# deweylab/RSEM

Hardware: AMD Instinct MI355X
Metric: EM read-alignments/s (nnz x EM iterations per second), rsem-run-em theta-only rounds (higher is better)
Workload: dtype f64; 1 GPU; BASELINE configs[2] (PairedEndQModel-shaped, the north-star target config): EM matrix of 50000000 reads x 200000 transcripts, 570042118 alignments (11.40/read) per GPU, frozen conprb (rounds >= 12); synthetic_config=C3, kernel=0, parallelism=1 GPU

## Files before the change

### rsem_amd/csrc/em.hip

```cpp
#include <climits>
#include <cstdlib>
#include <cmath>
#include <type_traits>

#include "comm_internal.hpp"
#include "em_internal.hpp"
#include "upload.hpp"
#include "sell_layout.hpp"

namespace {

using rsem::kEpsilon;

constexpr int kReduceBlocks = 64;
constexpr int kMaxTimedRounds = 4096;
constexpr int kWindow = 2048;
static_assert(kWindow == kLayoutWindow, "the layout sorts reads apart and sizes windows for the E step's LDS window (sell_layout.hpp)");

constexpr int kTotSlots = 64;

struct Ctrl {
    int done;
    int final_round;
    int totNum;
// ... 256 lines not shown
constexpr int kCloseMax = 128;
__device__ inline void solo_close_round(const SoloArgs& A, int M, double N0, const double* __restrict__ cur) {
    const int n_close = min((int)gridDim.x, kCloseMax);
    const int stride = (int)gridDim.x / n_close;
    const int rel = (int)blockIdx.x - stride / 2;
    if (rel < 0 || rel % stride != 0 || rel / stride >= n_close) return;
    const int me = rel / stride;
    const int lane = threadIdx.x & 63;
    const int n = M + 1;
    const int per = (n + n_close - 1) / n_close;
    const int lo = me * per, hi = min(n, lo + per);
    constexpr int kPre = 8;
    double pc[kPre], pp[kPre];
    const bool pre = per <= kPre * kBlock;
    if (pre) {
#pragma unroll
        for (int k = 0; k < kPre; k++) {
            const int i = lo + (int)threadIdx.x + kBlock * k;
            pc[k] = i < hi ? cur[i] : 0.0;
            pp[k] = i < hi ? A.prev[i] : 0.0;
        }
    }
    const double extra_c = wave_sum(cur[n + lane]) + N0, sum_c = wave_sum(cur[n + kTotSlots + lane]) + N0;
    const double extra_p = wave_sum(A.prev[n + lane]) + N0, sum_p = wave_sum(A.prev[n + kTotSlots + lane]) + N0;
    int tot = 0;
    double bmax = 0.0, csum = 0.0;
    auto one = [&](int i, double craw, double praw) {
        csum += craw + (i == 0 ? extra_c : 0.0);
        const double th = (craw + (i == 0 ? extra_c : 0.0)) / sum_c;
        const double old = (praw + (i == 0 ? extra_p : 0.0)) / sum_p;
        A.prev[i] = 0.0;
        if (old >= 1e-7) {
            const double change = fabs(th - old) / old;
            if (change >= 0.001) ++tot;
            bmax = fmax(bmax, change);
        }
    };
    if (pre) {
#pragma unroll
        for (int k = 0; k < kPre; k++) {
            const int i = lo + (int)threadIdx.x + kBlock * k;
            if (i < hi) one(i, pc[k], pp[k]);
        }
    } else {
        for (int i = lo + threadIdx.x; i < hi; i += kBlock) one(i, cur[i], A.prev[i]);
    }
    for (int d = 32; d >= 1; d >>= 1) {
        tot += __shfl_xor(tot, d);
        bmax = fmax(bmax, __shfl_xor(bmax, d));
    }
    csum = wave_sum(csum);
    __shared__ int s_tot[kBlock / 64];
    __shared__ double s_b[kBlock / 64], s_c[kBlock / 64];
    if (lane == 0) { s_tot[threadIdx.x >> 6] = tot; s_b[threadIdx.x >> 6] = bmax; s_c[threadIdx.x >> 6] = csum; }
    __syncthreads();
    if (threadIdx.x == 0) {
        for (int i = 1; i < kBlock / 64; i++) { tot += s_tot[i]; bmax = fmax(bmax, s_b[i]); csum += s_c[i]; }
        Ctrl* ctrl = A.ctrl;
        unsigned int zero = 0;
        if (bmax > 0.0) {
            const unsigned long long was = __hip_atomic_fetch_max(&ctrl->bbits, (unsigned long long)__double_as_longlong(bmax),
                                                                  __ATOMIC_RELAXED, __HIP_MEMORY_SCOPE_AGENT);
            asm volatile("v_and_b32 %0, 0, %1" : "=v"(zero) : "v"((unsigned int)was));
        }
        zero += sum_slot_put(ctrl, me, csum);
        const unsigned long long old = __hip_atomic_fetch_add(&ctrl->tick2, (((unsigned long long)(unsigned)tot << 32) | 1ull) + zero,
                                                              __ATOMIC_RELAXED, __HIP_MEMORY_SCOPE_AGENT);
        if ((int)(old & 0xffffffffull) == n_close - 1) {
            const int round = A.stat_round;
            const int totNum = (int)(old >> 32) + tot;
            const unsigned long long bb = __hip_atomic_load(&ctrl->bbits, __ATOMIC_RELAXED, __HIP_MEMORY_SCOPE_AGENT);
            const double fsum = sum_slots_take(ctrl, n_close);
            ctrl->last_sum = fsum;
            ctrl->last_bchange = __longlong_as_double((long long)bb);
            ctrl->last_totNum = totNum;
            ctrl->last_round = round;
            const bool stop = !(round < A.min_round || (totNum > 0 && round < A.max_round));
            if (stop) {
                ctrl->done = 1;
                ctrl->final_round = round;
            }
            if (A.mirror) {
                RoundStat* h = &A.mirror->hist[(round - 1) % kHistCap];
                h->sum = fsum;
                h->bchange = __longlong_as_double((long long)bb);
                h->totNum = totNum;
                h->round = round;
                if (stop) A.mirror->final_round = round;
                __hip_atomic_store(&A.mirror->last_round, round, __ATOMIC_RELEASE, __HIP_MEMORY_SCOPE_SYSTEM);
                if (stop) __hip_atomic_store(&A.mirror->done, 1, __ATOMIC_RELEASE, __HIP_MEMORY_SCOPE_SYSTEM);
            }
            __hip_atomic_store(&ctrl->bbits, 0ull, __ATOMIC_RELAXED, __HIP_MEMORY_SCOPE_AGENT);
            __hip_atomic_store(&ctrl->tick2, 0ull, __ATOMIC_RELAXED, __HIP_MEMORY_SCOPE_AGENT);
            for (int k = 0; k < 2 * kTotSlots; k++) A.prev[n + k] = 0.0;
        }
    }
}

__global__ __launch_bounds__(kBlock) void k_solo_finish(int32_t M, double N0, const double* __restrict__ buf, double* theta, double* counts_last) {
    const int n = M + 1;
    const int lane = threadIdx.x & 63;
    const double extra0 = wave_sum(buf[n + lane]) + N0, sum = wave_sum(buf[n + kTotSlots + lane]) + N0;
    const int i = blockIdx.x * blockDim.x + threadIdx.x;
    if (i < n) {
        const double c = buf[i] + (i == 0 ? extra0 : 0.0);
        counts_last[i] = c;
        theta[i] = c / sum;
    }
}

#ifndef RSEM_FQ_DEPTH
#define RSEM_FQ_DEPTH 3
#endif
constexpr int kFarQDepth = RSEM_FQ_DEPTH;
template <bool kFC, bool kSolo = false, bool kFQ = false>
__global__ __launch_bounds__(kBlock) void k_estep_lane(
    const Shape* __restrict__ shapes, const Unit* __restrict__ units, uint32_t T, int M,
    const double* __restrict__ theta, const double* __restrict__ tsrc, double N0, const unsigned char* __restrict__ sval,
    const int16_t* __restrict__ sexp, const int32_t* __restrict__ ssid, const double* __restrict__ sncp,
    const unsigned long long* __restrict__ masks, double* counts, double* noise_partial, double* totals, const Ctrl* ctrl,
    unsigned long long* trace, SoloArgs solo = SoloArgs(), XArgs xa = XArgs()) {
    if (ctrl->done) return;
    if (trace && threadIdx.x == 0) trace[2 * blockIdx.x] = wall_clock64();
    __shared__ double th_win[kWindow];
    __shared__ double cnt_win[kWindow];
    __shared__ int fq_sid[kFQ ? (kBlock / 64) * kFarQCap : 1];
    __shared__ double fq_val[kFQ ? (kBlock / 64) * kFarQCap : 1];
    __shared__ int fq_n[kBlock / 64];
    const Unit U = units[blockIdx.x];
    const int lane = threadIdx.x & 63;
    const int w = __builtin_amdgcn_readfirstlane((int)(threadIdx.x >> 6));
    FarQueue fq;
    if (kFQ) {
        fq.sid = fq_sid + w * kFarQCap;
        fq.val = fq_val + w * kFarQCap;
        fq.n = fq_n + w;
        if (lane == 0) fq_n[w] = 0;
    }
    if (kSolo && solo.stat_round > 0) solo_close_round(solo, M, N0, theta);
    double noise = 0.0, neff = 0.0;
    {
        const Shape& G = U.S;
        Shape S;
        S.plane_base = G.plane_base;
        S.slice_base = G.slice_base;
        S.n_slices = G.n_slices;
        S.row_base = 0;
        S.n_rows = 0;
        S.slot_base = G.slot_base;
        S.K = G.K;
        S.lg = G.lg;
        S.fmt = G.fmt;
        S.val_base = G.val_base;
        const uint32_t u_end = S.slice_base + U.slice_begin + U.n_slices;
        const uint32_t s_begin = S.slice_base + U.slice_begin + (uint32_t)w * U.per_wave;
        const uint32_t s_end = min(u_end, s_begin + U.per_wave);
#define RSEM_ESTEP_BLOCK(KK, QQ, FF, XX) \
    estep_block<KK, kFC, QQ, (QQ ? kQ32Depth[KK - 1] : kF64Depth[KK - 1]), FF, XX>(S, s_begin, s_end, lane, U.base, U.span, theta, tsrc, N0, th_win, cnt_win, sval, sexp, ssid, sncp, masks, counts, noise, neff, M, xa)
#define RSEM_ESTEP_BLOCK_FQ(KK, QQ, XX) \
    estep_block<KK, kFC, QQ, kFarQDepth, true, XX, true>(S, s_begin, s_end, lane, U.base, U.span, theta, tsrc, N0, th_win, cnt_win, sval, sexp, ssid, sncp, masks, counts, noise, neff, M, xa, fq)
        const int code = (S.K - 1) | ((S.fmt == kFmtQ32 ? 1 : 0) << 2) | ((U.pad[0] != 0 ? 1 : 0) << 3) | (((!kFC && S.fmt == kFmtF64X) ? 1 : 0) << 4);
        if constexpr (kFQ) {
            if (s_begin < u_end) switch ((code & 7) | ((code >> 4) << 3)) {
                case 0: RSEM_ESTEP_BLOCK_FQ(1, false, false); break;
                case 1: RSEM_ESTEP_BLOCK_FQ(2, false, false); break;
                case 2: RSEM_ESTEP_BLOCK_FQ(3, false, false); break;
                case 3: RSEM_ESTEP_BLOCK_FQ(4, false, false); break;
                case 4: RSEM_ESTEP_BLOCK_FQ(1, true, false); break;
                case 5: RSEM_ESTEP_BLOCK_FQ(2, true, false); break;
                case 6: RSEM_ESTEP_BLOCK_FQ(3, true, false); break;
                case 7: RSEM_ESTEP_BLOCK_FQ(4, true, false); break;
                default:
                    if constexpr (!kFC) switch (code & 3) {
                        case 0: RSEM_ESTEP_BLOCK_FQ(1, false, true); break;
                        case 1: RSEM_ESTEP_BLOCK_FQ(2, false, true); break;
                        case 2: RSEM_ESTEP_BLOCK_FQ(3, false, true); break;
                        default: RSEM_ESTEP_BLOCK_FQ(4, false, true); break;
                    }
                    break;
            } else {
                const ThetaSrc th = theta_src<kFC>(theta, tsrc, N0, lane);
                stage_windows<kFC>(U.base, U.span, M, th, th_win, cnt_win);
            }
        } else
        if (s_begin < u_end) switch (code) {
            case 0: RSEM_ESTEP_BLOCK(1, false, false, false); break;
            case 1: RSEM_ESTEP_BLOCK(2, false, false, false); break;
            case 2: RSEM_ESTEP_BLOCK(3, false, false, false); break;
            case 3: RSEM_ESTEP_BLOCK(4, false, false, false); break;
            case 4: RSEM_ESTEP_BLOCK(1, true, false, false); break;
            case 5: RSEM_ESTEP_BLOCK(2, true, false, false); break;
            case 6: RSEM_ESTEP_BLOCK(3, true, false, false); break;
            case 7: RSEM_ESTEP_BLOCK(4, true, false, false); break;
            case 8: RSEM_ESTEP_BLOCK(1, false, true, false); break;
            case 9: RSEM_ESTEP_BLOCK(2, false, true, false); break;
            case 10: RSEM_ESTEP_BLOCK(3, false, true, false); break;
            case 11: RSEM_ESTEP_BLOCK(4, false, true, false); break;
            case 12: RSEM_ESTEP_BLOCK(1, true, true, false); break;
            case 13: RSEM_ESTEP_BLOCK(2, true, true, false); break;
            case 14: RSEM_ESTEP_BLOCK(3, true, true, false); break;
            case 15: RSEM_ESTEP_BLOCK(4, true, true, false); break;
            default:
                if constexpr (!kFC) switch (code & 11) {
                    case 0: RSEM_ESTEP_BLOCK(1, false, false, true); break;
                    case 1: RSEM_ESTEP_BLOCK(2, false, false, true); break;
                    case 2: RSEM_ESTEP_BLOCK(3, false, false, true); break;
                    case 3: RSEM_ESTEP_BLOCK(4, false, false, true); break;
                    case 8: RSEM_ESTEP_BLOCK(1, false, true, true); break;
                    case 9: RSEM_ESTEP_BLOCK(2, false, true, true); break;
                    case 10: RSEM_ESTEP_BLOCK(3, false, true, true); break;
                    default: RSEM_ESTEP_BLOCK(4, false, true, true); break;
                }
                break;
#undef RSEM_ESTEP_BLOCK
#undef RSEM_ESTEP_BLOCK_FQ
        } else {
            const ThetaSrc th = theta_src<kFC>(theta, tsrc, N0, lane);
            stage_windows<kFC>(U.base, U.span, M, th, th_win, cnt_win);
        }
    }
    __syncthreads();
    for (int i = threadIdx.x; i < U.span; i += blockDim.x) {
        const double v = cnt_win[i];
        if (v != 0.0) unsafeAtomicAdd(&counts[U.base + i], v);
    }
    block_add_totals(noise, neff, noise_partial, totals);
    if (trace && threadIdx.x == 0) trace[2 * blockIdx.x + 1] = wall_clock64();
}


__device__ inline double block_sum_det(double v) {
    __shared__ double red[kBlock / 64];
    __syncthreads();
    v = wave_sum(v);
    if ((threadIdx.x & 63) == 0) red[threadIdx.x >> 6] = v;
    __syncthreads();
    double t = 0.0;
    for (int i = 0; i < kBlock / 64; i++) t += red[i];
    return t;
}

__global__ __launch_bounds__(kBlock) void k_mstep_reduce(int32_t M, double N0, double* counts,
                                                          const double* __restrict__ noise_a, int n_a,
                                                          const double* __restrict__ noise_b, int n_b,
                                                          double* partials, const Ctrl* ctrl) {
    if (ctrl && ctrl->done) return;
    const int n = M + 1;
    const int per = (n + gridDim.x - 1) / gridDim.x;
    const int lo = blockIdx.x * per, hi = min(n, lo + per);
    if (blockIdx.x == 0) {
        double v = 0.0;
        for (int i = threadIdx.x; i < n_a; i += blockDim.x) v += noise_a[i];
        for (int i = threadIdx.x; i < n_b; i += blockDim.x) v += noise_b[i];
        double t = block_sum_det(v);
        if (threadIdx.x == 0) counts[0] = counts[0] + t + N0;
        __syncthreads();
    }
    double v = 0.0;
    for (int i = lo + threadIdx.x; i < hi; i += blockDim.x) v += counts[i];
    double t = block_sum_det(v);
    if (threadIdx.x == 0) partials[blockIdx.x] = t;
}

__global__ __launch_bounds__(kBlock) void k_mstep_apply(int32_t M, const double* __restrict__ partials,
                                                         int n_partials, double* counts,
                                                         const double* __restrict__ theta_old,
                                                         double* theta_new, double* counts_last, Ctrl* ctrl,
                                                         int round, int min_round, int max_round) {
    if (ctrl->done) return;
    double sum = 0.0;
    for (int i = 0; i < n_partials; i++) sum += partials[i];
    int tot = 0;
    double bmax = 0.0;
    for (int i = blockIdx.x * blockDim.x + threadIdx.x; i <= M; i += gridDim.x * blockDim.x) {
        double c = counts[i];
        double th = c / sum;
        theta_new[i] = th;
        counts_last[i] = c;
        counts[i] = 0.0;
        double old = theta_old[i];
        if (old >= 1e-7) {
            double change = fabs(th - old) / old;
            if (change >= 0.001) ++tot;
            bmax = fmax(bmax, change);
        }
    }
    __shared__ int s_tot[kBlock / 64];
    __shared__ double s_b[kBlock / 64];
    for (int d = 32; d >= 1; d >>= 1) {
        tot += __shfl_xor(tot, d);
        bmax = fmax(bmax, __shfl_xor(bmax, d));
    }
    if ((threadIdx.x & 63) == 0) { s_tot[threadIdx.x >> 6] = tot; s_b[threadIdx.x >> 6] = bmax; }
    __syncthreads();
    if (threadIdx.x == 0) {
        for (int i = 1; i < kBlock / 64; i++) { tot += s_tot[i]; bmax = fmax(bmax, s_b[i]); }
        if (tot) atomicAdd(&ctrl->totNum, tot);
        atomicMax(&ctrl->bbits, (unsigned long long)__double_as_longlong(bmax));
        __threadfence();
        unsigned int t = atomicAdd(&ctrl->ticket, 1u);
        if (t == gridDim.x - 1) {
            int totNum = atomicAdd(&ctrl->totNum, 0);
            unsigned long long bb = atomicMax(&ctrl->bbits, 0ull);
            ctrl->last_sum = sum;
            ctrl->last_bchange = __longlong_as_double((long long)bb);
            ctrl->last_totNum = totNum;
// ... 84 lines not shown
        unsigned int tk = atomicAdd(&ctrl->ticket, 1u);
        if (tk == gridDim.x - 1) {
            int totNum = atomicAdd(&ctrl->totNum, 0);
            unsigned long long bb = atomicMax(&ctrl->bbits, 0ull);
            ctrl->last_sum = sum;
            ctrl->last_bchange = __longlong_as_double((long long)bb);
            ctrl->last_totNum = totNum;
            ctrl->last_round = round;
            if (!(round < min_round || (totNum > 0 && round < max_round))) {
                ctrl->done = 1;
                ctrl->final_round = round;
            }
            atomicExch(&ctrl->totNum, 0);
            atomicExch(&ctrl->bbits, 0ull);
            atomicExch(&ctrl->ticket, 0u);
            atomicExch(&ctrl->bar, 0u);
        }
    }
}

template <bool kFused>
__global__ __launch_bounds__(kBlock) void k_mstep_fast(int32_t M, double N0, double* counts, double* totals,
                                                        const double* __restrict__ theta_old, double* theta_new,
                                                        double* counts_last, Ctrl* ctrl, int round, int min_round, int max_round,
                                                        HostMirror* mirror, double* spent) {
    if (ctrl->done) return;
    const int n = M + 1;
    const int nb = gridDim.x;
    const int per = (n + nb - 1) / nb;
    const int lo = blockIdx.x * per, hi = min(n, lo + per);
    __shared__ double s_totals[2];
    if (threadIdx.x < 64) {
        double a = __hip_atomic_load(&totals[threadIdx.x], __ATOMIC_RELAXED, __HIP_MEMORY_SCOPE_AGENT);
        double b = __hip_atomic_load(&totals[kTotSlots + threadIdx.x], __ATOMIC_RELAXED, __HIP_MEMORY_SCOPE_AGENT);
        a = wave_sum(a);
        b = wave_sum(b);
        if (threadIdx.x == 0) { s_totals[0] = a; s_totals[1] = b; }
    }
    constexpr int kPre = 8;
    const bool pre = (hi - lo) <= kPre * (int)blockDim.x;
    double pc[kPre], po[kPre];
    if (pre) {
#pragma unroll
        for (int k = 0; k < kPre; k++) {
            const int i = lo + (int)threadIdx.x + k * (int)blockDim.x;
            pc[k] = i < hi ? counts[i] : 0.0;
            po[k] = i < hi ? theta_old[i] : 0.0;
        }
    }
    __syncthreads();
    const double extra0 = s_totals[0] + N0;
    const double sum = s_totals[1] + N0;
    int tot = 0;
    double bmax = 0.0, csum = 0.0;
    auto one = [&](int i, double craw, double old) {
        const double c = craw + (i == 0 ? extra0 : 0.0);
        csum += c;
        const double th = c / sum;
        theta_new[i] = th;
        counts_last[i] = c;
        if (kFused) spent[i] = 0.0;
        else counts[i] = 0.0;
        if (old >= 1e-7) {
            const double change = fabs(th - old) / old;
            if (change >= 0.001) ++tot;
            bmax = fmax(bmax, change);
        }
    };
    if (kFused && blockIdx.x == 0 && threadIdx.x < 2 * kTotSlots) spent[n + threadIdx.x] = 0.0;
    if (pre) {
#pragma unroll
        for (int k = 0; k < kPre; k++) {
            const int i = lo + (int)threadIdx.x + k * (int)blockDim.x;
            if (i < hi) one(i, pc[k], po[k]);
        }
    } else {
        for (int i = lo + threadIdx.x; i < hi; i += blockDim.x) one(i, counts[i], theta_old[i]);
    }
    __shared__ int s_tot[kBlock / 64];
    __shared__ double s_b[kBlock / 64], s_c[kBlock / 64];
    for (int d = 32; d >= 1; d >>= 1) {
        tot += __shfl_xor(tot, d);
        bmax = fmax(bmax, __shfl_xor(bmax, d));
    }
    csum = wave_sum(csum);
    __shared__ int s_last;
    if ((threadIdx.x & 63) == 0) { s_tot[threadIdx.x >> 6] = tot; s_b[threadIdx.x >> 6] = bmax; s_c[threadIdx.x >> 6] = csum; }
    if (threadIdx.x == 0) s_last = 0;
    __syncthreads();
    if (threadIdx.x == 0) {
        for (int i = 1; i < kBlock / 64; i++) { tot += s_tot[i]; bmax = fmax(bmax, s_b[i]); csum += s_c[i]; }
        unsigned int zero = 0;
        if (bmax > 0.0) {
            const unsigned long long was = __hip_atomic_fetch_max(&ctrl->bbits, (unsigned long long)__double_as_longlong(bmax),
                                                                  __ATOMIC_RELAXED, __HIP_MEMORY_SCOPE_AGENT);
            asm volatile("v_and_b32 %0, 0, %1" : "=v"(zero) : "v"((unsigned int)was));
        }
        zero += sum_slot_put(ctrl, (int)blockIdx.x, csum);
        const unsigned long long old = __hip_atomic_fetch_add(&ctrl->tick2, (((unsigned long long)(unsigned)tot << 32) | 1ull) + zero,
                                                              __ATOMIC_RELAXED, __HIP_MEMORY_SCOPE_AGENT);
        if ((unsigned)(old & 0xffffffffull) == gridDim.x - 1) {
            const int totNum = (int)(old >> 32) + tot;
            const unsigned long long bb = __hip_atomic_load(&ctrl->bbits, __ATOMIC_RELAXED, __HIP_MEMORY_SCOPE_AGENT);
            const double fsum = sum_slots_take(ctrl, (int)gridDim.x);
            ctrl->last_sum = fsum;
            ctrl->last_bchange = __longlong_as_double((long long)bb);
            ctrl->last_totNum = totNum;
            ctrl->last_round = round;
            const bool stop = !(round < min_round || (totNum > 0 && round < max_round));
            if (stop) {
                ctrl->done = 1;
                ctrl->final_round = round;
            }
            if (mirror) {
                RoundStat* h = &mirror->hist[(round - 1) % kHistCap];
                h->sum = fsum;
                h->bchange = __longlong_as_double((long long)bb);
                h->totNum = totNum;
                h->round = round;
                if (stop) mirror->final_round = round;
                __hip_atomic_store(&mirror->last_round, round, __ATOMIC_RELEASE, __HIP_MEMORY_SCOPE_SYSTEM);
                if (stop) __hip_atomic_store(&mirror->done, 1, __ATOMIC_RELEASE, __HIP_MEMORY_SCOPE_SYSTEM);
            }
            __hip_atomic_store(&ctrl->bbits, 0ull, __ATOMIC_RELAXED, __HIP_MEMORY_SCOPE_AGENT);
            __hip_atomic_store(&ctrl->tick2, 0ull, __ATOMIC_RELAXED, __HIP_MEMORY_SCOPE_AGENT);
            s_last = 1;
        }
    }
    __syncthreads();
    if (!kFused && s_last && threadIdx.x < 2 * kTotSlots) __hip_atomic_store(&totals[threadIdx.x], 0.0, __ATOMIC_RELAXED, __HIP_MEMORY_SCOPE_AGENT);
}

}


struct rsem_em_ctx {
    int device = 0;
    int32_t M = 0;
    uint64_t N1 = 0, nnz = 0;
    hipStream_t stream = nullptr;
    bool own_stream = true;
    uint64_t* d_row_ptr = nullptr;
    int32_t* d_sid = nullptr;
    double* d_cp = nullptr;
    double* d_ncp = nullptr;
    bool have_values = false;
    SellLayout L;
    unsigned char* d_sval = nullptr;
    double* d_sncp = nullptr;
    int16_t* d_sexp = nullptr;
    int* d_fill_err = nullptr;
    int value_bits = 64;
    int value_range_bits = 8;
    bool layout_has_q32 = false;
    bool layout_ok = false;
    Unit* d_units = nullptr;
    unsigned long long* d_trace = nullptr;
    std::vector<Unit> h_units;
    uint64_t long_nnz = 0;
    uint32_t* d_rank = nullptr;
    double *d_xextra = nullptr, *d_xinv = nullptr;
    int split_rows = 1;
    int split_policy = 1;
    uint32_t n_far_units = 0;
    unsigned long long n_stray_reads = 0;
    int tune_passes_left = 1;
    uint32_t n_units = 0;
    uint32_t n_units_main = 0;
    uint32_t n_units_compact = 0;
    uint32_t n_units_queued = 0;
    int far_queue = 1;
    hipStream_t stream_x = nullptr;
    hipEvent_t ev_x_fork = nullptr, ev_x_join = nullptr;
    int x_overlap = 0;
    int noise_n = 0;
    size_t noise_cap = 0;
    double* d_theta[2] = {nullptr, nullptr};
    double* d_red3 = nullptr;
    double* d_red = nullptr;
    double* d_counts = nullptr;
    double* d_counts_last = nullptr;
    double* d_noise_a = nullptr;
    double* d_noise_b = nullptr;
    double* d_totals = nullptr;
    bool use_totals = false;
    double* d_partials = nullptr;
    double* d_w = nullptr;
    double* d_wn = nullptr;
    Ctrl* d_ctrl = nullptr;
    int grid_main = 0, grid_long = 0, grid_apply = 0;
    int kernel = RSEM_EM_KERNEL_AUTO;
    uint32_t forced_T = 0;
    int check_every = 64;
    int n_cus = 256;
    std::vector<hipEvent_t> events;
    HostMirror* mirror = nullptr;
    hipEvent_t lag_ev[2] = {nullptr, nullptr};
    hipStream_t stream2 = nullptr;
    hipEvent_t ev_e[4] = {nullptr, nullptr, nullptr, nullptr}, ev_s[4] = {nullptr, nullptr, nullptr, nullptr};
    rsem_comm* comm = nullptr;
    bool csr_released = false;
    int views_out = 0;
    rsem_em_progress_fn progress = nullptr;
    void* progress_user = nullptr;
};

namespace {

int resolved_kernel(const rsem_em_ctx* c) {
    return c->kernel == RSEM_EM_KERNEL_AUTO ? RSEM_EM_KERNEL_LANE : c->kernel;
}

bool same_unit(const Unit& a, const Unit& b) {
    return a.shape == b.shape && a.slice_begin == b.slice_begin && a.n_slices == b.n_slices && a.per_wave == b.per_wave && a.base == b.base &&
           a.span == b.span && a.pad[0] == b.pad[0] && a.pad[1] == b.pad[1] && !memcmp(&a.S, &b.S, sizeof(Shape));
}

int partition_units(rsem_em_ctx* c) {
    auto is_main = [](const Unit& u) { return u.S.fmt != kFmtF64X; };
    const auto mid = std::stable_partition(c->h_units.begin(), c->h_units.end(), is_main);
    c->n_units_main = (uint32_t)(mid - c->h_units.begin());
    auto queued = [](const Unit& u) { return u.pad[0] != 0 && (uint64_t)u.pad[1] <= 48ull * u.n_slices; };
    c->n_units_queued = (uint32_t)std::count_if(c->h_units.begin(), mid, queued);
    c->n_units_compact = c->n_units_main;
    if (c->far_queue && c->n_units_queued * 25ull >= c->n_units_main && c->n_units_queued)
        c->n_units_compact = (uint32_t)(std::stable_partition(c->h_units.begin(), mid, [&](const Unit& u) { return !queued(u); }) - c->h_units.begin());
    if (c->n_units)
        RSEM_HIP_TRY(hipMemcpyAsync(c->d_units, c->h_units.data(), sizeof(Unit) * c->n_units, hipMemcpyHostToDevice, c->stream));
    RSEM_HIP_TRY(hipStreamSynchronize(c->stream));
    return RSEM_OK;
}

int launch_estep(rsem_em_ctx* c, const double* d_theta, double* d_counts, hipStream_t st, bool use_ctrl) {
    const Ctrl* ctrl = c->d_ctrl;
    (void)use_ctrl;
    c->noise_n = (int)c->n_units;
    {
        XArgs xa;
        const uint32_t nc = c->n_units_compact, n_main = c->n_units_main, n_all = c->n_units;
        const bool far_launch = c->far_queue && nc < n_main;
        const bool x_beside = c->x_overlap && c->L.n_x_rows && n_main > 0 && n_main < n_all;
        const bool second = c->stream_x && (x_beside || (far_launch && nc > 0));
        hipStream_t s2 = second ? c->stream_x : st;
        hipStream_t sx = x_beside ? s2 : st, sf = far_launch ? s2 : st;
        if (second) {
            RSEM_HIP_TRY(hipEventRecord(c->ev_x_fork, st));
            RSEM_HIP_TRY(hipStreamWaitEvent(s2, c->ev_x_fork, 0));
        }
        auto lane = [&](uint32_t u0, uint32_t u1, hipStream_t s) {
            if (u1 > u0)
                hipLaunchKernelGGL((k_estep_lane<false, false>), dim3(u1 - u0), dim3(kBlock), 0, s, c->L.d_shapes, c->d_units + u0, c->L.T, c->M,
                                   d_theta, (const double*)nullptr, 0.0, (const unsigned char*)c->d_sval, (const int16_t*)c->d_sexp, c->L.d_ssid,
                                   c->d_sncp, c->L.d_masks, d_counts, c->d_noise_a + u0, c->use_totals ? c->d_totals : nullptr, ctrl,
                                   c->d_trace ? c->d_trace + 2 * (size_t)u0 : nullptr, SoloArgs(), xa);
        };
        auto lane_fq = [&](uint32_t u0, uint32_t u1, hipStream_t s) {
            if (u1 > u0)
                hipLaunchKernelGGL((k_estep_lane<false, false, true>), dim3(u1 - u0), dim3(kBlock), 0, s, c->L.d_shapes, c->d_units + u0, c->L.T, c->M,
                                   d_theta, (const double*)nullptr, 0.0, (const unsigned char*)c->d_sval, (const int16_t*)c->d_sexp, c->L.d_ssid,
                                   c->d_sncp, c->L.d_masks, d_counts, c->d_noise_a + u0, c->use_totals ? c->d_totals : nullptr, ctrl,
                                   c->d_trace ? c->d_trace + 2 * (size_t)u0 : nullptr, SoloArgs(), xa);
        };
        if (c->L.n_x_rows) {
            xa.extra = c->d_xextra; xa.inv = c->d_xinv; xa.slot_base = c->L.x_slot_base;
            static const bool batched = !(getenv("RSEM_HIP_ROWSUM_BATCHED") && atoi(getenv("RSEM_HIP_ROWSUM_BATCHED")) == 0);
            hipLaunchKernelGGL(batched ? k_far_rowsum<true> : k_far_rowsum<false>, dim3(rsem::ceil_div(c->L.n_x_slots, kBlock)), dim3(kBlock), 0, sx, c->L.n_x_slots,
                               (const uint64_t*)c->L.d_far_ptr, (const int32_t*)c->L.d_far_sid, (const double*)c->L.d_far_cp, d_theta, c->d_xextra, ctrl);
        }
        if (far_launch) lane_fq(nc, n_main, sf);
        if (!far_launch && sx == st) lane(0, n_all, st);
        else {
            lane(0, far_launch ? nc : n_main, st);
            lane(n_main, n_all, sx);
        }
        if (c->L.n_far) {
            const int grid = std::max(1, rsem::ceil_div(c->L.n_far, kBlock * 4));
            static const bool xcd = !(getenv("RSEM_HIP_COLSUM_XCD") && atoi(getenv("RSEM_HIP_COLSUM_XCD")) == 0);
            hipLaunchKernelGGL(xcd ? k_far_colsum<true> : k_far_colsum<false>, dim3(grid), dim3(kBlock), 0, sx, c->L.n_far, (const int32_t*)c->L.d_csc_sid,
                               (const double*)c->L.d_csc_cp, (const uint32_t*)c->L.d_csc_slot, c->L.x_slot_base, d_theta, (const double*)c->d_xinv, d_counts, ctrl);
        }
        if (second) {
            RSEM_HIP_TRY(hipGetLastError());
            RSEM_HIP_TRY(hipEventRecord(c->ev_x_join, s2));
            RSEM_HIP_TRY(hipStreamWaitEvent(st, c->ev_x_join, 0));
        }
    }
    RSEM_HIP_TRY(hipGetLastError());
    if (c->L.n_long_rows) {
        hipLaunchKernelGGL(k_estep_long, dim3(c->grid_long), dim3(kBlock), 0, st, (uint64_t)c->L.n_long_rows,
                           (const uint32_t*)(c->L.d_order + c->L.n_sell_rows), (const uint64_t*)c->d_row_ptr, (const int32_t*)c->d_sid, (const double*)c->d_cp,
                           (const double*)c->d_ncp, d_theta, d_counts, c->d_noise_b, ctrl, c->use_totals ? c->d_totals : nullptr);
        RSEM_HIP_TRY(hipGetLastError());
    }
    return RSEM_OK;
}

int n_noise_b(const rsem_em_ctx* c) {
    return c->L.n_long_rows ? c->grid_long : 0;
}

int launch_weights(rsem_em_ctx* c, const double* d_theta, hipStream_t st) {
    const int grid = std::max(1, std::min<int>(c->n_cus * 16, rsem::ceil_div(c->N1, kBlock)));
    hipLaunchKernelGGL(k_weights_csr, dim3(grid), dim3(kBlock), 0, st, c->N1, c->d_row_ptr, c->d_sid, c->d_cp, c->d_ncp, d_theta,
                       c->d_w, c->d_wn);
    RSEM_HIP_TRY(hipGetLastError());
    return RSEM_OK;
}

int launch_mstep(rsem_em_ctx* c, double N0, double* d_counts, const double* d_theta_old, double* d_theta_new,
                 int round, int min_round, int max_round, hipStream_t st, HostMirror* mirror = nullptr) {
    const int grid = std::max(1, std::min(kMstepBlocks, rsem::ceil_div((uint64_t)c->M + 1, kBlock * 4)));
    if (c->use_totals) {
        const int gridf = std::max(1, std::min(2 * kMstepBlocks, rsem::ceil_div((uint64_t)c->M + 1, kBlock * 2)));
        hipLaunchKernelGGL(k_mstep_fast<false>, dim3(gridf), dim3(kBlock), 0, st, c->M, N0, d_counts, c->d_totals, d_theta_old, d_theta_new,
                           c->d_counts_last, c->d_ctrl, round, min_round, max_round, mirror, (double*)nullptr);
        RSEM_HIP_TRY(hipGetLastError());
        return RSEM_OK;
    }
    hipLaunchKernelGGL(k_mstep_fused, dim3(grid), dim3(kBlock), 0, st, c->M, N0, d_counts, c->d_noise_a, c->noise_n,
                       c->d_noise_b, n_noise_b(c), c->d_partials, d_theta_old, d_theta_new, c->d_counts_last, c->d_ctrl,
                       round, min_round, max_round);
    RSEM_HIP_TRY(hipGetLastError());
    return RSEM_OK;
}

int build_layout(rsem_em_ctx* c);
void free_layout(rsem_em_ctx* c);

__global__ void k_sum_row_lengths(uint32_t n, const uint32_t* __restrict__ rows, const uint64_t* __restrict__ row_ptr, unsigned long long* out) {
    unsigned long long v = 0;
    for (uint32_t i = blockIdx.x * blockDim.x + threadIdx.x; i < n; i += gridDim.x * blockDim.x) v += row_ptr[rows[i] + 1] - row_ptr[rows[i]];
    for (int d = 32; d >= 1; d >>= 1) v += __shfl_xor(v, d);
    if ((threadIdx.x & 63) == 0 && v) atomicAdd(out, v);
}

int release_csr(rsem_em_ctx* c) {
    if (c->csr_released) return RSEM_OK;
    const char* why = nullptr;
    if (!c->layout_ok || !c->have_values) why = "there is no layout with values yet";
    else if (c->layout_has_q32 || c->value_bits == 32) why = "Q32 planes hold rounded values";
    else if (c->L.n_x_rows) why = "split rows keep part of their alignments outside the planes";
    else if (c->L.n_long_rows) why = "reads with more than 256 alignments live in the CSR alone";
    else if (c->views_out > 0) why = "a model context still holds the arrays";
    if (why) { rsem::set_last_error("release_csr: %s", why); return RSEM_ERR_STATE; }
    RSEM_HIP_TRY(hipSetDevice(c->device));
    RSEM_HIP_TRY(hipStreamSynchronize(c->stream));
    (void)hipFree(c->d_sid); c->d_sid = nullptr;
    (void)hipFree(c->d_cp); c->d_cp = nullptr;
    c->csr_released = true;
    return RSEM_OK;
}

int ensure_csr(rsem_em_ctx* c) {
    if (!c->csr_released) return RSEM_OK;
    RSEM_HIP_TRY(hipSetDevice(c->device));
    RSEM_HIP_TRY(dmalloc(&c->d_sid, c->nnz));
    if (hipError_t e = dmalloc(&c->d_cp, c->nnz); e != hipSuccess) {
        (void)hipFree(c->d_sid);
        c->d_sid = nullptr;
        RSEM_HIP_TRY(e);
    }
    if (c->L.n_sell_rows)
        hipLaunchKernelGGL(k_unfill_sell, dim3(rsem::ceil_div(c->L.n_sell_rows, kBlock)), dim3(kBlock), 0, c->stream, c->L.d_shapes, c->L.n_shapes, c->L.T,
                           c->L.n_sell_rows, (const uint32_t*)c->L.d_order, (const uint64_t*)c->d_row_ptr, (const int32_t*)c->L.d_ssid,
                           (const unsigned char*)c->d_sval, c->d_sid, c->d_cp);
    RSEM_HIP_TRY(hipGetLastError());
    RSEM_HIP_TRY(hipStreamSynchronize(c->stream));
    c->csr_released = false;
    return RSEM_OK;
}

int write_values(rsem_em_ctx* c) {
    if (c->d_fill_err) RSEM_HIP_TRY(hipMemsetAsync(c->d_fill_err, 0, sizeof(int), c->stream));
    int rc = sell_fill_values(c->L, c->stream, c->d_row_ptr, c->d_cp, c->d_ncp, c->d_sval, c->d_sncp, c->d_sexp, c->d_fill_err, c->d_sid);
    if (rc != RSEM_OK) return rc;
    if (c->layout_has_q32) {
        int h = 0;
        RSEM_HIP_TRY(hipMemcpyAsync(&h, c->d_fill_err, sizeof(int), hipMemcpyDeviceToHost, c->stream));
        RSEM_HIP_TRY(hipStreamSynchronize(c->stream));
        if (h) { rsem::set_last_error("Q32 planes: a read's values left the range its format was chosen for"); return RSEM_ERR_STATE; }
    }
    return RSEM_OK;
}

int fill_values(rsem_em_ctx* c) {
    if (c->value_bits == 32 || c->layout_has_q32) {
        free_layout(c);
        return build_layout(c);
    }
    return write_values(c);
}

void free_layout(rsem_em_ctx* c) {
    sell_free(c->L);
    hipFree(c->d_rank); hipFree(c->d_xextra); hipFree(c->d_xinv);
    c->d_rank = nullptr; c->d_xextra = nullptr; c->d_xinv = nullptr;
    hipFree(c->d_sval); hipFree(c->d_sncp); hipFree(c->d_sexp); hipFree(c->d_fill_err); hipFree(c->d_units); hipFree(c->d_noise_a);
    c->d_sval = nullptr; c->d_sncp = nullptr; c->d_sexp = nullptr; c->d_fill_err = nullptr; c->d_units = nullptr; c->d_noise_a = nullptr;
    c->h_units.clear();
    c->n_units = 0;
    c->layout_has_q32 = false;
    c->layout_ok = false;
}

int build_layout(rsem_em_ctx* c) {
    const uint32_t target_waves = (uint32_t)c->n_cus * 4 * 6 * 5 / 2;
    const bool q32 = c->value_bits == 32 && c->have_values;
    std::vector<Unit> units;
    int split = c->split_rows && resolved_kernel(c) == RSEM_EM_KERNEL_LANE && !q32;
    if (const char* e = getenv("RSEM_HIP_SPLIT")) split = split && atoi(e) != 0;
    if (split) split = c->split_policy;
    if (const char* e = getenv("RSEM_HIP_SPLIT_POLICY")) { if (split) split = !strcmp(e, "all") ? 2 : 1; }
    int rc = sell_build_refined(c->L, c->stream, c->N1, c->M, c->d_row_ptr, c->d_sid, target_waves, c->forced_T,
                                q32 ? c->d_cp : nullptr, c->value_range_bits, kWindow, units, &c->d_units, &c->n_stray_reads, split);
    if (rc != RSEM_OK) return rc;
    if (c->L.n_x_rows) {
        const size_t nxs = (size_t)(c->L.n_slots - c->L.x_slot_base);
        RSEM_HIP_TRY(dmalloc(&c->d_xextra, nxs));
        RSEM_HIP_TRY(dmalloc(&c->d_xinv, nxs));
        RSEM_HIP_TRY(hipMemsetAsync(c->d_xextra, 0, sizeof(double) * std::max<size_t>(nxs, 1), c->stream));
        RSEM_HIP_TRY(hipMemsetAsync(c->d_xinv, 0, sizeof(double) * std::max<size_t>(nxs, 1), c->stream));
    }
    c->layout_has_q32 = q32;
    RSEM_HIP_TRY(hipMalloc((void**)&c->d_sval, std::max<uint64_t>(c->L.val_bytes, 1)));
    RSEM_HIP_TRY(dmalloc(&c->d_sncp, (size_t)c->L.n_slots));
    if (q32) {
        RSEM_HIP_TRY(dmalloc(&c->d_sexp, (size_t)c->L.n_slots));
        RSEM_HIP_TRY(dmalloc(&c->d_fill_err, 1));
    }
    RSEM_HIP_TRY(hipMemsetAsync(c->d_sval, 0, c->L.val_bytes, c->stream));
    RSEM_HIP_TRY(hipMemsetAsync(c->d_sncp, 0, sizeof(double) * c->L.n_slots, c->stream));
    if (c->have_values) {
        rc = write_values(c);
        if (rc != RSEM_OK) return rc;
    }
    RSEM_HIP_TRY(hipStreamSynchronize(c->stream));
    c->n_units = (uint32_t)units.size();
    c->h_units = units;
    if (const char* e = getenv("RSEM_HIP_X_OVERLAP")) c->x_overlap = atoi(e);
    if (const char* e = getenv("RSEM_HIP_FAR_QUEUE")) c->far_queue = atoi(e);
    rc = partition_units(c);
    if (rc != RSEM_OK) return rc;
    if ((c->L.n_x_rows || c->n_units_compact < c->n_units_main) && !c->stream_x) {
        RSEM_HIP_TRY(hipStreamCreateWithFlags(&c->stream_x, hipStreamNonBlocking));
        RSEM_HIP_TRY(hipEventCreateWithFlags(&c->ev_x_fork, hipEventDisableTiming));
        RSEM_HIP_TRY(hipEventCreateWithFlags(&c->ev_x_join, hipEventDisableTiming));
    }
    c->tune_passes_left = 1;
    if (const char* e = getenv("RSEM_HIP_TUNE")) c->tune_passes_left = atoi(e);
    c->n_far_units = 0;
    for (const Unit& u : c->h_units) c->n_far_units += u.pad[0] != 0;
    c->noise_cap = std::max<size_t>((size_t)c->n_cus * 8, c->n_units);
    RSEM_HIP_TRY(dmalloc(&c->d_noise_a, c->noise_cap));
    RSEM_HIP_TRY(hipMemsetAsync(c->d_noise_a, 0, sizeof(double) * c->noise_cap, c->stream));

    c->grid_long = std::max(1, std::min<int>(c->n_cus * 8, rsem::ceil_div(c->L.n_long_rows, kBlock / 64)));
    c->long_nnz = 0;
    if (c->L.n_long_rows) {
        unsigned long long* d_n = (unsigned long long*)c->d_noise_a;
        hipLaunchKernelGGL(k_sum_row_lengths, dim3(c->grid_long), dim3(kBlock), 0, c->stream, c->L.n_long_rows, c->L.d_order + c->L.n_sell_rows,
                           c->d_row_ptr, d_n);
        RSEM_HIP_TRY(hipGetLastError());
        unsigned long long h = 0;
        RSEM_HIP_TRY(hipMemcpyAsync(&h, d_n, sizeof(h), hipMemcpyDeviceToHost, c->stream));
        RSEM_HIP_TRY(hipMemsetAsync(c->d_noise_a, 0, sizeof(double), c->stream));
        RSEM_HIP_TRY(hipStreamSynchronize(c->stream));
        c->long_nnz = h;
    }
    c->layout_ok = true;
    return RSEM_OK;
}

void set_grid_for_kernel(rsem_em_ctx* c) {
    c->grid_main = std::max(1, std::min<int>(c->n_cus * 8, rsem::ceil_div(c->L.n_slices, kBlock / 64)));
}

}

extern "C" {

int rsem_em_create(rsem_em_ctx** out, int device, int32_t M, uint64_t N1, uint64_t nnz, const uint64_t* row_ptr,
                   const int32_t* sid, const double* conprb, const double* ncp) {
    RSEM_REQUIRE(out != nullptr, "out is NULL");
    *out = nullptr;
    RSEM_REQUIRE(M >= 1, "M must be >= 1");
    RSEM_REQUIRE(row_ptr != nullptr && (sid != nullptr || nnz == 0), "row_ptr / sid is NULL");
    RSEM_REQUIRE(N1 < 0xfffffff0ull, "N1 too large for one shard (max 2^32-16 reads)");
    RSEM_REQUIRE(row_ptr[0] == 0 && row_ptr[N1] == nnz, "row_ptr[0] != 0 or row_ptr[N1] != nnz");
    RSEM_REQUIRE((conprb == nullptr) == (ncp == nullptr), "conprb and ncp must be given together");
    int ndev = 0;
    if (hipGetDeviceCount(&ndev) != hipSuccess || device < 0 || device >= ndev) {
        (void)hipGetLastError();
        rsem::set_last_error("no HIP device %d (have %d)", device, ndev);
        return RSEM_ERR_NODEVICE;
    }
    RSEM_HIP_TRY(hipSetDevice(device));
    hipDeviceProp_t prop;
    RSEM_HIP_TRY(hipGetDeviceProperties(&prop, device));
    rsem_em_ctx* c = new (std::nothrow) rsem_em_ctx();
    if (!c) return RSEM_ERR_NOMEM;
    c->device = device;
    c->M = M;
    c->N1 = N1;
    c->nnz = nnz;
    c->n_cus = prop.multiProcessorCount > 0 ? prop.multiProcessorCount : 256;
    int rc = RSEM_OK;
    auto fail = [&](int code) { rsem_em_destroy(c); return code; };
#define TRY_OR_FAIL(expr)                                                                               \
    do {                                                                                                \
        hipError_t _e = (expr);                                                                         \
        if (_e != hipSuccess) {                                                                         \
            rsem::set_last_error("%s:%d: %s -> %s", __FILE__, __LINE__, #expr, hipGetErrorString(_e));  \
            return fail(_e == hipErrorOutOfMemory ? RSEM_ERR_NOMEM : RSEM_ERR_HIP);                     \
        }                                                                                               \
    } while (0)
    TRY_OR_FAIL(hipStreamCreateWithFlags(&c->stream, hipStreamNonBlocking));
    TRY_OR_FAIL(dmalloc(&c->d_row_ptr, N1 + 1));
    TRY_OR_FAIL(dmalloc(&c->d_sid, nnz));
    TRY_OR_FAIL(dmalloc(&c->d_cp, nnz));
    TRY_OR_FAIL(dmalloc(&c->d_ncp, N1));
    if ((rc = rsem::staged_h2d(c->d_row_ptr, row_ptr, sizeof(uint64_t) * (N1 + 1), c->stream)) != RSEM_OK) return fail(rc);
    if ((rc = rsem::staged_h2d(c->d_sid, sid, sizeof(int32_t) * nnz, c->stream)) != RSEM_OK) return fail(rc);
    if (conprb) {
        if ((rc = rsem::staged_h2d(c->d_cp, conprb, sizeof(double) * nnz, c->stream)) != RSEM_OK) return fail(rc);
        if ((rc = rsem::staged_h2d(c->d_ncp, ncp, sizeof(double) * N1, c->stream)) != RSEM_OK) return fail(rc);
        c->have_values = true;
    }
    for (int i = 0; i < 2; i++) TRY_OR_FAIL(dmalloc(&c->d_theta[i], (size_t)M + 1));
    TRY_OR_FAIL(dmalloc(&c->d_red3, 3 * ((size_t)M + 1 + 2 * kTotSlots)));
    c->d_red = c->d_red3;
    c->d_counts = c->d_red;
    c->d_totals = c->d_red + (size_t)M + 1;
    TRY_OR_FAIL(dmalloc(&c->d_counts_last, (size_t)M + 1));
    TRY_OR_FAIL(dmalloc(&c->d_noise_b, (size_t)c->n_cus * 8));
    TRY_OR_FAIL(hipMemsetAsync(c->d_totals, 0, sizeof(double) * 2 * kTotSlots, c->stream));
    TRY_OR_FAIL(hipHostMalloc((void**)&c->mirror, sizeof(HostMirror), hipHostMallocDefault));
    memset(c->mirror, 0, sizeof(HostMirror));
    for (int i = 0; i < 2; i++) TRY_OR_FAIL(hipEventCreateWithFlags(&c->lag_ev[i], hipEventDisableTiming));
    {
        int least = 0, greatest = 0;
        TRY_OR_FAIL(hipDeviceGetStreamPriorityRange(&least, &greatest));
        TRY_OR_FAIL(hipStreamCreateWithPriority(&c->stream2, hipStreamNonBlocking, greatest));
    }
    for (int i = 0; i < 4; i++) {
        TRY_OR_FAIL(hipEventCreateWithFlags(&c->ev_e[i], hipEventDisableTiming));
        TRY_OR_FAIL(hipEventCreateWithFlags(&c->ev_s[i], hipEventDisableTiming));
    }
    TRY_OR_FAIL(dmalloc(&c->d_partials, 2 * kReduceBlocks));
    TRY_OR_FAIL(dmalloc(&c->d_ctrl, 1));
    TRY_OR_FAIL(hipMemsetAsync(c->d_counts, 0, sizeof(double) * ((size_t)M + 1), c->stream));
    TRY_OR_FAIL(hipMemsetAsync(c->d_noise_b, 0, sizeof(double) * c->n_cus * 8, c->stream));
    TRY_OR_FAIL(hipMemsetAsync(c->d_ctrl, 0, sizeof(Ctrl), c->stream));
    c->grid_apply = std::max(1, std::min(c->n_cus * 2, rsem::ceil_div((uint64_t)M + 1, kBlock)));
    if (const char* e = getenv("RSEM_HIP_T")) c->forced_T = (uint32_t)atoi(e);
    rc = build_layout(c);
    if (rc != RSEM_OK) return fail(rc);
    set_grid_for_kernel(c);
    rsem::thread_stager().release();
#undef TRY_OR_FAIL
    *out = c;
    return RSEM_OK;
}

int rsem_em_set_values(rsem_em_ctx* c, const double* conprb, const double* ncp) {
    RSEM_REQUIRE(c && conprb && ncp, "NULL argument");
    RSEM_HIP_TRY(hipSetDevice(c->device));
    { int rc0 = ensure_csr(c); if (rc0 != RSEM_OK) return rc0; }
    if (c->nnz) RSEM_HIP_TRY(hipMemcpyAsync(c->d_cp, conprb, sizeof(double) * c->nnz, hipMemcpyHostToDevice, c->stream));
    if (c->N1) RSEM_HIP_TRY(hipMemcpyAsync(c->d_ncp, ncp, sizeof(double) * c->N1, hipMemcpyHostToDevice, c->stream));
    c->have_values = true;
    int rc = fill_values(c);
    if (rc != RSEM_OK) return rc;
    RSEM_HIP_TRY(hipStreamSynchronize(c->stream));
    return RSEM_OK;
}

int rsem_em_get_values(rsem_em_ctx* c, double* conprb, double* ncp) {
    RSEM_REQUIRE(c && conprb && ncp, "NULL argument");
    if (!c->have_values) { rsem::set_last_error("CSR values were never set"); return RSEM_ERR_STATE; }
    RSEM_HIP_TRY(hipSetDevice(c->device));
    { int rc0 = ensure_csr(c); if (rc0 != RSEM_OK) return rc0; }
    if (c->nnz) RSEM_HIP_TRY(hipMemcpyAsync(conprb, c->d_cp, sizeof(double) * c->nnz, hipMemcpyDeviceToHost, c->stream));
    if (c->N1) RSEM_HIP_TRY(hipMemcpyAsync(ncp, c->d_ncp, sizeof(double) * c->N1, hipMemcpyDeviceToHost, c->stream));
    RSEM_HIP_TRY(hipStreamSynchronize(c->stream));
    return RSEM_OK;
}

int rsem_em_shard_rows(uint64_t N1, const uint64_t* row_ptr, int world, uint64_t* bounds) {
    RSEM_REQUIRE(row_ptr && bounds && world >= 1, "bad argument");
    const uint64_t nhT = row_ptr[N1] / (uint64_t)world;
    uint64_t cur = 0;
    bounds[0] = 0;
    for (int i = 0; i < world; i++) {
        const uint64_t left_threads = (uint64_t)(world - i - 1);
        if (i == world - 1) cur = N1;
        else {
            const uint64_t cap = N1 > left_threads ? N1 - left_threads : 0;
            const uint64_t target = row_ptr[cur] + nhT;
            uint64_t nxt = (uint64_t)(std::lower_bound(row_ptr + cur, row_ptr + N1 + 1, target) - row_ptr);
            nxt = std::min(nxt, std::max(cap, cur));
            cur = std::max(cur, nxt);
        }
        bounds[i + 1] = cur;
    }
    return RSEM_OK;
}

int rsem_em_set_comm(rsem_em_ctx* c, rsem_comm* comm) {
    RSEM_REQUIRE(c != nullptr, "NULL argument");
    c->comm = comm;
    return RSEM_OK;
}

int rsem_em_set_progress(rsem_em_ctx* c, rsem_em_progress_fn fn, void* user) {
    RSEM_REQUIRE(c != nullptr, "NULL argument");
    c->progress = fn;
    c->progress_user = user;
    return RSEM_OK;
}

int rsem_em_set_option(rsem_em_ctx* c, const char* key, int64_t value) {
    RSEM_REQUIRE(c && key, "NULL argument");
    if (!strcmp(key, "release_csr")) {
        RSEM_REQUIRE(value == 0 || value == 1, "release_csr must be 0 or 1");
        return value ? release_csr(c) : ensure_csr(c);
    }
    if (!strcmp(key, "kernel") || !strcmp(key, "split_rows") || !strcmp(key, "split_policy") || !strcmp(key, "value_bits") || !strcmp(key, "value_range_bits")) {
        int rc0 = ensure_csr(c);
        if (rc0 != RSEM_OK) return rc0;
    }
    if (!strcmp(key, "kernel")) {
        RSEM_REQUIRE(value >= RSEM_EM_KERNEL_AUTO && value <= RSEM_EM_KERNEL_LANE, "unknown kernel variant");
        RSEM_REQUIRE(value == RSEM_EM_KERNEL_AUTO || value == RSEM_EM_KERNEL_LANE, "kernel variants CSR (1) and SELL (2) were retired: AUTO (0) or LANE (3)");
        c->kernel = (int)value;
        if (c->layout_ok && c->L.n_x_rows && resolved_kernel(c) != RSEM_EM_KERNEL_LANE) {
            RSEM_HIP_TRY(hipSetDevice(c->device));
            free_layout(c);
            int rc = build_layout(c);
            if (rc != RSEM_OK) return rc;
        }
        set_grid_for_kernel(c);
        return RSEM_OK;
    }
    if (!strcmp(key, "split_overlap")) {
        RSEM_REQUIRE(value == 0 || value == 1, "split_overlap must be 0 or 1");
        c->x_overlap = (int)value;
        return RSEM_OK;
    }
    if (!strcmp(key, "split_policy")) {
        RSEM_REQUIRE(value == 1 || value == 2, "split_policy must be 1 (reads mostly outside their window) or 2 (every read with an id outside)");
        if (c->split_policy == (int)value) return RSEM_OK;
        c->split_policy = (int)value;
        c->x_overlap = value == 2 ? 1 : 0;
        RSEM_HIP_TRY(hipSetDevice(c->device));
        free_layout(c);
        int rc = build_layout(c);
        if (rc != RSEM_OK) return rc;
        set_grid_for_kernel(c);
        return RSEM_OK;
    }
    if (!strcmp(key, "split_rows")) {
        RSEM_REQUIRE(value == 0 || value == 1, "split_rows must be 0 or 1");
        if (c->split_rows == (int)value) return RSEM_OK;
        c->split_rows = (int)value;
        RSEM_HIP_TRY(hipSetDevice(c->device));
        free_layout(c);
        int rc = build_layout(c);
        if (rc != RSEM_OK) return rc;
        set_grid_for_kernel(c);
        return RSEM_OK;
    }
    if (!strcmp(key, "value_bits") || !strcmp(key, "value_range_bits")) {
        const bool bits = !strcmp(key, "value_bits");
        if (bits) RSEM_REQUIRE(value == 64 || value == 32, "value_bits must be 64 or 32");
        else RSEM_REQUIRE(value >= 0 && value <= 24, "value_range_bits must be in 0..24");
        int& field = bits ? c->value_bits : c->value_range_bits;
        if (field == (int)value) return RSEM_OK;
        field = (int)value;
        if (c->value_bits == 64 && !c->layout_has_q32) return RSEM_OK;
        RSEM_HIP_TRY(hipSetDevice(c->device));
        free_layout(c);
        int rc = build_layout(c);
        if (rc != RSEM_OK) return rc;
        set_grid_for_kernel(c);
        return RSEM_OK;
    }
    if (!strcmp(key, "check_every")) {
        RSEM_REQUIRE(value >= 1 && value <= kHistCap / 4, "check_every out of range");
        c->check_every = (int)value;
        return RSEM_OK;
    }
    rsem::set_last_error("unknown option '%s'", key);
    return RSEM_ERR_INVALID;
}

int rsem_em_get_info(const rsem_em_ctx* c, const char* key, int64_t* value) {
    RSEM_REQUIRE(c && key && value, "NULL argument");
    if (!strcmp(key, "value_bits")) *value = c->value_bits;
    else if (!strcmp(key, "csr_released")) *value = c->csr_released ? 1 : 0;
    else if (!strcmp(key, "csr_bytes")) *value = (int64_t)(12 * c->nnz);
    else if (!strcmp(key, "value_range_bits")) *value = c->value_range_bits;
    else if (!strcmp(key, "far_units")) *value = c->n_far_units;
    else if (!strcmp(key, "units")) *value = c->n_units;
    else if (!strcmp(key, "units_compact")) *value = c->n_units_compact;
    else if (!strcmp(key, "units_main")) *value = c->n_units_main;
    else if (!strcmp(key, "units_queued")) *value = c->n_units_queued;
    else if (!strcmp(key, "unit_tables_agree")) {
        std::vector<Unit> d(c->n_units);
        if (c->n_units) {
            RSEM_HIP_TRY(hipSetDevice(c->device));
            RSEM_HIP_TRY(hipMemcpyAsync(d.data(), c->d_units, sizeof(Unit) * c->n_units, hipMemcpyDeviceToHost, c->stream));
            RSEM_HIP_TRY(hipStreamSynchronize(c->stream));
        }
        bool same = d.size() == c->h_units.size();
        for (size_t i = 0; same && i < d.size(); i++) same = same_unit(d[i], c->h_units[i]);
        *value = same ? 1 : 0;
    }
    else if (!strcmp(key, "stray_reads")) *value = (int64_t)c->n_stray_reads;
    else if (!strcmp(key, "reads_q32")) *value = c->L.n_q32_rows;
    else if (!strcmp(key, "reads_sliced")) *value = c->L.n_sell_rows;
    else if (!strcmp(key, "reads_long")) *value = c->L.n_long_rows;
    else if (!strcmp(key, "value_plane_bytes")) *value = (int64_t)c->L.val_bytes;
    else if (!strcmp(key, "sid_plane_bytes")) *value = (int64_t)(c->L.n_planes * 256);
    else if (!strcmp(key, "slots")) *value = c->L.n_slots;
    else if (!strcmp(key, "sid_plane_bytes_loaded")) *value = (int64_t)(c->L.n_sid_planes_loaded * 256);
    else if (!strcmp(key, "slices")) *value = c->L.n_slices;
    else if (!strcmp(key, "split_rows")) *value = c->L.n_x_rows;
    else if (!strcmp(key, "far_entries")) *value = (int64_t)c->L.n_far;
    else if (!strcmp(key, "window_entries")) {
        int64_t w = 0;
        for (const Unit& u : c->h_units) w += u.span;
        *value = w;
    } else if (!strcmp(key, "physical_bytes_per_launch")) {
        int64_t w = 0;
        for (const Unit& u : c->h_units) w += u.span;
        const uint64_t long_nnz = c->long_nnz + (c->L.n_long_rows * 4ull) / 3;
        const uint64_t far_bytes = 28 * c->L.n_far + 40 * (uint64_t)c->L.n_x_slots;
        *value = (int64_t)(c->L.val_bytes + c->L.n_sid_planes_loaded * 256 + (uint64_t)c->L.n_slots * (8 + (c->layout_has_q32 ? 2 : 0)) +
                           (uint64_t)c->L.n_slices * 8 + (uint64_t)c->n_units * sizeof(Unit) + (uint64_t)w * 16 + 16 * ((uint64_t)c->M + 1)) +
                 (int64_t)(12 * long_nnz + far_bytes);
    }
    else if (!strcmp(key, "units")) *value = c->n_units;
    else { rsem::set_last_error("unknown info key '%s'", key); return RSEM_ERR_INVALID; }
    return RSEM_OK;
}

int rsem_em_debug_trace(rsem_em_ctx* c, const double* theta, unsigned long long* out, uint32_t* n_units_io) {
    RSEM_REQUIRE(c && theta && out && n_units_io, "NULL argument");
    RSEM_REQUIRE(resolved_kernel(c) == RSEM_EM_KERNEL_LANE && c->have_values && c->layout_ok, "needs the LANE kernel with values set");
    RSEM_REQUIRE(*n_units_io >= c->n_units, "trace buffer too small");
    RSEM_HIP_TRY(hipSetDevice(c->device));
    unsigned long long* d = nullptr;
    RSEM_HIP_TRY(hipMalloc((void**)&d, sizeof(unsigned long long) * 2 * std::max<uint32_t>(c->n_units, 1)));
    RSEM_HIP_TRY(hipMemcpyAsync(c->d_theta[0], theta, sizeof(double) * ((size_t)c->M + 1), hipMemcpyHostToDevice, c->stream));
    RSEM_HIP_TRY(hipMemsetAsync(c->d_ctrl, 0, sizeof(Ctrl), c->stream));
    int rc = RSEM_OK;
    for (int rep = 0; rep < 3 && rc == RSEM_OK; rep++) {
        c->d_trace = d;
        rc = launch_estep(c, c->d_theta[0], c->d_counts, c->stream, true);
        c->d_trace = nullptr;
    }
    hipError_t e = hipMemcpyAsync(out, d, sizeof(unsigned long long) * 2 * c->n_units, hipMemcpyDeviceToHost, c->stream);
    if (e == hipSuccess) e = hipStreamSynchronize(c->stream);
    (void)hipMemsetAsync(c->d_counts, 0, sizeof(double) * ((size_t)c->M + 1), c->stream);
    (void)hipStreamSynchronize(c->stream);
    (void)hipFree(d);
    if (e != hipSuccess) { rsem::set_last_error("trace download failed"); return RSEM_ERR_HIP; }
    *n_units_io = c->n_units;
    return rc;
}

int rsem_em_destroy(rsem_em_ctx* c) {
    if (!c) return RSEM_OK;
    (void)hipSetDevice(c->device);
    for (hipEvent_t e : c->events) (void)hipEventDestroy(e);
    hipFree(c->d_row_ptr); hipFree(c->d_sid); hipFree(c->d_cp); hipFree(c->d_ncp);
    sell_free(c->L); hipFree(c->d_sval); hipFree(c->d_sncp); hipFree(c->d_sexp); hipFree(c->d_fill_err);
    hipFree(c->d_theta[0]); hipFree(c->d_theta[1]); hipFree(c->d_red3);
    for (int i = 0; i < 4; i++) { if (c->ev_e[i]) (void)hipEventDestroy(c->ev_e[i]); if (c->ev_s[i]) (void)hipEventDestroy(c->ev_s[i]); }
    if (c->stream2) (void)hipStreamDestroy(c->stream2);
    if (c->stream_x) (void)hipStreamDestroy(c->stream_x);
    if (c->ev_x_fork) (void)hipEventDestroy(c->ev_x_fork);
    if (c->ev_x_join) (void)hipEventDestroy(c->ev_x_join);
    hipFree(c->d_counts_last); hipFree(c->d_noise_a); hipFree(c->d_noise_b); hipFree(c->d_partials);
    if (c->mirror) (void)hipHostFree(c->mirror);
    for (int i = 0; i < 2; i++) if (c->lag_ev[i]) (void)hipEventDestroy(c->lag_ev[i]);
    hipFree(c->d_w); hipFree(c->d_wn); hipFree(c->d_ctrl); hipFree(c->d_units);
    if (c->stream && c->own_stream) (void)hipStreamDestroy(c->stream);
    delete c;
    return RSEM_OK;
}

static int tune_unit_order(rsem_em_ctx* c, const double* d_theta) {
    while (c->tune_passes_left > 0) {
        --c->tune_passes_left;
        if (resolved_kernel(c) != RSEM_EM_KERNEL_LANE || c->n_units < 2048) return RSEM_OK;
        const uint32_t n = c->n_units;
        unsigned long long* d = nullptr;
        RSEM_HIP_TRY(hipMalloc((void**)&d, sizeof(unsigned long long) * 2 * n));
        std::vector<unsigned long long> t(2 * (size_t)n);
        int rc = RSEM_OK;
        for (int rep = 0; rep < 2 && rc == RSEM_OK; rep++) {
            c->d_trace = d;
            rc = launch_estep(c, d_theta, c->d_counts, c->stream, true);
            c->d_trace = nullptr;
        }
        hipError_t e = hipMemcpyAsync(t.data(), d, sizeof(unsigned long long) * 2 * n, hipMemcpyDeviceToHost, c->stream);
        if (e == hipSuccess) e = hipStreamSynchronize(c->stream);
        (void)hipFree(d);
        if (rc != RSEM_OK) return rc;
        if (e != hipSuccess) { rsem::set_last_error("unit tuning: trace download failed"); return RSEM_ERR_HIP; }
        std::vector<uint32_t> order(n);
        for (uint32_t i = 0; i < n; i++) order[i] = i;
        std::stable_sort(order.begin(), order.end(), [&](uint32_t a, uint32_t b) { return t[2 * a + 1] - t[2 * a] > t[2 * b + 1] - t[2 * b]; });
        std::vector<Unit> sorted(n);
        for (uint32_t i = 0; i < n; i++) sorted[i] = c->h_units[order[i]];
        c->h_units.swap(sorted);
        rc = partition_units(c);
        if (rc != RSEM_OK) return rc;
    }
    return RSEM_OK;
}

namespace {
__global__ void k_seed_theta_source(int32_t M, const double* __restrict__ theta, double N0, double* buf) {
    const int i = blockIdx.x * blockDim.x + threadIdx.x;
    const int n = M + 1;
    if (i < n) buf[i] = theta[i];
    if (i < 2 * kTotSlots) buf[n + i] = (i == 0) ? -N0 : (i == kTotSlots ? 1.0 - N0 : 0.0);
}

__global__ __launch_bounds__(kBlock) void k_solo_close(int M, const double* __restrict__ cur, double N0, const Ctrl* ctrl, SoloArgs solo) {
    if (ctrl->done) return;
    solo_close_round(solo, M, N0, cur);
}

enum class Loop { PLAIN, FUSED, SOLO };
Loop loop_wanted(const rsem_em_ctx* c, bool sharded) {
    const bool possible = resolved_kernel(c) == RSEM_EM_KERNEL_LANE && c->L.n_long_rows == 0 && c->n_units > 0 && c->L.n_x_rows == 0;
    if (!possible) return Loop::PLAIN;
    const char* e = getenv("RSEM_EM_FUSED");
    if (e && !strcmp(e, "0")) return Loop::PLAIN;
    if (e && !strcmp(e, "1")) return Loop::FUSED;
    if (e && !strcmp(e, "2") && !sharded) return Loop::SOLO;
    if (!sharded) return Loop::SOLO;
    return 12ull * c->nnz + 16ull * c->N1 >= 2500000000ull ? Loop::FUSED : Loop::PLAIN;
}
}

int rsem_em_run(rsem_em_ctx* c, double* theta, double N0, int round0, int min_round, int max_round, int* rounds_done,
                double* counts, double* bChange, int32_t* totNum, rsem_em_profile* prof) {
    RSEM_REQUIRE(c && theta, "NULL argument");
    RSEM_REQUIRE(max_round > round0, "max_round must exceed round0");
    if (!c->have_values) { rsem::set_last_error("CSR values were never set"); return RSEM_ERR_STATE; }
    if (!c->layout_ok) { rsem::set_last_error("the device layout could not be rebuilt after the last change of values / options"); return RSEM_ERR_STATE; }
    RSEM_HIP_TRY(hipSetDevice(c->device));
    hipStream_t st = c->stream;
    const size_t nb = sizeof(double) * ((size_t)c->M + 1);
    RSEM_HIP_TRY(hipMemcpyAsync(c->d_theta[round0 & 1], theta, nb, hipMemcpyHostToDevice, st));
    RSEM_HIP_TRY(hipMemsetAsync(c->d_ctrl, 0, sizeof(Ctrl), st));
    if (c->tune_passes_left > 0) {
        int trc = tune_unit_order(c, c->d_theta[round0 & 1]);
        if (trc != RSEM_OK) return trc;
    }
    RSEM_HIP_TRY(hipMemsetAsync(c->d_counts, 0, nb, st));
    RSEM_HIP_TRY(hipMemsetAsync(c->d_totals, 0, sizeof(double) * 2 * kTotSlots, st));
    c->use_totals = resolved_kernel(c) == RSEM_EM_KERNEL_LANE;
    struct TotalsOff { rsem_em_ctx* c; ~TotalsOff() { c->use_totals = false; } } totals_off{c};
    const int timed = prof ? std::min(max_round - round0, kMaxTimedRounds) : 0;
    if (prof) {
        while ((int)c->events.size() < 2 * timed + 2) {
            hipEvent_t e;
            RSEM_HIP_TRY(hipEventCreate(&e));
            c->events.push_back(e);
        }
// ... 317 lines not shown
```

### rsem_amd/csrc/estep_block.hpp

```cpp
#pragma once
#include <type_traits>

#include "simt_macros.hpp"

RSEM_DEVFN double wave_sum(double v) {
#pragma unroll
    for (int d = 32; d >= 1; d >>= 1) v += RSEM_SHFL_XOR(v, d);
    return v;
}


struct ThetaSrc {
    const double* v;
    double extra0, sum;
};
template <bool kFC>
RSEM_DEVFN double theta_at(const ThetaSrc& t, int i) {
    if (!kFC) return t.v[i];
    return (t.v[i] + (i == 0 ? t.extra0 : 0.0)) / t.sum;
}
template <bool kFC>
RSEM_DEVFN ThetaSrc theta_src(const double* __restrict__ v, const double* __restrict__ tsrc, double N0, int lane);

template <bool kFC>
RSEM_DEVFN void stage_windows(int base, int span, int M, const ThetaSrc& th, double* th_win, double* cnt_win) {
    for (int i = RSEM_TIDX; i < span; i += RSEM_BDIM) {
        const int sidv = base + i;
        th_win[i] = (sidv >= 0 && sidv <= M) ? theta_at<kFC>(th, sidv) : 0.0;
        cnt_win[i] = 0.0;
    }
    RSEM_SYNC();
}

struct XArgs {
    const double* extra = nullptr;
    double* inv = nullptr;
    uint32_t slot_base = 0;
};

#ifndef RSEM_FARQ_CAP
#define RSEM_FARQ_CAP 384
#endif
constexpr int kFarQCap = RSEM_FARQ_CAP;
static_assert(kFarQCap > 256, "a slice of K = 4 planes can append 256 entries");
struct FarQueue {
    int* sid = nullptr;
    double* val = nullptr;
    int* n = nullptr;
};

template <int K, bool kQ>
struct SliceRegs {
    int id[K];
    typename std::conditional<kQ, uint32_t, double>::type c[K];
    double nc;
    int e;
    double x;
    uint32_t slot0;
    double traw[K];
};

RSEM_DEVFN double pow2_of(int e) { return RSEM_LL_AS_DOUBLE((long long)(1023 + e) << 52); }

#ifndef RSEM_F64_DEPTHS
#define RSEM_F64_DEPTHS 2, 2, 2, 2
#endif
#ifndef RSEM_Q32_DEPTHS
#define RSEM_Q32_DEPTHS 2, 2, 2, 2
#endif
template <typename T>
RSEM_DEVFN T stream_load(const T* p) { return RSEM_NT_LOAD(p); }
template <int kCtrl>
RSEM_DEVFN double dpp_take(double v) {
    const long long b = RSEM_DOUBLE_AS_LL(v);
    const int lo = RSEM_DPP_MOV((int)(unsigned)b, kCtrl);
    const int hi = RSEM_DPP_MOV((int)(unsigned)(b >> 32), kCtrl);
    return RSEM_LL_AS_DOUBLE(((long long)hi << 32) | (unsigned)lo);
}
RSEM_DEVFN double read_sum_dpp(double part, int lg) {
    if (lg >= 1) part += dpp_take<0xB1>(part);
    if (lg >= 2) part += dpp_take<0x4E>(part);
    if (lg >= 3) part += dpp_take<0x141>(part);
    if (lg >= 4) part += dpp_take<0x140>(part);
    for (int d = 16; d < (1 << lg); d <<= 1) part += RSEM_SHFL_XOR(part, d);
    return part;
}
constexpr int kF64Depth[4] = {RSEM_F64_DEPTHS};
constexpr int kQ32Depth[4] = {RSEM_Q32_DEPTHS};

template <int K, bool kFC, bool kQ, int NBUF, bool kFar, bool kX = false, bool kFQ = false>
RSEM_DEVFN void estep_block(const Shape& S, uint32_t s_begin, uint32_t s_end, int lane, int base, int span,
                                   const double* __restrict__ theta, const double* __restrict__ tsrc, double N0, double* th_win, double* cnt_win,
                                   const unsigned char* __restrict__ sval, const int16_t* __restrict__ sexp, const int32_t* __restrict__ ssid,
                                   const double* __restrict__ sncp, const unsigned long long* __restrict__ masks,
                                   double* counts, double& noise, double& neff, int M, const XArgs& X = XArgs(), const FarQueue& FQ = FarQueue()) {
    static_assert(!kFQ || kFar, "the far queue belongs to the loop of the units with ids outside their window");
    static_assert(!kFQ || NBUF >= 3, "the far-queue loop requests theta a slice ahead: three register sets at least (the ring loop)");
    using ValT = typename std::conditional<kQ, uint32_t, double>::type;
    const ValT* __restrict__ scp = (const ValT*)(sval + S.val_base);
    const int lg = S.lg;
    const int g = lane & ((1 << lg) - 1);
    const bool g0 = (g == 0);
    const uint32_t R = 64u >> lg;
    uint32_t m_base = s_begin;
    unsigned long long mv = (s_begin + lane < s_end) ? masks[s_begin + lane] : ~0ull;
    auto mask_of = [&](uint32_t t) -> unsigned long long {
        if (t - m_base >= 64u) {
            m_base = t;
            mv = (t + lane < s_end) ? masks[t + lane] : ~0ull;
            RSEM_PIN(mv);
        }
        const int src = (int)(t - m_base);
        const uint32_t lo = RSEM_READLANE((int)(uint32_t)mv, src);
        const uint32_t hi = RSEM_READLANE((int)(uint32_t)(mv >> 32), src);
        return ((unsigned long long)hi << 32) | lo;
    };
    const unsigned ulane = (unsigned)lane, uslot = ulane >> lg;
    auto issue = [&](uint32_t t, unsigned long long m, SliceRegs<K, kQ>& b) {
        const uint32_t sl = t - S.slice_base;
        const uint64_t v0 = (uint64_t)sl * (K * 64);
        const ValT* __restrict__ vp = scp + v0;
        if (kFQ || m != 0ull) {
            const int32_t* __restrict__ ip = ssid + (S.plane_base * 64 + v0);
#pragma unroll
            for (int k = 0; k < K; k++) b.id[k] = ip[k * 64 + ulane];
        }
#pragma unroll
        for (int k = 0; k < K; k++) b.c[k] = stream_load(&vp[k * 64 + ulane]);
        const uint32_t slot0 = S.slot_base + sl * R;
        b.nc = (sncp + slot0)[uslot];
        b.e = kQ ? (int)(sexp + slot0)[uslot] : 0;
        b.x = kX ? (X.extra + (slot0 - X.slot_base))[uslot] : 0.0;
        b.slot0 = slot0;
    };
    auto spill = [&](const int* rsid, double* acc) {
#pragma unroll
        for (int k = 0; k < K; k++) {
            if (acc[k] != 0.0) {
                const unsigned off = (unsigned)(rsid[k] - base);
                if (!kFar) RSEM_LDS_ADD(&cnt_win[off < (unsigned)span ? off : 0u], acc[k]);
                else if (off < (unsigned)span) RSEM_LDS_ADD(&cnt_win[off], acc[k]);
                else if (kFQ) {
                    const int at = RSEM_LDS_FETCH_ADD_I32(FQ.n, 1);
                    FQ.sid[at] = rsid[k];
                    FQ.val[at] = acc[k];
                } else RSEM_ATOMIC_ADD(&counts[rsid[k]], acc[k]);
            }
            acc[k] = 0.0;
        }
    };
    auto far_queue_room = [&](bool all) {
        if (!kFQ) return;
        RSEM_WAVE_SYNC();
        const int n = RSEM_READFIRSTLANE(*FQ.n);
        if (n > (all ? 0 : kFarQCap - 64 * K)) {
            for (int i = lane; i < n; i += 64) RSEM_ATOMIC_ADD(&counts[FQ.sid[i]], FQ.val[i]);
            RSEM_WAIT_VM0();
            RSEM_WAVE_SYNC();
            if (lane == 0) *FQ.n = 0;
            RSEM_WAVE_SYNC();
        }
    };

    int rsid[K];
    double rth[K], acc[K];
#pragma unroll
    for (int k = 0; k < K; k++) { rsid[k] = 0; rth[k] = 0.0; acc[k] = 0.0; }
    ThetaSrc th{theta, 0.0, 1.0};
    double th0 = 0.0;
    auto pregather = [&](SliceRegs<K, kQ>& b, unsigned long long m) {
        if (!kFQ) return;
        const bool starts = ((m >> lane) & 1ull) != 0ull;
#pragma unroll
        for (int k = 0; k < K; k++) {
            const int sidv = b.id[k];
            const bool want = starts && !((unsigned)(sidv - base) < (unsigned)span);
            b.traw[k] = th.v[want ? sidv : 0];
        }
    };
    auto reduce = [&](const SliceRegs<K, kQ>& cur, unsigned long long cur_m) {
        if (cur_m != 0ull) {
            far_queue_room(false);
            if ((cur_m >> lane) & 1ull) {
                spill(rsid, acc);
                bool far = false;
#pragma unroll
                for (int k = 0; k < K; k++) {
                    const int sidv = cur.id[k];
                    rsid[k] = sidv;
                    const unsigned off = (unsigned)(sidv - base);
                    const bool in = off < (unsigned)span;
                    rth[k] = th_win[in ? off : 0u];
                    far = far || !in;
                }
                if (kFQ) {
#pragma unroll
                    for (int k = 0; k < K; k++)
                        if (!((unsigned)(rsid[k] - base) < (unsigned)span))
                            rth[k] = kFC ? (cur.traw[k] + (rsid[k] == 0 ? th.extra0 : 0.0)) / th.sum : cur.traw[k];
                } else if (kFar && far) {
                    double t[K];
#pragma unroll
                    for (int k = 0; k < K; k++) {
                        const bool in = (unsigned)(rsid[k] - base) < (unsigned)span;
                        t[k] = theta_at<kFC>(th, in ? 0 : rsid[k]);
                    }
#pragma unroll
                    for (int k = 0; k < K; k++) {
                        RSEM_PIN(t[k]);
                        if (!((unsigned)(rsid[k] - base) < (unsigned)span)) rth[k] = t[k];
                    }
                }
            }
        }
        double f0 = g0 ? th0 * cur.nc : 0.0;
        if (f0 < kEpsilon) f0 = 0.0;
        double f[K];
        double part = f0 + ((kX && g0) ? cur.x : 0.0);
        const double scale = kQ ? pow2_of(cur.e) : 1.0;
#pragma unroll
        for (int k = 0; k < K; k++) {
            const double cv = kQ ? (double)cur.c[k] * scale : (double)cur.c[k];
            double v = rth[k] * cv;
            if (v < kEpsilon) v = 0.0;
            f[k] = v;
            part += v;
        }
        part = read_sum_dpp(part, lg);
        const double inv = (part >= kEpsilon) ? 1.0 / part : 0.0;
        if (kX) RSEM_STORE_SAME(&(X.inv + (cur.slot0 - X.slot_base))[uslot], inv);
        noise += f0 * inv;
        neff += (g0 && part >= kEpsilon) ? 1.0 : 0.0;
#pragma unroll
        for (int k = 0; k < K; k++) acc[k] = acc[k] + f[k] * inv;
    };
    if constexpr (NBUF == 2) {
        SliceRegs<K, kQ> A, B;
        unsigned long long mA = ~0ull, mB = 0;
        issue(s_begin, mA, A);
        th = theta_src<kFC>(theta, tsrc, N0, lane);
        th0 = theta_at<kFC>(th, 0);
        stage_windows<kFC>(base, span, M, th, th_win, cnt_win);
        uint32_t s = s_begin;
        for (; s + 2 < s_end; s += 2) {
            mB = mask_of(s + 1);
            issue(s + 1, mB, B);
            reduce(A, mA);
            mA = mask_of(s + 2);
            issue(s + 2, mA, A);
            reduce(B, mB);
        }
        if (s + 1 < s_end) {
            mB = mask_of(s + 1);
            issue(s + 1, mB, B);
            reduce(A, mA);
            reduce(B, mB);
        } else {
            reduce(A, mA);
        }
    } else {
        SliceRegs<K, kQ> buf[NBUF];
        unsigned long long mk[NBUF];
        mk[0] = ~0ull;
        issue(s_begin, mk[0], buf[0]);
        th = theta_src<kFC>(theta, tsrc, N0, lane);
        th0 = theta_at<kFC>(th, 0);
        stage_windows<kFC>(base, span, M, th, th_win, cnt_win);
        auto within = [&](uint32_t t) -> uint32_t { return t < s_end ? t : s_end - 1u; };
#pragma unroll
        for (int j = 1; j < NBUF - 1; j++) {
            const uint32_t tt = within(s_begin + j);
            mk[j] = mask_of(tt);
            issue(tt, mk[j], buf[j]);
        }
        pregather(buf[0], mk[0]);
        uint32_t s = s_begin;
        for (; s + NBUF <= s_end; s += NBUF) {
#pragma unroll
            for (int j = 0; j < NBUF; j++) {
                constexpr int ahead = NBUF - 1;
                const int nj = (j + ahead) % NBUF;
                const uint32_t tt = within(s + j + ahead);
                mk[nj] = mask_of(tt);
                issue(tt, mk[nj], buf[nj]);
                pregather(buf[(j + 1) % NBUF], mk[(j + 1) % NBUF]);
                reduce(buf[j], mk[j]);
            }
        }
#pragma unroll
        for (int j = 0; j < NBUF - 1; j++)
            if (s + j < s_end) {
                if (j > 0) pregather(buf[j], mk[j]);
                reduce(buf[j], mk[j]);
            }
    }
    far_queue_room(false);
    spill(rsid, acc);
    far_queue_room(true);
}

template <bool kFC>
RSEM_DEVFN ThetaSrc theta_src(const double* __restrict__ v, const double* __restrict__ tsrc, double N0, int lane) {
    ThetaSrc t{v, 0.0, 1.0};
    if (kFC) {
        const double a = wave_sum(tsrc[lane]);
        const double b = wave_sum(tsrc[kTotSlots + lane]);
        t.extra0 = a + N0;
        t.sum = b + N0;
    }
    return t;
}
```

### rsem_amd/csrc/model.hip

```cpp
#include <cmath>
#include <thread>
#include <vector>

#include <hipcub/hipcub.hpp>

#include "em_internal.hpp"
#include "upload.hpp"

namespace {

using rsem::kEpsilon;
constexpr int kBlk = 256;

#include "sell_shape.hpp"
#include "model_block.hpp"

__device__ inline bool same_window(const uint64_t* __restrict__ refw, uint64_t a, uint64_t b, int len) {
    if (a == b) return true;
    const uint64_t* ra = refw + (a >> 3);
    const uint64_t* rb = refw + (b >> 3);
    const int sa = (int)(a & 7) * 8, sb = (int)(b & 7) * 8;
    uint64_t a0 = ra[0], b0 = rb[0];
    for (int i = 0; i < len; i += 8) {
        const uint64_t a1 = ra[(i >> 3) + 1], b1 = rb[(i >> 3) + 1];
// ... 75 lines not shown
        for (int i = threadIdx.x; i < kRspdLds; i += blockDim.x) s_rspd[i] = 0.0;
        for (int i = threadIdx.x; i < kGldLds; i += blockDim.x) s_gld[i] = 0.0;
    }
    __syncthreads();
    const int lane = threadIdx.x & 63;
    const uint64_t waves_per_block = blockDim.x / 64;
    if (kGroupChunk > 0)
        model_group_rows<kQ, kPE, kUpdate>(D, T, theta, cp, ncp, A, kQ ? s_prob : T.prof, s_nprob, s_prof, s_noise, s_rspd, s_gld, (uint64_t)(threadIdx.x >> 6) * 4,
                                           waves_per_block * 4, lane, PO, (uint64_t)kGroupChunk, (uint64_t)blockIdx.x, (uint64_t)gridDim.x);
    else
        model_group_rows<kQ, kPE, kUpdate>(D, T, theta, cp, ncp, A, kQ ? s_prob : T.prof, s_nprob, s_prof, s_noise, s_rspd, s_gld,
                                           ((uint64_t)blockIdx.x * waves_per_block + (threadIdx.x >> 6)) * 4, (uint64_t)gridDim.x * waves_per_block * 4, lane, PO);
    if (!kUpdate) return;
    __syncthreads();
    const int nprof = min(kProfCap, T.prof_rows * 25);
    for (int i = threadIdx.x; i < nprof; i += blockDim.x)
        if (s_prof[i] != 0.0) unsafeAtomicAdd(&A.prof[i], s_prof[i]);
    const int nnoise = kQ ? 500 : 5;
    for (int i = threadIdx.x; i < nnoise; i += blockDim.x)
        if (s_noise[i] != 0.0) unsafeAtomicAdd(&A.noise[i], s_noise[i]);
    if (A.rspd)
        for (int i = threadIdx.x; i < min(kRspdLds, T.B + 2); i += blockDim.x)
            if (s_rspd[i] != 0.0) unsafeAtomicAdd(&A.rspd[i], s_rspd[i]);
    if (A.gld)
        for (int i = threadIdx.x; i < min(kGldLds, A.gld0_ub - A.gld0_lb + 1); i += blockDim.x)
            if (s_gld[i] != 0.0) unsafeAtomicAdd(&A.gld[i], s_gld[i]);
}

__global__ void k_hit_rows(uint64_t N1, const uint64_t* __restrict__ row_ptr, uint32_t* hit_row) {
    const uint64_t i = (uint64_t)blockIdx.x * blockDim.x + threadIdx.x;
    if (i >= N1) return;
    for (uint64_t j = row_ptr[i]; j < row_ptr[i + 1]; j++) hit_row[j] = (uint32_t)i;
}

template <typename T>
hipError_t dmalloc(T** p, size_t n) { return hipMalloc((void**)p, (n ? n : 1) * sizeof(T)); }

template <typename T>
int upload(T** d, const T* h, size_t n, hipStream_t st) {
    RSEM_HIP_TRY(dmalloc(d, n));
    if (n) return rsem::staged_h2d(*d, h, sizeof(T) * n, st);
    return RSEM_OK;
}

__global__ void k_read_words(uint64_t N1, const uint64_t* __restrict__ off, uint64_t* nwords, int32_t* len) {
    const uint64_t i = (uint64_t)blockIdx.x * blockDim.x + threadIdx.x;
    if (i > N1) return;
    if (i == N1) { nwords[i] = 0; return; }
    const uint64_t l = off[i + 1] - off[i];
    len[i] = (int32_t)l;
    nwords[i] = (l + 7) / 8;
}

__global__ void k_pack_reads(uint64_t N1, const uint64_t* __restrict__ off, const uint64_t* __restrict__ off8,
                             const uint8_t* __restrict__ raw, uint64_t* words) {
    const uint64_t i = (uint64_t)blockIdx.x * blockDim.x + threadIdx.x;
    if (i >= N1) return;
    const uint64_t b0 = off[i] - off[0], l = off[i + 1] - off[i];
    uint64_t* o = words + off8[i];
    for (uint64_t w = 0; w * 8 < l; w++) {
        uint64_t v = 0;
        const uint64_t n = l - w * 8 < 8 ? l - w * 8 : 8;
        for (uint64_t k = 0; k < n; k++) v |= (uint64_t)raw[b0 + w * 8 + k] << (8 * k);
        o[w] = v;
    }
}

__global__ void k_code_reads(uint64_t N1, const uint64_t* __restrict__ off, const uint64_t* __restrict__ off8, const uint8_t* __restrict__ seq,
                             const uint8_t* __restrict__ qual, uint64_t* lo, uint64_t* hi) {
    const uint64_t t = (uint64_t)blockIdx.x * blockDim.x + threadIdx.x;
    const uint64_t i = t >> 4;
    if (i >= N1) return;
    const uint64_t b0 = off[i] - off[0], l = off[i + 1] - off[i], o8 = off8[i];
    for (uint64_t w = t & 15u; w * 8 < l; w += 16) {
        const uint64_t at = b0 + w * 8, n = l - w * 8 < 8 ? l - w * 8 : 8;
        uint64_t sb = 0, qb = 0;
        if (n == 8) {
            __builtin_memcpy(&sb, seq + at, 8);
            __builtin_memcpy(&qb, qual + at, 8);
        } else {
            for (uint64_t k = 0; k < n; k++) { sb |= (uint64_t)seq[at + k] << (8 * k); qb |= (uint64_t)qual[at + k] << (8 * k); }
        }
        uint64_t v[2] = {0, 0};
#pragma unroll
        for (int k = 0; k < 8; k++) {
            const uint64_t c = (uint64_t)k < n ? (uint64_t)read_code8((unsigned)((qb >> (8 * k)) & 0xff), (unsigned)((sb >> (8 * k)) & 0xff)) : (uint64_t)kPadCode8;
            v[k >> 2] |= c << (16 * (k & 3));
        }
        lo[o8 + w] = v[0];
        hi[o8 + w] = v[1];
    }
}

}

struct rsem_model_ctx {
    rsem_em_ctx* em = nullptr;
    bool holds_view = false;
    rsem::EmDeviceView v;
    DevData D;
    DevTables T;
    bool have_tables = false;
    int B_alloc = 0, gld_n = 0, mld_n = 0, prof_n = 0, noise_n = 0;
    std::vector<void*> owned;
    uint32_t *d_aw0 = nullptr, *d_aw1 = nullptr, *d_afull = nullptr, *d_atot = nullptr;
    uint8_t* d_flags = nullptr;
    int fields_seedLen = -1;
    double* d_theta = nullptr;
    int n_cus = 0;
    double *t_rspd_pdf = nullptr, *t_rspd_cdf = nullptr, *t_gld_pdf = nullptr, *t_gld_cdf = nullptr, *t_mld_pdf = nullptr,
           *t_mld_cdf = nullptr, *t_prof = nullptr, *t_noise = nullptr, *t_mw = nullptr;
    double *a_prof = nullptr, *a_noise = nullptr, *a_rspd = nullptr, *a_gld = nullptr;
    size_t a_prof_n = 0, a_gld_n = 0;
};

namespace {

template <typename T>
int up_field(rsem_model_ctx* c, const T*& field, const T* src, size_t n, hipStream_t st) {
    T* p = nullptr;
    int rc = upload(&p, src, n, st);
    if (rc != RSEM_OK) return rc;
    c->owned.push_back(p);
    field = p;
    return RSEM_OK;
}

template <bool kQ, bool kPE>
int launch_group(rsem_model_ctx* c, const double* d_theta, const AccumPtrs* A, const PlaneOut& PO) {
    if (!c->D.N1) return RSEM_OK;
    if (!c->n_cus) {
        hipDeviceProp_t p;
        RSEM_HIP_TRY(hipGetDeviceProperties(&p, c->v.device));
        c->n_cus = std::max(1, p.multiProcessorCount);
    }
    const uint64_t chunks = kGroupChunk > 0 ? (c->D.N1 + kGroupChunk - 1) / kGroupChunk : (c->D.N1 + 31) / 32;
    const int grid = (int)std::max<uint64_t>(1, std::min<uint64_t>((uint64_t)c->n_cus * 2, chunks));
    if (A)
        hipLaunchKernelGGL((k_model_group<kQ, kPE, true>), dim3(grid), dim3(kGroupBlk), 0, c->v.stream, c->D, c->T, d_theta, c->v.d_cp, c->v.d_ncp, *A, PO);
    else
        hipLaunchKernelGGL((k_model_group<kQ, kPE, false>), dim3(grid), dim3(kGroupBlk), 0, c->v.stream, c->D, c->T, (const double*)nullptr, c->v.d_cp,
                           c->v.d_ncp, AccumPtrs{nullptr, nullptr, nullptr, nullptr, 0, 0}, PO);
    RSEM_HIP_TRY(hipGetLastError());
    return RSEM_OK;
}
int launch_group_any(rsem_model_ctx* c, const double* d_theta, const AccumPtrs* A) {
    PlaneOut PO{nullptr, nullptr, 0, 0, 0, nullptr, nullptr};
    rsem::EmPlanesView pv;
    const char* e = getenv("RSEM_MODEL_PLANES");
    bool in_place = !(e && !strcmp(e, "0")) && rsem::em_planes_writable(c->em);
    if (in_place) {
        const int vrc = rsem::em_planes_view(c->em, &pv);
        if (vrc != RSEM_OK) return vrc;
    }
    if (in_place) PO = PlaneOut{pv.d_rank, (const Shape*)pv.d_shapes, pv.n_shapes, pv.T, pv.n_sell_rows, pv.d_sval, pv.d_sncp};
    int rc;
    switch (c->D.model_type) {
        case 0: rc = launch_group<false, false>(c, d_theta, A, PO); break;
        case 1: rc = launch_group<true, false>(c, d_theta, A, PO); break;
        case 2: rc = launch_group<false, true>(c, d_theta, A, PO); break;
        default: rc = launch_group<true, true>(c, d_theta, A, PO); break;
    }
    if (rc != RSEM_OK) return rc;
    return in_place ? rsem::em_values_written_in_place(c->em) : rsem::em_values_changed(c->em);
}

int resize_buf(double** p, int* cur, int n) {
    if (*p && *cur >= n) return RSEM_OK;
    if (*p) hipFree(*p);
    *p = nullptr;
    RSEM_HIP_TRY(dmalloc(p, (size_t)n));
    *cur = n;
    return RSEM_OK;
}

}

extern "C" {

int rsem_model_destroy(rsem_model_ctx* c) {
    if (!c) return RSEM_OK;
    (void)hipSetDevice(c->v.device);
    if (c->em && c->holds_view) rsem::em_view_release(c->em);
    for (void* p : c->owned) hipFree(p);
    hipFree(c->d_aw0); hipFree(c->d_aw1); hipFree(c->d_afull); hipFree(c->d_atot);
    hipFree(c->t_rspd_pdf); hipFree(c->t_rspd_cdf); hipFree(c->t_gld_pdf); hipFree(c->t_gld_cdf); hipFree(c->t_mld_pdf);
    hipFree(c->t_mld_cdf); hipFree(c->t_prof); hipFree(c->t_noise); hipFree(c->t_mw);
    hipFree(c->a_prof); hipFree(c->a_noise); hipFree(c->a_rspd); hipFree(c->a_gld);
    hipFree(c->d_theta);
    delete c;
    return RSEM_OK;
}

int rsem_model_create(rsem_model_ctx** out, rsem_em_ctx* em, const rsem_model_data* d) {
    RSEM_REQUIRE(out && em && d, "NULL argument");
    *out = nullptr;
    RSEM_REQUIRE(d->model_type >= 0 && d->model_type <= 3, "model_type must be 0..3");
    const bool q = d->model_type == 1 || d->model_type == 3, pe = d->model_type >= 2;
    RSEM_REQUIRE(d->row_ptr && d->sid_signed && d->pos && d->read_off[0] && d->read_seq[0] && d->low_quality && d->ref_off &&
                     d->ref_seq && d->fullLen && d->totLen && d->mask_off && d->mask_words,
                 "NULL array in rsem_model_data");
    RSEM_REQUIRE(!pe || (d->insertL && d->read_off[1] && d->read_seq[1]), "paired-end data needs insertL and mate 2");
    RSEM_REQUIRE(!q || (d->read_qual[0] && (!pe || d->read_qual[1])), "quality models need read_qual");
    rsem_model_ctx* c = new (std::nothrow) rsem_model_ctx();
    if (!c) return RSEM_ERR_NOMEM;
    c->em = em;
    int rc = rsem::em_device_view(em, &c->v);
    if (rc != RSEM_OK) { delete c; return rc; }
    rsem::em_view_hold(em);
    c->holds_view = true;
    if (c->v.N1 != d->N1 || c->v.nnz != d->nnz || c->v.M != d->M) {
        rsem_model_destroy(c);
        rsem::set_last_error("model data does not match the EM context (N1/nnz/M)");
        return RSEM_ERR_INVALID;
    }
    hipStream_t st = c->v.stream;
    DevData& D = c->D;
    memset(&D, 0, sizeof(D));
    D.model_type = d->model_type; D.M = d->M; D.N1 = d->N1; D.nnz = d->nnz;
    D.row_ptr = c->v.d_row_ptr;
#define UP(field, src, n)                                           \
    do {                                                            \
        rc = up_field(c, D.field, src, (size_t)(n), st);            \
        if (rc != RSEM_OK) { rsem_model_destroy(c); return rc; }    \
    } while (0)
    std::vector<uint64_t> soff(2 * ((size_t)d->M + 1), 0);
    uint64_t tot = 0;
    for (int sid = 1; sid <= d->M; sid++)
        for (int dir = 0; dir < 2; dir++) {
            soff[2 * sid + dir] = tot;
            tot += ((uint64_t)d->totLen[sid] + 7) / 8 * 8;
        }
    std::vector<uint8_t> strands;
    std::thread strand_builder([&]() {
        strands.assign(tot + 16, 0);
        const int nt = d->M > 2000 ? 16 : 1;
        std::vector<std::thread> th;
        for (int t = 0; t < nt; t++)
            th.emplace_back([&, t]() {
                for (int sid = 1 + t; sid <= d->M; sid += nt) {
                    const uint8_t* f = d->ref_seq + d->ref_off[sid];
                    const int tl = d->totLen[sid];
                    uint8_t* o0 = strands.data() + soff[2 * sid];
                    uint8_t* o1 = strands.data() + soff[2 * sid + 1];
                    memcpy(o0, f, (size_t)tl);
                    for (int p = 0; p < tl; p++) {
                        const uint8_t b = f[tl - p - 1];
                        o1[p] = b == 4 ? 4 : 3 - b;
                    }
                }
            });
        for (auto& x : th) x.join();
    });
    struct StrandJoin { std::thread& t; ~StrandJoin() { if (t.joinable()) t.join(); } } strand_join{strand_builder};
    UP(sid_signed, d->sid_signed, d->nnz);
    UP(pos, d->pos, d->nnz);
    if (pe) UP(insertL, d->insertL, d->nnz);
    for (int m = 0; m < (pe ? 2 : 1); m++) {
        const uint64_t b_lo = d->read_off[m][0], nbytes = d->read_off[m][d->N1] - b_lo;
        uint64_t *d_off = nullptr, *d_nw = nullptr, *d_off8 = nullptr, *d_ws = nullptr, *d_wq = nullptr;
        int32_t* d_len = nullptr;
        uint8_t *d_raw = nullptr, *d_raw_q = nullptr;
        void* d_tmp = nullptr;
        auto drop = [&]() { hipFree(d_off); hipFree(d_nw); hipFree(d_raw); hipFree(d_raw_q); hipFree(d_tmp); };
        auto bail = [&](int code) { drop(); hipFree(d_off8); hipFree(d_len); hipFree(d_ws); hipFree(d_wq); rsem_model_destroy(c); return code; };
        if ((rc = upload(&d_off, d->read_off[m], (size_t)d->N1 + 1, st)) != RSEM_OK) return bail(rc);
        if (dmalloc(&d_nw, (size_t)d->N1 + 1) != hipSuccess || dmalloc(&d_off8, (size_t)d->N1 + 1) != hipSuccess ||
            dmalloc(&d_len, (size_t)d->N1) != hipSuccess || dmalloc(&d_raw, (size_t)nbytes) != hipSuccess)
            return bail(RSEM_ERR_NOMEM);
        hipLaunchKernelGGL(k_read_words, dim3(rsem::ceil_div(d->N1 + 1, kBlk)), dim3(kBlk), 0, st, d->N1, d_off, d_nw, d_len);
        size_t tb = 0;
        if (hipcub::DeviceScan::ExclusiveSum(nullptr, tb, d_nw, d_off8, d->N1 + 1, st) != hipSuccess || hipMalloc(&d_tmp, tb ? tb : 1) != hipSuccess ||
            hipcub::DeviceScan::ExclusiveSum(d_tmp, tb, d_nw, d_off8, d->N1 + 1, st) != hipSuccess)
            return bail(RSEM_ERR_HIP);
        uint64_t nw = 0;
        if (hipMemcpyAsync(&nw, d_off8 + d->N1, sizeof(uint64_t), hipMemcpyDeviceToHost, st) != hipSuccess || hipStreamSynchronize(st) != hipSuccess)
            return bail(RSEM_ERR_HIP);
        nw += 1;
        for (int what = 0; what < (q ? 2 : 1); what++) {
            uint64_t*& d_w = what ? d_wq : d_ws;
            if (dmalloc(&d_w, (size_t)nw) != hipSuccess) return bail(RSEM_ERR_NOMEM);
            if (hipMemsetAsync(d_w + (nw - 1), 0, sizeof(uint64_t), st) != hipSuccess) return bail(RSEM_ERR_HIP);
        }
        if ((rc = rsem::staged_h2d(d_raw, d->read_seq[m] + b_lo, (size_t)nbytes, st)) != RSEM_OK) return bail(rc);
        if (q) {
            if (dmalloc(&d_raw_q, (size_t)nbytes) != hipSuccess) return bail(RSEM_ERR_NOMEM);
            if ((rc = rsem::staged_h2d(d_raw_q, d->read_qual[m] + b_lo, (size_t)nbytes, st)) != RSEM_OK) return bail(rc);
        }
        if (d->N1) {
            if (!q) hipLaunchKernelGGL(k_pack_reads, dim3(rsem::ceil_div(d->N1, kBlk)), dim3(kBlk), 0, st, d->N1, d_off, d_off8, d_raw, d_ws);
            else hipLaunchKernelGGL(k_code_reads, dim3(rsem::ceil_div(d->N1 * 16, kBlk)), dim3(kBlk), 0, st, d->N1, d_off, d_off8, d_raw, d_raw_q, d_ws, d_wq);
        }
        if (hipGetLastError() != hipSuccess) return bail(RSEM_ERR_HIP);
        if (hipStreamSynchronize(st) != hipSuccess) return bail(RSEM_ERR_HIP);
        drop();
        c->owned.push_back(d_off8); D.roff8[m] = d_off8;
        c->owned.push_back(d_len); D.rlen[m] = d_len;
        c->owned.push_back(d_ws); D.rseq_w[m] = d_ws;
        if (q) { c->owned.push_back(d_wq); D.rqual_w[m] = d_wq; }
    }
    UP(lq, d->low_quality, d->N1);
    {
        strand_builder.join();
        UP(soff, soff.data(), soff.size());
        const uint64_t* wptr = nullptr;
        rc = up_field(c, wptr, reinterpret_cast<const uint64_t*>(strands.data()), (tot + 16) / 8, st);
// ... 163 lines not shown
```

### rsem_amd/csrc/model_block.hpp

```cpp
#pragma once
#include "simt_macros.hpp"

constexpr int kProfLds = 5120;
constexpr int kGldLds = 1024;
constexpr int kRspdLds = 128;
constexpr int kNoiseLds = 512;
constexpr unsigned kPadCode8 = 8u * 2500u;
constexpr int kQProbLds = 2528, kQNoiseProbLds = 512;
RSEM_DEVFN unsigned read_code8(unsigned quality, unsigned base) { return 8u * (25u * quality + base); }
RSEM_DEVFN unsigned noise_off8(unsigned code8) { return code8 - 160u * ((code8 * 1311u) >> 18); }

struct DevTables {
    double probF;
    int seedLen, estRSPD, B;
    const double *rspd_pdf, *rspd_cdf;
    int gld_lb, gld_ub;
    const double *gld_pdf, *gld_cdf;
    int has_mld, mld_lb, mld_ub;
    const double *mld_pdf, *mld_cdf;
    int prof_rows;
    const double* prof;
    const double* noise;
    const double* mw;
};

struct DevData {
    int model_type, M;
    uint64_t N1, nnz;
    const uint64_t* row_ptr;
    const uint32_t* hit_row;
    const int32_t* sid_signed;
    const int32_t* pos;
    const int32_t* insertL;
    const uint64_t* roff8[2];
    const int32_t* rlen[2];
    const uint64_t* rseq_w[2];
    const uint64_t* rqual_w[2];
    const uint8_t* lq;
    const uint64_t* soff;
    const uint64_t* refw;
    const int32_t* fullLen;
    const int32_t* totLen;
    const uint64_t* mask_off;
    const uint32_t* mask_words;
    const uint8_t* same_prev;
    const uint32_t* aw0;
    const uint32_t* aw1;
    const uint32_t* afull;
    const uint32_t* atot;
};

struct PlaneOut {
    const uint32_t* rank;
    const Shape* shapes;
    int n_shapes;
    uint32_t T, n_sell_rows;
    unsigned char* sval;
    double* sncp;
};
constexpr int kPlaneShapesMax = 96;

RSEM_DEVFN int plane_shape_of(const Shape* shapes, int n_shapes, uint32_t ps) {
    int lo = 0, hi = n_shapes;
    while (hi - lo > 1) {
        const int mid = (lo + hi) >> 1;
        if (shapes[mid].row_base <= ps) lo = mid; else hi = mid;
    }
    return lo;
}

struct AccumPtrs {
    double* prof;
    double* noise;
    double* rspd;
    double* gld;
    int gld0_lb, gld0_ub;
};

RSEM_DEVFN double ld_adj(const double* pdf, const double* cdf, int lb, int ub, int len, int refL) {
    if (len <= lb || len > ub || refL <= lb) return 0.0;
    return pdf[len - lb] / cdf[(ub < refL ? ub : refL) - lb];
}
RSEM_DEVFN double rspd_cdf_at(const DevTables& T, int fpos, int fullLen) {
    int i = (int)(((long long)fpos) * T.B / fullLen);
    double val = fpos * 1.0 / fullLen * T.B;
    return T.rspd_cdf[i] + (val - i) * T.rspd_pdf[i + 1];
}
RSEM_DEVFN double rspd_adj(const DevTables& T, int fpos, int effL, int fullLen) {
    if (!T.estRSPD) return 1.0 / effL;
    double denom = rspd_cdf_at(T, effL, fullLen);
    return denom >= kEpsilon ? (rspd_cdf_at(T, fpos + 1, fullLen) - rspd_cdf_at(T, fpos, fullLen)) / denom : 0.0;
}
RSEM_DEVFN uint64_t funnel8(uint64_t w0, uint64_t w1, int sh) { return sh ? (w0 >> sh) | (w1 << (64 - sh)) : w0; }
RSEM_DEVFN bool ref_mask(const DevData& D, int sid, int p) {
    return (D.mask_words[D.mask_off[sid] + (p >> 5)] >> (p & 31)) & 1u;
}
struct AlnFields { uint32_t a0, a1, full, tot; bool masked; };
template <bool kPE>
RSEM_DEVFN AlnFields alignment_fields(const DevData& D, int seedLen, uint64_t j) {
    AlnFields F;
    const int s = D.sid_signed[j];
    const int sid = s < 0 ? -s : s, dir = s < 0 ? 1 : 0;
    const int pos = D.pos[j], ins = kPE ? D.insertL[j] : 0;
    const int full = D.fullLen[sid], tot = D.totLen[sid];
    F.full = (uint32_t)full;
    F.tot = (uint32_t)tot;
    F.a0 = (uint32_t)(D.soff[2 * sid + dir] + (uint64_t)pos);
    F.a1 = kPE ? (uint32_t)(D.soff[2 * sid + (dir ^ 1)] + (uint64_t)(tot - pos - ins)) : 0u;
    const int p = kPE ? (dir == 0 ? pos : tot - pos - ins) : (dir == 0 ? pos : tot - pos - seedLen);
    F.masked = (p >= 0 && p < full) ? ref_mask(D, sid, p) : false;
    return F;
}
RSEM_DEVFN void add_tbl(double* lds, int cap, double* glob, int idx, double v) {
    if (idx < cap) RSEM_LDS_ADD(&lds[idx], v);
    else RSEM_ATOMIC_ADD(&glob[idx], v);
}
RSEM_DEVFN void rspd_update(double* lds, double* glob, int B, int fpos, int fullLen, double frac) {
    if (fpos >= fullLen) return;
    int i;
    double a = fpos * 1.0 / fullLen, b;
    for (i = (int)(((long long)fpos) * B / fullLen + 1); i < (int)((((long long)fpos + 1) * B - 1) / fullLen + 1); i++) {
        b = i * 1.0 / B;
        add_tbl(lds, kRspdLds, glob, i, (b - a) * fullLen * frac);
        a = b;
    }
    b = (fpos + 1.0) / fullLen;
    add_tbl(lds, kRspdLds, glob, i, (b - a) * fullLen * frac);
}

constexpr int kGrp = 16;

template <int kCtrl>
RSEM_DEVFN double mdl_dpp_take(double v) {
    const long long b = RSEM_DOUBLE_AS_LL(v);
    const int lo = RSEM_DPP_MOV((int)(unsigned)b, kCtrl);
    const int hi = RSEM_DPP_MOV((int)(unsigned)(b >> 32), kCtrl);
    return RSEM_LL_AS_DOUBLE(((long long)hi << 32) | (unsigned)lo);
}
RSEM_DEVFN double grp_sum(double v) {
    v += mdl_dpp_take<0xB1>(v);
    v += mdl_dpp_take<0x4E>(v);
    v += mdl_dpp_take<0x141>(v);
    v += mdl_dpp_take<0x140>(v);
    return v;
}
RSEM_DEVFN double grp_prod(double v) {
    v *= mdl_dpp_take<0xB1>(v);
    v *= mdl_dpp_take<0x4E>(v);
    v *= mdl_dpp_take<0x141>(v);
    v *= mdl_dpp_take<0x140>(v);
    return v;
}
RSEM_DEVFN int grp_ctz(unsigned m) {
    int i = 0;
    while (!((m >> i) & 1u)) ++i;
    return i;
}

struct MateWords {
    const uint64_t* seq;
    const uint64_t* qual;
    uint64_t r8;
    int len;
};

template <bool kQ>
RSEM_DEVFN double lane_profile_product(const double* prof, const MateWords& W, const uint64_t* __restrict__ refw, uint64_t a, int g, bool on) {
    double p = 1.0;
    if (!on) return p;
    const uint64_t* rw = refw + (a >> 3);
    const int sh = (int)(a & 7) * 8;
    for (int wi = g; wi * 8 < W.len; wi += kGrp) {
        const uint64_t rf = funnel8(rw[wi], rw[wi + 1], sh);
        const uint64_t sb = W.seq[W.r8 + wi];
        const uint64_t qb = kQ ? W.qual[W.r8 + wi] : 0;
        if (kQ) {
            double t[8];
#pragma unroll
            for (int u = 0; u < 8; u++) {
                const unsigned code = (unsigned)(((u < 4 ? sb : qb) >> (16 * (u & 3))) & 0xffffu);
                const unsigned r = (unsigned)((rf >> (8 * u)) & 0xffu);
                t[u] = *(const double*)((const char*)prof + (code + 40u * r));
            }
            RSEM_SCHED_FENCE();
#pragma unroll
            for (int u = 0; u < 8; u++) p *= t[u];
            continue;
        }
        const int n = W.len - wi * 8;
#pragma unroll
        for (int u = 0; u < 8; u++) {
            const int row = wi * 8 + u;
            const int idx = (row * 5 + (int)((rf >> (8 * u)) & 0xff)) * 5 + (int)((sb >> (8 * u)) & 0xff);
            const double t = prof[(u < n) ? idx : 0];
            p *= (u < n) ? t : 1.0;
        }
    }
    return p;
}

template <bool kQ>
RSEM_DEVFN void lane_profile_update(double* s_prof, double* g_prof, const MateWords& W, const uint64_t* __restrict__ refw, uint64_t a, int g,
                                    double frac) {
    const uint64_t* rw = refw + (a >> 3);
    const int sh = (int)(a & 7) * 8;
    for (int wi = g; wi * 8 < W.len; wi += kGrp) {
        const uint64_t rf = funnel8(rw[wi], rw[wi + 1], sh);
        const uint64_t sb = W.seq[W.r8 + wi];
        const uint64_t qb = kQ ? W.qual[W.r8 + wi] : 0;
        const int n = W.len - wi * 8 < 8 ? W.len - wi * 8 : 8;
        for (int u = 0; u < n; u++) {
            if (kQ) {
                const unsigned code = (unsigned)(((u < 4 ? sb : qb) >> (16 * (u & 3))) & 0xffffu);
// ... 7 lines not shown

template <bool kQ>
RSEM_DEVFN double lane_noise_product(const double* nprob, const MateWords& W, int g, bool on) {
    double p = 1.0;
    if (!on) return p;
    for (int wi = g; wi * 8 < W.len; wi += kGrp) {
        const uint64_t sb = W.seq[W.r8 + wi];
        const uint64_t qb = kQ ? W.qual[W.r8 + wi] : 0;
        if (kQ) {
            double t[8];
#pragma unroll
            for (int u = 0; u < 8; u++) {
                const unsigned code = (unsigned)(((u < 4 ? sb : qb) >> (16 * (u & 3))) & 0xffffu);
                t[u] = *(const double*)((const char*)nprob + noise_off8(code));
            }
            RSEM_SCHED_FENCE();
#pragma unroll
            for (int u = 0; u < 8; u++) p *= t[u];
            continue;
        }
        const int n = W.len - wi * 8;
#pragma unroll
        for (int u = 0; u < 8; u++) {
            const int b = (int)((sb >> (8 * u)) & 0xff);
            const double t = nprob[(u < n) ? b : 0];
            p *= (u < n) ? t : 1.0;
        }
    }
    return p;
}
template <bool kQ>
RSEM_DEVFN void lane_noise_update(double* s_noise, const MateWords& W, int g, double frac) {
    for (int wi = g; wi * 8 < W.len; wi += kGrp) {
        const uint64_t sb = W.seq[W.r8 + wi];
        const uint64_t qb = kQ ? W.qual[W.r8 + wi] : 0;
        const int n = W.len - wi * 8 < 8 ? W.len - wi * 8 : 8;
        for (int u = 0; u < n; u++) {
            if (kQ) {
                const unsigned code = (unsigned)(((u < 4 ? sb : qb) >> (16 * (u & 3))) & 0xffffu);
                RSEM_LDS_ADD((double*)((char*)s_noise + noise_off8(code)), frac);
            } else {
                RSEM_LDS_ADD(&s_noise[(int)((sb >> (8 * u)) & 0xff)], frac);
            }
        }
    }
}

struct ChunkRegs {
    bool has;
    int sid, dir, pos, insertL, fullLen, totLen;
    unsigned flags;
    uint64_t a[2];
    double cp;
};

template <bool kPE>
RSEM_DEVFN double alignment_prob(const DevData& D, const DevTables& T, const ChunkRegs& R, int len1, int len2, double pp1, double pp2) {
    double prob = 0.0;
    const int sid = R.sid, dir = R.dir, pos = R.pos, fullLen = R.fullLen, totLen = R.totLen;
    if (!kPE) {
        const int fpos = dir == 0 ? pos : totLen - pos - len1;
        const int seedPos = dir == 0 ? pos : totLen - pos - T.seedLen;
        if (!(seedPos >= fullLen || (R.flags & 4u))) {
            double value;
            if (T.has_mld) {
                const int minL = len1 > T.gld_lb + 1 ? len1 : T.gld_lb + 1, maxL = totLen - pos < T.gld_ub ? totLen - pos : T.gld_ub;
                value = 0.0;
                for (int fragLen = minL; fragLen <= maxL; fragLen++) {
                    const int pfpos = dir == 0 ? pos : totLen - pos - fragLen;
                    const int effL = fullLen < totLen - fragLen + 1 ? fullLen : totLen - fragLen + 1;
                    value += ld_adj(T.gld_pdf, T.gld_cdf, T.gld_lb, T.gld_ub, fragLen, totLen) * rspd_adj(T, pfpos, effL, fullLen) *
                             ld_adj(T.mld_pdf, T.mld_cdf, T.mld_lb, T.mld_ub, len1, fragLen);
                }
            } else {
                const int effL = fullLen < totLen - len1 + 1 ? fullLen : totLen - len1 + 1;
                value = ld_adj(T.gld_pdf, T.gld_cdf, T.gld_lb, T.gld_ub, len1, totLen) * rspd_adj(T, fpos, effL, fullLen);
            }
            const double ori = dir == 0 ? T.probF : 1.0 - T.probF;
            prob = ori * value * pp1;
            if (prob < kEpsilon) prob = 0.0;
            prob = (T.mw[sid] < kEpsilon) ? 0.0 : prob / T.mw[sid];
        }
    } else {
        const int insertLen = R.insertL;
        const int fpos = dir == 0 ? pos : totLen - pos - insertLen;
        const int effL = fullLen < totLen - insertLen + 1 ? fullLen : totLen - insertLen + 1;
        if (!(fpos >= fullLen || (R.flags & 4u))) {
            const double ori = dir == 0 ? T.probF : 1.0 - T.probF;
            prob = ori * ld_adj(T.gld_pdf, T.gld_cdf, T.gld_lb, T.gld_ub, insertLen, totLen) * rspd_adj(T, fpos, effL, fullLen);
            prob *= ld_adj(T.mld_pdf, T.mld_cdf, T.mld_lb, T.mld_ub, len1, insertLen) * pp1;
            prob *= ld_adj(T.mld_pdf, T.mld_cdf, T.mld_lb, T.mld_ub, len2, insertLen) * pp2;
            if (prob < kEpsilon) prob = 0.0;
            prob = (T.mw[sid] < kEpsilon) ? 0.0 : prob / T.mw[sid];
        }
    }
    return prob;
}

template <bool kQ, bool kPE, bool kUpdate>
RSEM_DEVFN void model_group_rows(const DevData& D, const DevTables& T, const double* __restrict__ theta, double* __restrict__ cp,
                                 double* __restrict__ ncp, const AccumPtrs& A, const double* prob, const double* nprob, double* s_prof,
                                 double* s_noise, double* s_rspd, double* s_gld, uint64_t row0, uint64_t row_stride, int lane,
                                 const PlaneOut& PO, uint64_t chunk_rows = 0, uint64_t chunk0 = 0, uint64_t chunk_stride = 1) {
    const int g = lane & (kGrp - 1);
    const int g0 = lane & ~(kGrp - 1);
    constexpr int kMates = kPE ? 2 : 1;
    struct RowHdr {
        uint8_t lq;
        uint64_t fr, to;
        uint64_t r8[2];
        int rl[2];
        uint32_t rank;
    };
    auto load_hdr = [&](uint64_t row) -> RowHdr {
        RowHdr H;
        const uint64_t rowc = row < D.N1 ? row : D.N1 - 1;
        H.lq = D.lq[rowc];
        H.fr = D.row_ptr[rowc];
        H.to = D.row_ptr[rowc + 1];
        H.r8[0] = H.r8[1] = 0;
        H.rl[0] = H.rl[1] = 0;
#pragma unroll
        for (int m = 0; m < (kPE ? 2 : 1); m++) { H.r8[m] = D.roff8[m][rowc]; H.rl[m] = D.rlen[m][rowc]; }
        H.rank = PO.rank ? PO.rank[rowc] : 0u;
        return H;
    };
    const uint64_t n_chunks = chunk_rows ? (D.N1 + chunk_rows - 1) / chunk_rows : 1;
    for (uint64_t ch = chunk_rows ? chunk0 : 0; ch < n_chunks; ch += chunk_stride)
    for (uint64_t rbase = ch * chunk_rows + row0, rend = chunk_rows ? (ch + 1) * chunk_rows : D.N1; rbase < rend && rbase < D.N1; rbase += row_stride) {
        const uint64_t row = rbase + (uint64_t)(lane >> 4);
        const bool valid = row < D.N1;
        const RowHdr H = load_hdr(row);
        const uint8_t lq_v = H.lq;
        const uint64_t fr_v = H.fr, to_v = H.to;
        uint64_t r8_v[2] = {H.r8[0], H.r8[1]};
        int rl_v[2] = {H.rl[0], H.rl[1]};
        const uint32_t rank_v = H.rank;
        const bool active = valid && !lq_v;
        const uint64_t fr = valid ? fr_v : 0, to = valid ? to_v : 0;
        const int L = (int)(to - fr);
        int maxL = L;
        { int o = RSEM_SHFL_XOR(maxL, 16); maxL = o > maxL ? o : maxL; o = RSEM_SHFL_XOR(maxL, 32); maxL = o > maxL ? o : maxL; }
        MateWords W[kMates];
#pragma unroll
        for (int m = 0; m < kMates; m++) {
            W[m].r8 = active ? r8_v[m] : 0;
            W[m].seq = D.rseq_w[m];
            W[m].qual = kQ ? D.rqual_w[m] : nullptr;
            W[m].len = active ? rl_v[m] : 0;
        }
        const int len1 = W[0].len, len2 = kPE ? W[kMates - 1].len : 0;
        double* plane = nullptr;
        double* nslot = nullptr;
        int p_lg = 0;
        uint32_t p_r = 0;
        if (PO.rank && valid) {
            const uint32_t ps = rank_v;
            if (ps < PO.n_sell_rows) {
                const Shape& S = PO.shapes[plane_shape_of(PO.shapes, PO.n_shapes, ps)];
                uint32_t slice_local;
                row_to_slot(S, PO.T, ps - S.row_base, slice_local, p_r);
                plane = (double*)(PO.sval + S.val_base) + (uint64_t)slice_local * S.K * 64;
                nslot = PO.sncp + (S.slot_base + slice_local * shape_R(S) + p_r);
                p_lg = S.lg;
                p_r = (p_r << p_lg);
            }
        }
        auto plane_put = [&](int c_idx, double v) {
            if (plane) plane[(uint64_t)(c_idx >> p_lg) * 64 + p_r + (uint32_t)(c_idx & ((1 << p_lg) - 1))] = v;
        };

        uint64_t carry_a[kMates];
        double carry_p[kMates];
#pragma unroll
        for (int m = 0; m < kMates; m++) { carry_a[m] = 0; carry_p[m] = 0.0; }

        auto load_chunk = [&](int c, ChunkRegs& R) {
            const int idx = c * kGrp + g;
            const bool in = valid && idx < L;
            R.has = active && idx < L;
            const uint64_t j = fr + (uint64_t)(in ? idx : 0);
            const int s_v = D.sid_signed[j], pos_v = D.pos[j], ins_v = kPE ? D.insertL[j] : 0;
            const unsigned fl_v = D.same_prev[j];
            const uint32_t a0_v = D.aw0[j], a1_v = kPE ? D.aw1[j] : 0u, full_v = D.afull[j], tot_v = D.atot[j];
            const int s = R.has ? s_v : 1;
            R.sid = s < 0 ? -s : s;
            R.dir = s < 0 ? 1 : 0;
            R.pos = R.has ? pos_v : 0;
            R.insertL = R.has ? ins_v : 0;
            R.flags = R.has ? fl_v : 0u;
            R.fullLen = R.has ? (int)full_v : 1;
            R.totLen = R.has ? (int)tot_v : 1;
            R.a[0] = R.has ? (uint64_t)a0_v : 0;
            if (kPE) R.a[kMates - 1] = R.has ? (uint64_t)a1_v : 0;
            R.cp = 0.0;
            if (in && !R.has) { cp[j] = 0.0; plane_put(idx, 0.0); }
        };
        auto runs_of = [&](const ChunkRegs& R, int m, int c, auto&& fn) {
            const unsigned bit = 1u << m;
            const bool cont0 = (g == 0) && c > 0 && R.has && (R.flags & bit);
            const bool head = R.has && (!(R.flags & bit) || g == 0);
            const unsigned long long hb = RSEM_BALLOT(head);
            unsigned hg = (unsigned)((hb >> g0) & 0xffffull);
            const uint64_t ea = cont0 ? carry_a[m] : R.a[m];
            const int c0 = RSEM_SHFL((int)cont0, g0);
            bool first = true;
            uint64_t last_a = carry_a[m];
            while (RSEM_BALLOT(hg != 0u) != 0ull) {
                const bool on = hg != 0u;
                const int h = on ? grp_ctz(hg) : 0;
                const unsigned rest = hg & (hg - 1u);
                const int nh = (on && rest) ? grp_ctz(rest) : kGrp;
                const uint64_t ah = RSEM_SHFL(ea, g0 + h);
                fn(on, ah, h, nh, on && first && c0 != 0);
                if (on) last_a = ah;
                first = false;
                hg = rest;
            }
            carry_a[m] = last_a;
        };

        double rowsum = 0.0;
        const int nchunks = (maxL + kGrp - 1) / kGrp;
        for (int c = 0; c < nchunks; c++) {
            ChunkRegs R;
            load_chunk(c, R);
            double pp[kMates];
#pragma unroll
            for (int m = 0; m < kMates; m++) {
                pp[m] = carry_p[m];
                double lastp = carry_p[m];
                runs_of(R, m, c, [&](bool on, uint64_t ah, int h, int nh, bool continues) {
                    double p;
                    if (RSEM_BALLOT(on && !continues) != 0ull) {
                        p = grp_prod(lane_profile_product<kQ>(prob, W[m], D.refw, ah, g, on && !continues));
                        if (continues) p = carry_p[m];
                    } else p = carry_p[m];
                    if (on && g >= h && g < nh) pp[m] = p;
                    if (on) lastp = p;
                });
                carry_p[m] = lastp;
            }
            if (R.has) {
                R.cp = alignment_prob<kPE>(D, T, R, len1, len2, pp[0], kPE ? pp[kMates - 1] : 1.0);
                cp[fr + (uint64_t)(c * kGrp + g)] = R.cp;
                plane_put(c * kGrp + g, R.cp);
            }
            if (kUpdate) {
                const double th_v = theta[R.sid];
                double f = R.has ? th_v * R.cp : 0.0;
                if (f < kEpsilon) f = 0.0;
                rowsum += grp_sum(f);
            }
        }
        double nval = 0.0;
        {
            const double* lpdf = (kPE || T.has_mld) ? T.mld_pdf : T.gld_pdf;
            const int llb = (kPE || T.has_mld) ? T.mld_lb : T.gld_lb;
            double p = grp_prod(lane_noise_product<kQ>(nprob, W[0], g, active));
            double pr = active ? lpdf[len1 - llb] * p : 0.0;
            if (kPE) {
                const double p2 = grp_prod(lane_noise_product<kQ>(nprob, W[kMates - 1], g, active));
                if (active) pr *= lpdf[len2 - llb] * p2;
            }
            if (pr < kEpsilon) pr = 0.0;
            nval = (T.mw[0] < kEpsilon) ? 0.0 : pr / T.mw[0];
            if (!active) nval = 0.0;
            if (valid && g == 0) {
                ncp[row] = nval;
                if (nslot) *nslot = nval;
            }
        }
        if (!kUpdate) continue;

        double f0 = theta[0] * nval;
        if (f0 < kEpsilon) f0 = 0.0;
        const double sum = rowsum + f0;
        const bool ok = active && sum >= kEpsilon;
        const double wn = ok ? f0 / sum : 0.0;
#pragma unroll
        for (int m = 0; m < kMates; m++) carry_a[m] = 0;
        for (int c = 0; c < nchunks; c++) {
            ChunkRegs R;
            load_chunk(c, R);
            const double cp_v = cp[fr + (uint64_t)((valid && c * kGrp + g < L) ? c * kGrp + g : 0)], th_v = theta[R.sid];
            R.cp = R.has ? cp_v : 0.0;
            double f = R.has ? th_v * R.cp : 0.0;
            if (f < kEpsilon) f = 0.0;
            double w = ok ? f / sum : 0.0;
            if (w < kEpsilon) w = 0.0;
            if (w > 0.0) {
                if (!kPE) {
                    if (T.estRSPD) {
                        if (T.probF >= 0.1 && R.dir == 0) rspd_update(s_rspd, A.rspd, T.B, R.pos, R.fullLen, w);
                        if (T.probF < 0.1 && R.dir == 1) rspd_update(s_rspd, A.rspd, T.B, R.totLen - R.pos - len1, R.fullLen, w);
                    }
                } else {
                    add_tbl(s_gld, kGldLds, A.gld, R.insertL - A.gld0_lb, w);
                    if (T.estRSPD) {
                        const int fpos = R.dir == 0 ? R.pos : R.totLen - R.pos - R.insertL;
                        rspd_update(s_rspd, A.rspd, T.B, fpos, R.fullLen, w);
                    }
                }
            }
#pragma unroll
            for (int m = 0; m < kMates; m++)
                runs_of(R, m, c, [&](bool on, uint64_t ah, int h, int nh, bool) {
                    const double gw = grp_sum((on && g >= h && g < nh) ? w : 0.0);
                    if (on && gw > 0.0) lane_profile_update<kQ>(s_prof, A.prof, W[m], D.refw, ah, g, gw);
                });
        }
        if (wn >= kEpsilon) {
#pragma unroll
            for (int m = 0; m < kMates; m++) lane_noise_update<kQ>(s_noise, W[m], g, wn);
        }
    }
}
```

### rsem_amd/csrc/sell_layout.hpp

```cpp
#pragma once
#include <hipcub/hipcub.hpp>

#include <algorithm>
#include <vector>

#include "common.hpp"

namespace {

#include "sell_shape.hpp"

constexpr int kShapesPerFmt = 28;
constexpr int kShapeBits = 7;
constexpr int kMaxShapes = 3 * kShapesPerFmt;
constexpr int kShapeIds = 1 << kShapeBits;
constexpr int kLongShape = kShapeIds - 1;
constexpr uint32_t kKeyMinSidCap = (1u << (31 - kShapeBits)) - 1;
constexpr int kKeyApartBit = 63 - kShapeBits;
constexpr int kMaxK = 4;
constexpr int kBlock = 256;

struct Q32Scale { int e; };
__host__ __device__ inline bool q32_scale_of(double mx, double mn_nonzero, int range_bits, Q32Scale& q) {
    if (!(mx > 0.0) || !(mx < 1e300)) return false;
    int ex;
    (void)frexp(mx, &ex);
    q.e = ex - 32;
    if (q.e < -1000 || q.e > 900) return false;
    return mn_nonzero >= ldexp(mx, -range_bits);
}
__host__ __device__ inline uint32_t q32_mantissa(double v, int e) {
    const double m = rint(ldexp(v, -e));
    return m >= 4294967295.0 ? 0xffffffffu : (uint32_t)m;
}

__host__ __device__ inline int shape_id_of(uint64_t L) {
    if (L <= 4) return (int)(L == 0 ? 0 : L - 1);
    int lg = 1;
    uint64_t cap = 8;
    while (L > cap) { cap <<= 1; ++lg; }
    if (lg > 6) return kLongShape;
    int K = (int)((L + (1u << lg) - 1) >> lg);
    return lg * 4 + (K - 1);
}

__host__ __device__ inline bool slot_to_row(const Shape& S, uint32_t T, uint32_t slice_local, uint32_t r, uint32_t& q) {
    const uint32_t R = shape_R(S), rpb = R * T;
    const uint32_t b = slice_local / T, t = slice_local % T;
    if ((uint64_t)b * rpb >= S.n_rows) return false;
    const uint32_t left = S.n_rows - b * rpb;
    const uint32_t nb = left < rpb ? left : rpb;
    const uint32_t Tb = (nb + R - 1) / R;
    if (t >= Tb || r * Tb + t >= nb) return false;
    q = b * rpb + r * Tb + t;
    return true;
}

__host__ __device__ inline uint32_t mix32(uint32_t h, uint32_t v) {
    h ^= v + 0x9e3779b9u + (h << 6) + (h >> 2);
    return h;
}


constexpr int kLayoutWindow = 2048;
constexpr int kAnchorReach = kLayoutWindow / 2;
constexpr int kMedianExactMax = 64;
__host__ __device__ inline uint64_t row_key_of(uint64_t i, int32_t M, const uint64_t* __restrict__ row_ptr,
                                               const int32_t* __restrict__ sid, const double* __restrict__ cp, int range_bits,
                                               int apart, int* err, int split = 0, uint32_t* split_far = nullptr) {
    uint64_t fr = row_ptr[i], to = row_ptr[i + 1];
    if (to < fr) { *err = 1; return 0; }
    uint32_t h = 0x811c9dc5u, mn = 0xffffffffu;
    double vmx = 0.0, vmn = 1.79e308;
    for (uint64_t j = fr; j < to; j++) {
        int32_t s = sid[j];
        if (s < 1 || s > M) { *err = 2; s = 1; }
        h = mix32(h, (uint32_t)s);
        mn = (uint32_t)s < mn ? (uint32_t)s : mn;
        if (cp) {
            const double v = cp[j];
            if (!(v >= 0.0)) vmx = 1e308;
            vmx = fmax(vmx, v);
            if (v > 0.0) vmn = fmin(vmn, v);
        }
    }
    const uint64_t L = to - fr;
    if (L > 1 && !*err) {
        uint32_t med = (uint32_t)sid[fr + L / 2];
        if (L <= (uint64_t)kMedianExactMax) {
            for (uint64_t j = fr; j < to; j++) {
                const uint32_t v = (uint32_t)sid[j];
                uint32_t less = 0, leq = 0;
                for (uint64_t k = fr; k < to; k++) {
                    const uint32_t u = (uint32_t)sid[k];
                    less += u < v ? 1u : 0u;
                    leq += u <= v ? 1u : 0u;
                }
                if (less <= L / 2 && L / 2 < leq) { med = v; break; }
            }
        }
        const uint32_t floor_sid = med > (uint32_t)kAnchorReach ? med - (uint32_t)kAnchorReach : 0u;
        uint32_t lo = med;
        for (uint64_t j = fr; j < to; j++) {
            const uint32_t v = (uint32_t)sid[j];
            if (v >= floor_sid && v < lo) lo = v;
        }
        mn = lo;
    }
    uint64_t far = 0, L_in = 0;
    uint32_t h_in = 0x811c9dc5u;
    if (apart && L > 1 && !*err)
        for (uint64_t j = fr; j < to; j++) {
            const uint32_t v = (uint32_t)sid[j];
            if (v < mn || v >= mn + (uint32_t)apart) far = 1;
            else { ++L_in; h_in = mix32(h_in, v); }
        }
    int shape = shape_id_of(to - fr);
    if (far && split && (split == 2 || 2 * L_in <= L) && shape != kLongShape && (uint64_t)mn <= kKeyMinSidCap) {
        shape = shape_id_of(L_in) + 2 * kShapesPerFmt;
        if (split_far) *split_far = (uint32_t)(L - L_in);
        return ((uint64_t)shape << (64 - kShapeBits)) | ((uint64_t)mn << 32) | h_in;
    }
    if (mn > kKeyMinSidCap) mn = kKeyMinSidCap;
    Q32Scale q;
    if (cp && shape != kLongShape && q32_scale_of(vmx, vmn, range_bits, q)) shape += kShapesPerFmt;
    return ((uint64_t)shape << (64 - kShapeBits)) | (far << kKeyApartBit) | ((uint64_t)mn << 32) | h;
}

__global__ void k_row_keys(uint64_t N1, int32_t M, const uint64_t* __restrict__ row_ptr,
                           const int32_t* __restrict__ sid, const double* __restrict__ cp, int range_bits, int apart, int split,
                           const unsigned char* __restrict__ also_apart, uint64_t* keys, uint32_t* vals, int* err,
                           unsigned long long* n_split = nullptr ) {
    uint64_t i = (uint64_t)blockIdx.x * blockDim.x + threadIdx.x;
    if (i >= N1) return;
    int e = 0;
    uint32_t nf = 0;
    uint64_t key = row_key_of(i, M, row_ptr, sid, cp, range_bits, apart, &e, split, &nf);
    if (n_split && nf) { atomicAdd(&n_split[0], 1ull); atomicAdd(&n_split[1], (unsigned long long)nf); }
    if (also_apart && also_apart[i] && (int)(key >> (64 - kShapeBits)) < 2 * kShapesPerFmt) key |= 1ull << kKeyApartBit;
    if (e) *err = e;
    if (e == 1) return;
    keys[i] = key;
    vals[i] = (uint32_t)i;
}

__global__ void k_shape_bounds(uint64_t N1, const uint64_t* __restrict__ keys, uint32_t* first) {
    uint64_t p = (uint64_t)blockIdx.x * blockDim.x + threadIdx.x;
    if (p >= N1) return;
    int sh = (int)(keys[p] >> (64 - kShapeBits));
    if (p == 0 || sh != (int)(keys[p - 1] >> (64 - kShapeBits))) first[sh] = (uint32_t)p;
}

__device__ inline int find_shape_by_row(const Shape* shapes, int n, uint32_t p) {
    int sh = 0;
    while (sh + 1 < n && p >= shapes[sh + 1].row_base) ++sh;
    return sh;
}

__host__ __device__ inline bool in_split_window(int32_t id, uint32_t anchor, int reach) { return (uint32_t)id - anchor < (uint32_t)reach; }

template <bool kIds>
__host__ __device__ inline void sell_fill_row(const Shape& S, uint32_t T, uint32_t p, const uint32_t* __restrict__ order,
                                              const uint64_t* __restrict__ row_ptr, const int32_t* __restrict__ sid,
                                              const double* __restrict__ cp, const double* __restrict__ ncp, int32_t* ssid,
                                              unsigned char* sval, double* sncp, int16_t* sexp, int* err, uint32_t anchor = 0,
                                              int reach = kLayoutWindow) {
    const int G = shape_G(S);
    uint32_t slice_local, r;
    row_to_slot(S, T, p - S.row_base, slice_local, r);
    uint32_t orig = order[p];
    uint64_t fr = row_ptr[orig];
    int L = (int)(row_ptr[orig + 1] - fr);
    const uint64_t pl_local = (uint64_t)slice_local * S.K * 64;
    const uint64_t pl0 = S.plane_base * 64 + pl_local;
    const uint32_t slot = S.slot_base + slice_local * shape_R(S) + r;
    Q32Scale q{0};
    if (cp && S.fmt == kFmtQ32) {
        double vmx = 0.0;
        for (int c = 0; c < L; c++) vmx = fmax(vmx, cp[fr + c]);
        if (!q32_scale_of(vmx, vmx, 0, q)) { if (err) *err = 3; q.e = 0; }
        if (sexp) sexp[slot] = (int16_t)q.e;
    }
    int ci = 0;
    for (int c = 0; c < L; c++) {
        if (S.fmt == kFmtF64X && !in_split_window(sid[fr + c], anchor, reach)) continue;
        const uint64_t off = (uint64_t)(ci >> S.lg) * 64 + r * G + (ci & (G - 1));
        ++ci;
        if (kIds) ssid[pl0 + off] = sid[fr + c];
        if (cp) {
            if (S.fmt == kFmtQ32) ((uint32_t*)(sval + S.val_base))[pl_local + off] = q32_mantissa(cp[fr + c], q.e);
            else ((double*)(sval + S.val_base))[pl_local + off] = cp[fr + c];
        }
    }
    if (ncp) sncp[slot] = ncp[orig];
}

__global__ void k_unfill_sell(const Shape* __restrict__ shapes, int n_shapes, uint32_t T, uint32_t n_sell_rows,
                              const uint32_t* __restrict__ order, const uint64_t* __restrict__ row_ptr, const int32_t* __restrict__ ssid,
                              const unsigned char* __restrict__ sval, int32_t* sid, double* cp) {
    const uint32_t p = blockIdx.x * blockDim.x + threadIdx.x;
    if (p >= n_sell_rows) return;
    const Shape S = shapes[find_shape_by_row(shapes, n_shapes, p)];
    const int G = shape_G(S);
    uint32_t slice_local, r;
    row_to_slot(S, T, p - S.row_base, slice_local, r);
    const uint32_t orig = order[p];
    const uint64_t fr = row_ptr[orig];
    const int L = (int)(row_ptr[orig + 1] - fr);
    const uint64_t pl_local = (uint64_t)slice_local * S.K * 64;
    const uint64_t pl0 = S.plane_base * 64 + pl_local;
    for (int c = 0; c < L; c++) {
        const uint64_t off = (uint64_t)(c >> S.lg) * 64 + r * G + (c & (G - 1));
        sid[fr + c] = ssid[pl0 + off];
        cp[fr + c] = ((const double*)(sval + S.val_base))[pl_local + off];
    }
}

template <bool kIds>
__global__ void k_fill_sell(const Shape* __restrict__ shapes, int n_shapes, uint32_t T, uint32_t n_sell_rows,
                            const uint32_t* __restrict__ order, const uint64_t* __restrict__ row_ptr,
                            const int32_t* __restrict__ sid, const double* __restrict__ cp,
                            const double* __restrict__ ncp, int32_t* ssid, unsigned char* sval, double* sncp,
                            int16_t* sexp, int* err, const uint32_t* __restrict__ xanchor, uint32_t x_row_base, int reach,
                            const uint32_t* __restrict__ xreach = nullptr ) {
    uint32_t p = blockIdx.x * blockDim.x + threadIdx.x;
    if (p >= n_sell_rows) return;
    const Shape S = shapes[find_shape_by_row(shapes, n_shapes, p)];
    const bool x = S.fmt == kFmtF64X;
    sell_fill_row<kIds>(S, T, p, order, row_ptr, sid, cp, ncp, ssid, sval, sncp, sexp, err, x ? xanchor[p - x_row_base] : 0u,
                        (x && xreach) ? (int)xreach[p - x_row_base] : reach);
}

__host__ __device__ inline bool slice_lane_changed(const Shape& S, uint32_t T, uint32_t sl, int lane, const int32_t* __restrict__ ssid) {
    if (sl % T == 0) return true;
    const uint64_t pl0 = (S.plane_base + (uint64_t)sl * S.K) * 64;
    bool changed = false;
    for (int k = 0; k < S.K; k++) {
        int v = ssid[pl0 + (uint64_t)k * 64 + lane];
        int pv = ssid[pl0 - (uint64_t)S.K * 64 + (uint64_t)k * 64 + lane];
        changed = changed || (pv != v);
    }
    return changed;
}
__host__ __device__ inline unsigned long long read_lanes_of(const Shape& S, int lane) {
    const int G = shape_G(S);
    const int gb = lane & ~(G - 1);
    return (G == 64) ? ~0ull : (((1ull << G) - 1) << gb);
}

__global__ void k_slice_masks(const Shape* __restrict__ shapes, int n_shapes, uint32_t T, uint32_t n_slices,
                              const int32_t* __restrict__ ssid, unsigned long long* masks) {
    __shared__ Shape sh_shapes[kMaxShapes];
    for (int i = threadIdx.x; i < n_shapes; i += blockDim.x) sh_shapes[i] = shapes[i];
    __syncthreads();
    int lane = threadIdx.x & 63;
    uint32_t s = blockIdx.x * (blockDim.x / 64) + (threadIdx.x >> 6);
    if (s >= n_slices) return;
    int sh = 0;
    while (sh + 1 < n_shapes && s >= sh_shapes[sh + 1].slice_base) ++sh;
    const Shape S = sh_shapes[sh];
    const bool changed = slice_lane_changed(S, T, s - S.slice_base, lane, ssid);
    unsigned long long m = __ballot(changed);
    m = __ballot((m & read_lanes_of(S, lane)) != 0);
    if (lane == 0) masks[s] = m;
}

__global__ void k_count_sid_planes(const Shape* __restrict__ shapes, int n_shapes, uint32_t n_slices,
                                   const unsigned long long* __restrict__ masks, unsigned long long* out) {
    const uint32_t s = blockIdx.x * blockDim.x + threadIdx.x;
    unsigned long long k = 0;
    if (s < n_slices && masks[s] != 0ull) {
        int sh = 0;
        while (sh + 1 < n_shapes && s >= shapes[sh + 1].slice_base) ++sh;
        k = (unsigned long long)shapes[sh].K;
    }
    for (int d = 32; d >= 1; d >>= 1) k += __shfl_xor(k, d);
    if ((threadIdx.x & 63) == 0 && k) atomicAdd(out, k);
}

__global__ void k_slice_minsid(const Shape* __restrict__ shapes, int n_shapes, uint32_t T, uint32_t n_slices,
                               const uint64_t* __restrict__ keys_sorted, uint32_t* slice_minsid) {
    uint32_t s = blockIdx.x * blockDim.x + threadIdx.x;
    if (s >= n_slices) return;
    int sh = 0;
    while (sh + 1 < n_shapes && s >= shapes[sh + 1].slice_base) ++sh;
    const Shape S = shapes[sh];
    const uint32_t sl = s - S.slice_base, R = shape_R(S);
    uint32_t q = (sl / T) * R * T + sl % T;
    slice_minsid[s] = (uint32_t)((keys_sorted[S.row_base + q] >> 32) & kKeyMinSidCap);
}

__global__ void k_slice_maxanchor(const Shape* __restrict__ shapes, int n_shapes, uint32_t T, uint32_t n_slices,
                                  const uint64_t* __restrict__ keys_sorted, uint32_t* slice_maxanchor) {
    uint32_t s = blockIdx.x * blockDim.x + threadIdx.x;
    if (s >= n_slices) return;
    int sh = 0;
    while (sh + 1 < n_shapes && s >= shapes[sh + 1].slice_base) ++sh;
    const Shape S = shapes[sh];
    const uint32_t sl = s - S.slice_base;
    uint32_t q = 0, best = 0;
    bool any = false;
    for (int r = (int)shape_R(S) - 1; r >= 0 && !any; r--)
        if (slot_to_row(S, T, sl, (uint32_t)r, q)) { best = q; any = true; }
    slice_maxanchor[s] = any ? (uint32_t)((keys_sorted[S.row_base + best] >> 32) & kKeyMinSidCap) : 0u;
}

__global__ void k_slice_maxsid(const Shape* __restrict__ shapes, int n_shapes, uint32_t n_slices,
                               const int32_t* __restrict__ ssid, const uint32_t* __restrict__ slice_minsid, int window_cap,
                               uint32_t* slice_maxsid) {
    __shared__ Shape sh_shapes[kMaxShapes];
    for (int i = threadIdx.x; i < n_shapes; i += blockDim.x) sh_shapes[i] = shapes[i];
    __syncthreads();
    int lane = threadIdx.x & 63;
    uint32_t s = blockIdx.x * (blockDim.x / 64) + (threadIdx.x >> 6);
    if (s >= n_slices) return;
    int sh = 0;
    while (sh + 1 < n_shapes && s >= sh_shapes[sh + 1].slice_base) ++sh;
    const Shape S = sh_shapes[sh];
    uint64_t pl0 = (S.plane_base + (uint64_t)(s - S.slice_base) * S.K) * 64;
    int mx = 0;
    const long long lim = (long long)slice_minsid[s] + window_cap;
    for (int k = 0; k < S.K; k++) {
        const int v = ssid[pl0 + (uint64_t)k * 64 + lane];
        if ((long long)v < lim) mx = max(mx, v);
    }
    for (int d = 32; d >= 1; d >>= 1) mx = max(mx, __shfl_xor(mx, d));
    if (lane == 0) slice_maxsid[s] = (uint32_t)mx;
}

template <typename T>
hipError_t dmalloc(T** p, size_t n) { return hipMalloc((void**)p, std::max<size_t>(n, 1) * sizeof(T)); }

__global__ void k_x_anchors(uint32_t n_x, uint32_t x_row_base, const uint64_t* __restrict__ keys_sorted, uint32_t* xanchor) {
    const uint32_t x = blockIdx.x * blockDim.x + threadIdx.x;
    if (x < n_x) xanchor[x] = (uint32_t)((keys_sorted[x_row_base + x] >> 32) & kKeyMinSidCap);
}
__global__ void k_x_far(const Shape* __restrict__ shapes, int n_shapes, uint32_t T, uint32_t n_x, uint32_t x_row_base, uint32_t x_slot_base,
                        const uint32_t* __restrict__ order, const uint64_t* __restrict__ row_ptr, const int32_t* __restrict__ sid,
                        const uint32_t* __restrict__ xanchor, uint64_t* nfar, const uint64_t* __restrict__ far_ptr, int32_t* far_sid, uint64_t* far_src,
                        uint32_t* far_eslot, int reach, const uint32_t* __restrict__ xreach = nullptr) {
    const uint32_t x = blockIdx.x * blockDim.x + threadIdx.x;
    if (x >= n_x) return;
    if (xreach) reach = (int)xreach[x];
    const uint32_t p = x_row_base + x, orig = order[p], anchor = xanchor[x];
    const uint64_t fr = row_ptr[orig], to = row_ptr[orig + 1];
    const Shape S = shapes[find_shape_by_row(shapes, n_shapes, p)];
    uint32_t slice_local, r;
    row_to_slot(S, T, p - S.row_base, slice_local, r);
    const uint32_t slot = S.slot_base + slice_local * shape_R(S) + r, xs = slot - x_slot_base;
    if (!far_ptr) {
        uint64_t n = 0;
        for (uint64_t j = fr; j < to; j++) n += in_split_window(sid[j], anchor, reach) ? 0 : 1;
        nfar[xs] = n;
        return;
    }
    uint64_t e = far_ptr[xs];
    for (uint64_t j = fr; j < to; j++)
        if (!in_split_window(sid[j], anchor, reach)) { far_sid[e] = sid[j]; far_src[e] = j; far_eslot[e] = slot; ++e; }
}
constexpr int kCscSlotBlockLg = 16;
__global__ void k_x_csc_keys(uint64_t n_far, uint32_t x_slot_base, const int32_t* __restrict__ far_sid, const uint32_t* __restrict__ far_eslot,
                             uint64_t* keys, uint64_t* vals, int block_lg) {
    const uint64_t e = (uint64_t)blockIdx.x * blockDim.x + threadIdx.x;
    if (e >= n_far) return;
    keys[e] = ((uint64_t)((far_eslot[e] - x_slot_base) >> block_lg) << 32) | (uint32_t)far_sid[e];
    vals[e] = e;
}
__global__ void k_x_csc(uint64_t n_far, const uint64_t* __restrict__ perm, const int32_t* __restrict__ far_sid, const uint64_t* __restrict__ far_src,
                        const uint32_t* __restrict__ far_eslot, int32_t* csc_sid, uint64_t* csc_src, uint32_t* csc_slot) {
    const uint64_t i = (uint64_t)blockIdx.x * blockDim.x + threadIdx.x;
    if (i >= n_far) return;
    const uint64_t e = perm[i];
    csc_sid[i] = far_sid[e];
    csc_src[i] = far_src[e];
    csc_slot[i] = far_eslot[e];
}
__global__ void k_x_values(uint64_t n_far, const double* __restrict__ cp, const uint64_t* __restrict__ far_src, const uint64_t* __restrict__ csc_src,
                           double* far_cp, double* csc_cp) {
    const uint64_t i = (uint64_t)blockIdx.x * blockDim.x + threadIdx.x;
    if (i >= n_far) return;
    far_cp[i] = cp[far_src[i]];
    csc_cp[i] = cp[csc_src[i]];
}

struct SellLayout {
    uint64_t N1 = 0;
    uint32_t T = 16;
    uint32_t* d_order = nullptr;
    uint32_t n_sell_rows = 0;
    uint32_t n_long_rows = 0;
    Shape h_shapes[kMaxShapes];
    int n_shapes = 0;
    Shape* d_shapes = nullptr;
    uint32_t n_slices = 0;
    uint32_t n_slots = 0;
    uint64_t n_planes = 0;
    uint64_t val_bytes = 0;
    uint32_t n_q32_rows = 0;
    uint64_t n_q32_planes = 0;
    uint64_t n_sid_planes_loaded = 0;
    uint32_t x_row_base = 0, n_x_rows = 0;
    uint32_t x_slot_base = 0;
    uint64_t n_far = 0;
    uint32_t* d_xanchor = nullptr;
    uint32_t* d_xreach = nullptr;
    uint32_t n_x_slots = 0;
    uint64_t* d_far_ptr = nullptr;
    int32_t* d_far_sid = nullptr;
    uint64_t* d_far_src = nullptr;
    double* d_far_cp = nullptr;
    int32_t* d_csc_sid = nullptr;
    uint64_t* d_csc_src = nullptr;
    uint32_t* d_csc_slot = nullptr;
    double* d_csc_cp = nullptr;
    int32_t* d_ssid = nullptr;
    unsigned long long* d_masks = nullptr;
    uint32_t* d_slice_minsid = nullptr;
    uint32_t* d_slice_maxsid = nullptr;
    uint32_t* d_slice_maxanchor = nullptr;
};

inline void sell_free(SellLayout& L) {
    hipFree(L.d_order); hipFree(L.d_shapes); hipFree(L.d_ssid); hipFree(L.d_masks); hipFree(L.d_slice_minsid); hipFree(L.d_slice_maxsid); hipFree(L.d_slice_maxanchor);
    hipFree(L.d_xanchor); hipFree(L.d_xreach); hipFree(L.d_far_ptr); hipFree(L.d_far_sid); hipFree(L.d_far_src); hipFree(L.d_far_cp);
    hipFree(L.d_csc_sid); hipFree(L.d_csc_src); hipFree(L.d_csc_slot); hipFree(L.d_csc_cp);
    L = SellLayout();
}

inline int sell_fill_values(const SellLayout& L, hipStream_t st, const uint64_t* d_row_ptr, const double* d_cp,
                            const double* d_ncp, void* d_sval, double* d_sncp, int16_t* d_sexp = nullptr,
                            int* d_err = nullptr, const int32_t* d_sid = nullptr) {
    RSEM_HIP_TRY(hipMemsetAsync(d_sval, 0, L.val_bytes, st));
    RSEM_HIP_TRY(hipMemsetAsync(d_sncp, 0, sizeof(double) * L.n_slots, st));
    if (d_sexp) RSEM_HIP_TRY(hipMemsetAsync(d_sexp, 0, sizeof(int16_t) * L.n_slots, st));
    if (L.n_x_rows && !d_sid) { rsem::set_last_error("a layout with split rows needs the transcript ids to place their values"); return RSEM_ERR_STATE; }
    if (L.n_sell_rows) {
        hipLaunchKernelGGL(k_fill_sell<false>, dim3(rsem::ceil_div(L.n_sell_rows, kBlock)), dim3(kBlock), 0, st,
                           L.d_shapes, L.n_shapes, L.T, L.n_sell_rows, L.d_order, d_row_ptr, d_sid,
                           d_cp, d_ncp, (int32_t*)nullptr, (unsigned char*)d_sval, d_sncp, d_sexp, d_err, (const uint32_t*)L.d_xanchor, L.x_row_base, kLayoutWindow,
                           (const uint32_t*)L.d_xreach);
        RSEM_HIP_TRY(hipGetLastError());
    }
    if (L.n_far) {
        hipLaunchKernelGGL(k_x_values, dim3(rsem::ceil_div(L.n_far, kBlock)), dim3(kBlock), 0, st, L.n_far, d_cp, (const uint64_t*)L.d_far_src,
                           (const uint64_t*)L.d_csc_src, L.d_far_cp, L.d_csc_cp);
        RSEM_HIP_TRY(hipGetLastError());
    }
    return RSEM_OK;
}

inline int sell_build_far(SellLayout& L, hipStream_t st, const uint64_t* d_row_ptr, const int32_t* d_sid, const uint64_t* d_keys_sorted) {
    const uint32_t nx = L.n_x_rows;
    if (!nx) return RSEM_OK;
    const uint32_t nxs = L.n_slots - L.x_slot_base;
    L.n_x_slots = nxs;
    if (d_keys_sorted) {
        RSEM_HIP_TRY(dmalloc(&L.d_xanchor, nx));
        hipLaunchKernelGGL(k_x_anchors, dim3(rsem::ceil_div(nx, kBlock)), dim3(kBlock), 0, st, nx, L.x_row_base, d_keys_sorted, L.d_xanchor);
    } else {
        hipFree(L.d_far_ptr); hipFree(L.d_far_sid); hipFree(L.d_far_src); hipFree(L.d_far_cp);
        hipFree(L.d_csc_sid); hipFree(L.d_csc_src); hipFree(L.d_csc_slot); hipFree(L.d_csc_cp);
        L.d_far_ptr = nullptr; L.d_far_sid = nullptr; L.d_far_src = nullptr; L.d_far_cp = nullptr;
        L.d_csc_sid = nullptr; L.d_csc_src = nullptr; L.d_csc_slot = nullptr; L.d_csc_cp = nullptr;
        L.n_far = 0;
    }
    RSEM_HIP_TRY(dmalloc(&L.d_far_ptr, (size_t)nxs + 1));
    uint64_t* d_n = nullptr;
    void* d_tmp = nullptr;
    uint64_t *d_perm_in = nullptr, *d_perm = nullptr, *d_k_in = nullptr, *d_k_out = nullptr;
    uint32_t* d_eslot = nullptr;
    auto cleanup = [&]() { hipFree(d_n); hipFree(d_tmp); hipFree(d_perm_in); hipFree(d_perm); hipFree(d_k_in); hipFree(d_k_out); hipFree(d_eslot); };
    hipError_t e = dmalloc(&d_n, (size_t)nxs + 1);
    if (e == hipSuccess) e = hipMemsetAsync(d_n, 0, sizeof(uint64_t) * ((size_t)nxs + 1), st);
    if (e != hipSuccess) { cleanup(); RSEM_HIP_TRY(e); }
    hipLaunchKernelGGL(k_x_far, dim3(rsem::ceil_div(nx, kBlock)), dim3(kBlock), 0, st, (const Shape*)L.d_shapes, L.n_shapes, L.T, nx, L.x_row_base, L.x_slot_base,
                       (const uint32_t*)L.d_order, d_row_ptr, d_sid, (const uint32_t*)L.d_xanchor, d_n, (const uint64_t*)nullptr, (int32_t*)nullptr,
                       (uint64_t*)nullptr, (uint32_t*)nullptr, kLayoutWindow, (const uint32_t*)L.d_xreach);
    size_t tb = 0;
    e = hipcub::DeviceScan::ExclusiveSum(nullptr, tb, d_n, L.d_far_ptr, (size_t)nxs + 1, st);
    if (e == hipSuccess) e = hipMalloc(&d_tmp, tb ? tb : 1);
    if (e == hipSuccess) e = hipcub::DeviceScan::ExclusiveSum(d_tmp, tb, d_n, L.d_far_ptr, (size_t)nxs + 1, st);
    uint64_t nf = 0;
    if (e == hipSuccess) e = hipMemcpyAsync(&nf, L.d_far_ptr + nxs, sizeof(uint64_t), hipMemcpyDeviceToHost, st);
    if (e == hipSuccess) e = hipStreamSynchronize(st);
    if (e != hipSuccess) { cleanup(); RSEM_HIP_TRY(e); }
    L.n_far = nf;
    e = dmalloc(&L.d_far_sid, nf);
    if (e == hipSuccess) e = dmalloc(&L.d_far_src, nf);
    if (e == hipSuccess) e = dmalloc(&L.d_far_cp, nf);
    if (e == hipSuccess) e = dmalloc(&L.d_csc_sid, nf);
    if (e == hipSuccess) e = dmalloc(&L.d_csc_src, nf);
    if (e == hipSuccess) e = dmalloc(&L.d_csc_slot, nf);
    if (e == hipSuccess) e = dmalloc(&L.d_csc_cp, nf);
    if (e == hipSuccess) e = dmalloc(&d_eslot, nf);
    if (e == hipSuccess) e = hipMemsetAsync(L.d_far_cp, 0, sizeof(double) * std::max<uint64_t>(nf, 1), st);
    if (e == hipSuccess) e = hipMemsetAsync(L.d_csc_cp, 0, sizeof(double) * std::max<uint64_t>(nf, 1), st);
    if (e != hipSuccess) { cleanup(); RSEM_HIP_TRY(e); }
    hipLaunchKernelGGL(k_x_far, dim3(rsem::ceil_div(nx, kBlock)), dim3(kBlock), 0, st, (const Shape*)L.d_shapes, L.n_shapes, L.T, nx, L.x_row_base, L.x_slot_base,
                       (const uint32_t*)L.d_order, d_row_ptr, d_sid, (const uint32_t*)L.d_xanchor, (uint64_t*)nullptr, (const uint64_t*)L.d_far_ptr,
                       L.d_far_sid, L.d_far_src, d_eslot, kLayoutWindow, (const uint32_t*)L.d_xreach);
    if (nf) {
        hipFree(d_tmp); d_tmp = nullptr;
        e = dmalloc(&d_perm_in, nf);
        if (e == hipSuccess) e = dmalloc(&d_perm, nf);
        if (e == hipSuccess) e = dmalloc(&d_k_in, nf);
        if (e == hipSuccess) e = dmalloc(&d_k_out, nf);
        if (e != hipSuccess) { cleanup(); RSEM_HIP_TRY(e); }
        int block_lg = kCscSlotBlockLg;
        if (const char* eb = getenv("RSEM_HIP_CSC_BLOCK_LG")) block_lg = std::min(31, std::max(8, atoi(eb)));
        hipLaunchKernelGGL(k_x_csc_keys, dim3(rsem::ceil_div(nf, kBlock)), dim3(kBlock), 0, st, nf, L.x_slot_base, (const int32_t*)L.d_far_sid,
                           (const uint32_t*)d_eslot, d_k_in, d_perm_in, block_lg);
        tb = 0;
        e = hipcub::DeviceRadixSort::SortPairs(nullptr, tb, (const uint64_t*)d_k_in, d_k_out, (const uint64_t*)d_perm_in, d_perm, nf, 0, 64, st);
        if (e == hipSuccess) e = hipMalloc(&d_tmp, tb ? tb : 1);
        if (e == hipSuccess) e = hipcub::DeviceRadixSort::SortPairs(d_tmp, tb, (const uint64_t*)d_k_in, d_k_out, (const uint64_t*)d_perm_in, d_perm, nf, 0, 64, st);
        if (e != hipSuccess) { cleanup(); RSEM_HIP_TRY(e); }
        hipLaunchKernelGGL(k_x_csc, dim3(rsem::ceil_div(nf, kBlock)), dim3(kBlock), 0, st, nf, (const uint64_t*)d_perm, (const int32_t*)L.d_far_sid,
                           (const uint64_t*)L.d_far_src, (const uint32_t*)d_eslot, L.d_csc_sid, L.d_csc_src, L.d_csc_slot);
    }
    e = hipGetLastError();
    if (e == hipSuccess) e = hipStreamSynchronize(st);
    cleanup();
    RSEM_HIP_TRY(e);
    return RSEM_OK;
}

inline int sell_build(SellLayout& L, hipStream_t st, uint64_t N1, int32_t M, const uint64_t* d_row_ptr,
                      const int32_t* d_sid, uint32_t target_waves, uint32_t forced_T = 0,
                      const double* d_cp_for_q32 = nullptr, int range_bits = 0, const unsigned char* d_also_apart = nullptr, int split = 0) {
    L.N1 = N1;
    int apart = kLayoutWindow;
    if (const char* e = getenv("RSEM_HIP_APART")) apart = atoi(e) ? kLayoutWindow : 0;
    uint64_t *d_keys = nullptr, *d_keys2 = nullptr;
    uint32_t *d_vals = nullptr, *d_first = nullptr;
    int* d_err = nullptr;
    void* d_tmp = nullptr;
    unsigned long long* d_ns = nullptr;
    auto cleanup = [&]() {
        hipFree(d_keys); hipFree(d_keys2); hipFree(d_vals); hipFree(d_first); hipFree(d_err); hipFree(d_tmp); hipFree(d_ns);
    };
    RSEM_HIP_TRY(dmalloc(&d_keys, N1));
    RSEM_HIP_TRY(dmalloc(&d_keys2, N1));
    RSEM_HIP_TRY(dmalloc(&d_vals, N1));
    RSEM_HIP_TRY(dmalloc(&L.d_order, N1));
    RSEM_HIP_TRY(dmalloc(&d_first, kShapeIds));
    RSEM_HIP_TRY(dmalloc(&d_err, 1));
    RSEM_HIP_TRY(hipMemsetAsync(d_err, 0, sizeof(int), st));
    RSEM_HIP_TRY(hipMemsetAsync(d_first, 0xff, kShapeIds * sizeof(uint32_t), st));
    if (N1) {
        int do_split = apart ? split : 0;
        if (do_split) {
            unsigned long long h_ns[2] = {0, 0};
            RSEM_HIP_TRY(dmalloc(&d_ns, 2));
            RSEM_HIP_TRY(hipMemsetAsync(d_ns, 0, 2 * sizeof(unsigned long long), st));
            hipLaunchKernelGGL(k_row_keys, dim3(rsem::ceil_div(N1, kBlock)), dim3(kBlock), 0, st, N1, M, d_row_ptr, d_sid,
                               d_cp_for_q32, range_bits, apart, do_split, d_also_apart, d_keys, d_vals, d_err, d_ns);
            RSEM_HIP_TRY(hipGetLastError());
            RSEM_HIP_TRY(hipMemcpyAsync(h_ns, d_ns, sizeof(h_ns), hipMemcpyDeviceToHost, st));
            RSEM_HIP_TRY(hipStreamSynchronize(st));
            if (h_ns[0] * 20ull < N1 && !getenv("RSEM_HIP_SPLIT_ALWAYS")) do_split = 0;
        }
        if (!do_split) {
            hipLaunchKernelGGL(k_row_keys, dim3(rsem::ceil_div(N1, kBlock)), dim3(kBlock), 0, st, N1, M, d_row_ptr, d_sid,
                               d_cp_for_q32, range_bits, apart, 0, d_also_apart, d_keys, d_vals, d_err, (unsigned long long*)nullptr);
            RSEM_HIP_TRY(hipGetLastError());
        }
        size_t tb = 0;
        RSEM_HIP_TRY(hipcub::DeviceRadixSort::SortPairs(nullptr, tb, d_keys, d_keys2, d_vals, L.d_order, N1, 0, 64, st));
        RSEM_HIP_TRY(hipMalloc(&d_tmp, tb ? tb : 1));
        RSEM_HIP_TRY(hipcub::DeviceRadixSort::SortPairs(d_tmp, tb, d_keys, d_keys2, d_vals, L.d_order, N1, 0, 64, st));
        hipLaunchKernelGGL(k_shape_bounds, dim3(rsem::ceil_div(N1, kBlock)), dim3(kBlock), 0, st, N1, d_keys2, d_first);
        RSEM_HIP_TRY(hipGetLastError());
    }
    uint32_t h_first[kShapeIds];
    int h_err = 0;
    RSEM_HIP_TRY(hipMemcpyAsync(h_first, d_first, sizeof(h_first), hipMemcpyDeviceToHost, st));
    RSEM_HIP_TRY(hipMemcpyAsync(&h_err, d_err, sizeof(int), hipMemcpyDeviceToHost, st));
    RSEM_HIP_TRY(hipStreamSynchronize(st));
    if (h_err) {
        cleanup();
        rsem::set_last_error(h_err == 1 ? "row_ptr is not monotone" : "sid outside 1..M");
        return RSEM_ERR_INVALID;
    }
    L.n_shapes = 0;
    L.n_slices = 0;
    L.n_planes = 0;
    L.n_slots = 0;
    L.val_bytes = 0;
    L.n_q32_rows = 0;
    L.n_q32_planes = 0;
    L.n_x_rows = 0;
    L.x_row_base = 0;
    L.x_slot_base = 0;
    L.n_far = 0;
    L.n_x_slots = 0;
    uint32_t long_first = (h_first[kLongShape] == 0xffffffffu) ? (uint32_t)N1 : h_first[kLongShape];
    L.n_sell_rows = long_first;
    L.n_long_rows = (uint32_t)N1 - long_first;
    for (int id = 0; id < kMaxShapes; id++) {
        if (h_first[id] == 0xffffffffu) continue;
        uint32_t next = long_first;
        for (int j = id + 1; j < kMaxShapes; j++)
            if (h_first[j] != 0xffffffffu) { next = h_first[j]; break; }
        Shape& S = L.h_shapes[L.n_shapes++];
        S.fmt = id / kShapesPerFmt;
        S.lg = (id % kShapesPerFmt) / 4;
        S.K = id % 4 + 1;
        S.row_base = h_first[id];
        S.n_rows = next - h_first[id];
        uint32_t rps = shape_R(S);
        S.n_slices = (S.n_rows + rps - 1) / rps;
        S.slice_base = L.n_slices;
        S.plane_base = L.n_planes;
        S.slot_base = L.n_slots;
        S.val_base = L.val_bytes;
        L.n_slices += S.n_slices;
        L.n_planes += (uint64_t)S.n_slices * S.K;
        L.n_slots += S.n_slices * rps;
        L.val_bytes += (uint64_t)S.n_slices * S.K * plane_bytes(S.fmt);
        if (S.fmt == kFmtQ32) { L.n_q32_rows += S.n_rows; L.n_q32_planes += (uint64_t)S.n_slices * S.K; }
        if (S.fmt == kFmtF64X) {
            if (!L.n_x_rows) { L.x_row_base = S.row_base; L.x_slot_base = S.slot_base; }
            L.n_x_rows += S.n_rows;
        }
    }
    uint32_t T = forced_T ? forced_T : L.n_slices / std::max(1u, target_waves);
    L.T = std::min<uint32_t>(256, std::max<uint32_t>(forced_T ? 1 : 8, T));
    RSEM_HIP_TRY(dmalloc(&L.d_shapes, kMaxShapes));
    RSEM_HIP_TRY(hipMemcpyAsync(L.d_shapes, L.h_shapes, sizeof(Shape) * kMaxShapes, hipMemcpyHostToDevice, st));
    RSEM_HIP_TRY(dmalloc(&L.d_ssid, L.n_planes * 64));
    RSEM_HIP_TRY(dmalloc(&L.d_masks, (size_t)L.n_slices));
    RSEM_HIP_TRY(dmalloc(&L.d_slice_minsid, (size_t)L.n_slices));
    RSEM_HIP_TRY(dmalloc(&L.d_slice_maxsid, (size_t)L.n_slices));
    RSEM_HIP_TRY(dmalloc(&L.d_slice_maxanchor, (size_t)L.n_slices));
    RSEM_HIP_TRY(hipMemsetAsync(L.d_ssid, 0, sizeof(int32_t) * L.n_planes * 64, st));
    if (L.n_x_rows) {
        const int frc = sell_build_far(L, st, d_row_ptr, d_sid, d_keys2);
        if (frc != RSEM_OK) { cleanup(); return frc; }
    }
    if (L.n_sell_rows) {
        hipLaunchKernelGGL(k_fill_sell<true>, dim3(rsem::ceil_div(L.n_sell_rows, kBlock)), dim3(kBlock), 0, st,
                           L.d_shapes, L.n_shapes, L.T, L.n_sell_rows, L.d_order, d_row_ptr, d_sid, (const double*)nullptr,
                           (const double*)nullptr, L.d_ssid, (unsigned char*)nullptr, (double*)nullptr, (int16_t*)nullptr,
                           (int*)nullptr, (const uint32_t*)L.d_xanchor, L.x_row_base, kLayoutWindow);
        RSEM_HIP_TRY(hipGetLastError());
        hipLaunchKernelGGL(k_slice_minsid, dim3(rsem::ceil_div(L.n_slices, kBlock)), dim3(kBlock), 0, st, L.d_shapes,
                           L.n_shapes, L.T, L.n_slices, d_keys2, L.d_slice_minsid);
        RSEM_HIP_TRY(hipGetLastError());
        hipLaunchKernelGGL(k_slice_maxanchor, dim3(rsem::ceil_div(L.n_slices, kBlock)), dim3(kBlock), 0, st, L.d_shapes,
                           L.n_shapes, L.T, L.n_slices, d_keys2, L.d_slice_maxanchor);
        RSEM_HIP_TRY(hipGetLastError());
        hipLaunchKernelGGL(k_slice_maxsid, dim3(rsem::ceil_div(L.n_slices, kBlock / 64)), dim3(kBlock), 0, st, L.d_shapes,
                           L.n_shapes, L.n_slices, L.d_ssid, L.d_slice_minsid, kLayoutWindow, L.d_slice_maxsid);
        RSEM_HIP_TRY(hipGetLastError());
        hipLaunchKernelGGL(k_slice_masks, dim3(rsem::ceil_div(L.n_slices, kBlock / 64)), dim3(kBlock), 0, st,
                           L.d_shapes, L.n_shapes, L.T, L.n_slices, L.d_ssid, L.d_masks);
        RSEM_HIP_TRY(hipGetLastError());
        unsigned long long* d_cnt = (unsigned long long*)d_keys;
        RSEM_HIP_TRY(hipMemsetAsync(d_cnt, 0, sizeof(unsigned long long), st));
        hipLaunchKernelGGL(k_count_sid_planes, dim3(rsem::ceil_div(L.n_slices, kBlock)), dim3(kBlock), 0, st, L.d_shapes, L.n_shapes,
                           L.n_slices, (const unsigned long long*)L.d_masks, d_cnt);
        RSEM_HIP_TRY(hipGetLastError());
        unsigned long long h_cnt = 0;
        RSEM_HIP_TRY(hipMemcpyAsync(&h_cnt, d_cnt, sizeof(h_cnt), hipMemcpyDeviceToHost, st));
        RSEM_HIP_TRY(hipStreamSynchronize(st));
        L.n_sid_planes_loaded = h_cnt;
    }
    RSEM_HIP_TRY(hipStreamSynchronize(st));
    cleanup();
    return RSEM_OK;
}

struct Unit {
    int32_t shape;
    uint32_t slice_begin;
    uint32_t n_slices;
    uint32_t per_wave;
    int32_t base;
    int32_t span;
    int32_t pad[2];
    Shape S;
};

inline int sell_build_units(const SellLayout& L, std::vector<Unit>& units, int window_cap) {
    std::vector<uint32_t> ms(L.n_slices), mx(L.n_slices), ma(L.n_slices);
    if (L.n_slices) {
        RSEM_HIP_TRY(hipMemcpy(ms.data(), L.d_slice_minsid, sizeof(uint32_t) * L.n_slices, hipMemcpyDeviceToHost));
        RSEM_HIP_TRY(hipMemcpy(mx.data(), L.d_slice_maxsid, sizeof(uint32_t) * L.n_slices, hipMemcpyDeviceToHost));
        RSEM_HIP_TRY(hipMemcpy(ma.data(), L.d_slice_maxanchor, sizeof(uint32_t) * L.n_slices, hipMemcpyDeviceToHost));
    }
    double f_full = 1.0, f_half = 0.0;
    if (const char* e = getenv("RSEM_HIP_TAPER")) {
        double a = 0, b = 0;
        if (sscanf(e, "%lf,%lf", &a, &b) == 2 && a >= 0 && b >= 0 && a + b <= 1.0) { f_full = a; f_half = b; }
    }
    constexpr uint32_t W = 4;
    units.clear();
    auto add = [&](int sh, const Shape& S, uint32_t sl0, uint32_t n, uint32_t per_wave) {
        Unit U;
        U.shape = sh;
        U.slice_begin = sl0;
        U.n_slices = n;
        U.per_wave = std::max<uint32_t>(per_wave, 1);
        const uint32_t s0 = S.slice_base + sl0, s1 = s0 + n;
        uint32_t top = 0, low = ms[s0];
        for (uint32_t t = s0; t < s1; t++) { top = std::max(top, mx[t]); low = std::min(low, ms[t]); }
        U.base = (int32_t)low;
        const long long span = (long long)top - U.base + 1;
        U.span = (int32_t)std::min<long long>(std::max<long long>(span, 1), window_cap);
        U.pad[0] = U.pad[1] = 0;
        U.S = S;
        units.push_back(U);
    };
    for (int sh = 0; sh < L.n_shapes; sh++) {
        const Shape& S = L.h_shapes[sh];
        const uint32_t T = L.T, nb = (S.n_slices + T - 1) / T;
        uint32_t b_full = (uint32_t)(nb * f_full) / W * W;
        uint32_t b_half = (uint32_t)(nb * f_half) / 2 * 2;
        if (T < 4) { b_full = nb / W * W; b_half = 0; }
        if (b_full + b_half > nb) b_half = (nb - b_full) / 2 * 2;
        uint32_t b = 0;
        auto emit = [&](uint32_t nblocks, uint32_t per_wave) {
            const uint32_t sl0 = b * T, n = std::min(S.n_slices, (b + nblocks) * T) - sl0;
            add(sh, S, sl0, n, per_wave);
            b += nblocks;
        };
        auto fits = [&](uint32_t nblocks) -> bool {
            const uint32_t s0 = S.slice_base + b * T, s1 = S.slice_base + std::min(S.n_slices, (b + nblocks) * T);
            uint32_t top = 0, low = 0xffffffffu;
            for (uint32_t t = s0; t < s1; t++) { top = std::max(top, std::max(mx[t], ma[t])); low = std::min(low, ms[t]); }
            return s1 <= s0 || (long long)top - (long long)low + 1 <= (long long)window_cap;
        };
        auto emit_fitting = [&](uint32_t want) {
            if (want >= W && fits(W)) emit(W, T);
            else if (want >= 2 && T >= 2 && fits(2)) emit(2, (T + 1) / 2);
            else if (T >= 4) emit(1, (T + 3) / 4);
            else emit(std::min<uint32_t>(want, nb - b), T);
        };
        while (b < b_full) emit_fitting(std::min<uint32_t>(W, b_full - b));
        while (b < b_full + b_half) emit_fitting(2);
        if (T < 4) while (b < nb) emit(std::min<uint32_t>(W, nb - b), T);
        else while (b < nb) emit(1, (T + 3) / 4);
    }
    std::stable_sort(units.begin(), units.end(), [&](const Unit& a, const Unit& b) {
        return (uint64_t)L.h_shapes[a.shape].K * a.n_slices > (uint64_t)L.h_shapes[b.shape].K * b.n_slices;
    });
    return RSEM_OK;
}

__host__ __device__ inline bool unit_entry_is_far(const Unit& U, int32_t v) { return v > 0 && (unsigned)(v - U.base) >= (unsigned)U.span; }

__global__ __launch_bounds__(256) void k_unit_far(Unit* units, const int32_t* __restrict__ ssid) {
    __shared__ int n_far;
    if (threadIdx.x == 0) n_far = 0;
    __syncthreads();
    const Unit U = units[blockIdx.x];
    const uint64_t p0 = (U.S.plane_base + (uint64_t)U.slice_begin * U.S.K) * 64, n = (uint64_t)U.n_slices * U.S.K * 64;
    int mine = 0;
    for (uint64_t i = threadIdx.x; i < n; i += blockDim.x) mine += unit_entry_is_far(U, ssid[p0 + i]) ? 1 : 0;
    if (mine) atomicAdd(&n_far, mine);
    __syncthreads();
    if (threadIdx.x == 0) {
        units[blockIdx.x].pad[0] = n_far != 0;
        units[blockIdx.x].pad[1] = n_far;
    }
}

inline int sell_flag_far_units(const SellLayout& L, std::vector<Unit>& units, Unit* d_units, hipStream_t st) {
    if (units.empty()) return RSEM_OK;
    hipLaunchKernelGGL(k_unit_far, dim3((unsigned)units.size()), dim3(256), 0, st, d_units, (const int32_t*)L.d_ssid);
    RSEM_HIP_TRY(hipGetLastError());
    RSEM_HIP_TRY(hipMemcpyAsync(units.data(), d_units, sizeof(Unit) * units.size(), hipMemcpyDeviceToHost, st));
    RSEM_HIP_TRY(hipStreamSynchronize(st));
    return RSEM_OK;
}

__global__ __launch_bounds__(256) void k_x_reach(const Unit* __restrict__ units, uint32_t T, const uint32_t* __restrict__ xanchor, uint32_t x_row_base, uint32_t* xreach) {
    const Unit U = units[blockIdx.x];
    const Shape& S = U.S;
    if (S.fmt != kFmtF64X) return;
    const uint32_t R = shape_R(S);
    for (uint32_t i = threadIdx.x; i < U.n_slices * R; i += blockDim.x) {
        uint32_t q;
        if (!slot_to_row(S, T, U.slice_begin + i / R, i % R, q)) continue;
        const uint32_t x = S.row_base + q - x_row_base;
        const long long top = (long long)U.base + U.span;
        const long long r = top - (long long)xanchor[x];
        xreach[x] = (uint32_t)(r < 1 ? kLayoutWindow : (r > kLayoutWindow ? kLayoutWindow : r));
    }
}

inline int sell_masks(SellLayout& L, hipStream_t st) {
    if (!L.n_slices) return RSEM_OK;
    hipLaunchKernelGGL(k_slice_masks, dim3(rsem::ceil_div(L.n_slices, kBlock / 64)), dim3(kBlock), 0, st, L.d_shapes, L.n_shapes, L.T, L.n_slices, L.d_ssid, L.d_masks);
    RSEM_HIP_TRY(hipGetLastError());
    unsigned long long* d_cnt = nullptr;
    RSEM_HIP_TRY(dmalloc(&d_cnt, 1));
    hipError_t e = hipMemsetAsync(d_cnt, 0, sizeof(unsigned long long), st);
    if (e == hipSuccess) {
        hipLaunchKernelGGL(k_count_sid_planes, dim3(rsem::ceil_div(L.n_slices, kBlock)), dim3(kBlock), 0, st, L.d_shapes, L.n_shapes, L.n_slices,
                           (const unsigned long long*)L.d_masks, d_cnt);
        e = hipGetLastError();
    }
    unsigned long long h_cnt = 0;
    if (e == hipSuccess) e = hipMemcpyAsync(&h_cnt, d_cnt, sizeof(h_cnt), hipMemcpyDeviceToHost, st);
    if (e == hipSuccess) e = hipStreamSynchronize(st);
    (void)hipFree(d_cnt);
    RSEM_HIP_TRY(e);
    L.n_sid_planes_loaded = h_cnt;
    return RSEM_OK;
}

inline int sell_refine_split_windows(SellLayout& L, hipStream_t st, const uint64_t* d_row_ptr, const int32_t* d_sid, std::vector<Unit>& units, Unit* d_units) {
    if (!L.n_x_rows || units.empty()) return RSEM_OK;
    size_t n_far_x = 0;
    for (const Unit& u : units) n_far_x += (u.S.fmt == kFmtF64X && u.pad[0] != 0) ? 1 : 0;
    if (!n_far_x) return RSEM_OK;
    RSEM_HIP_TRY(dmalloc(&L.d_xreach, L.n_x_rows));
    hipLaunchKernelGGL(k_x_reach, dim3((unsigned)units.size()), dim3(256), 0, st, (const Unit*)d_units, L.T, (const uint32_t*)L.d_xanchor, L.x_row_base, L.d_xreach);
    RSEM_HIP_TRY(hipGetLastError());
    RSEM_HIP_TRY(hipMemsetAsync(L.d_ssid, 0, sizeof(int32_t) * L.n_planes * 64, st));
    hipLaunchKernelGGL(k_fill_sell<true>, dim3(rsem::ceil_div(L.n_sell_rows, kBlock)), dim3(kBlock), 0, st, L.d_shapes, L.n_shapes, L.T, L.n_sell_rows, L.d_order,
                       d_row_ptr, d_sid, (const double*)nullptr, (const double*)nullptr, L.d_ssid, (unsigned char*)nullptr, (double*)nullptr, (int16_t*)nullptr,
                       (int*)nullptr, (const uint32_t*)L.d_xanchor, L.x_row_base, kLayoutWindow, (const uint32_t*)L.d_xreach);
    RSEM_HIP_TRY(hipGetLastError());
    int rc = sell_masks(L, st);
    if (rc == RSEM_OK) rc = sell_build_far(L, st, d_row_ptr, d_sid, nullptr);
    if (rc == RSEM_OK) rc = sell_flag_far_units(L, units, d_units, st);
    return rc;
}

__global__ __launch_bounds__(256) void k_mark_stray_reads(const Unit* __restrict__ units, const int32_t* __restrict__ ssid, const uint32_t* __restrict__ order,
                                                          uint32_t T, int32_t M, const uint64_t* __restrict__ row_ptr, const int32_t* __restrict__ sid,
                                                          unsigned char* also_apart, unsigned long long* n_marked) {
    const Unit U = units[blockIdx.x];
    if (U.pad[0] == 0) return;
    const Shape& S = U.S;
    const uint64_t p0 = (S.plane_base + (uint64_t)U.slice_begin * S.K) * 64, n = (uint64_t)U.n_slices * S.K * 64;
    unsigned long long mine = 0;
    for (uint64_t i = threadIdx.x; i < n; i += blockDim.x) {
        if (!unit_entry_is_far(U, ssid[p0 + i])) continue;
        const uint32_t sl = U.slice_begin + (uint32_t)(i / ((uint64_t)S.K * 64));
        const uint32_t r = (uint32_t)(i % 64) >> S.lg;
        uint32_t q;
        if (!slot_to_row(S, T, sl, r, q)) continue;
        const uint32_t orig = order[S.row_base + q];
        int e = 0;
        const uint64_t key = row_key_of(orig, M, row_ptr, sid, nullptr, 0, kLayoutWindow, &e);
        if (((key >> kKeyApartBit) & 1ull) == 0ull && also_apart[orig] == 0) {
            also_apart[orig] = 1;
            ++mine;
        }
    }
    if (mine) atomicAdd(n_marked, mine);
}

inline int sell_build_refined(SellLayout& L, hipStream_t st, uint64_t N1, int32_t M, const uint64_t* d_row_ptr, const int32_t* d_sid,
                              uint32_t target_waves, uint32_t forced_T, const double* d_cp_for_q32, int range_bits, int window_cap,
                              std::vector<Unit>& units, Unit** d_units, unsigned long long* n_strays = nullptr, int split = 0) {
    unsigned char* d_also = nullptr;
    unsigned long long* d_n = nullptr;
    if (n_strays) *n_strays = 0;
    const char* knob = getenv("RSEM_HIP_APART");
    const bool refine = !(knob && atoi(knob) == 0);
    for (int pass = 0; pass < 2; pass++) {
        int rc = sell_build(L, st, N1, M, d_row_ptr, d_sid, target_waves, forced_T, d_cp_for_q32, range_bits, d_also, split);
        if (rc == RSEM_OK) rc = sell_build_units(L, units, window_cap);
        if (rc != RSEM_OK) { (void)hipFree(d_also); return rc; }
        (void)hipFree(*d_units);
        *d_units = nullptr;
        hipError_t e = dmalloc(d_units, units.size());
        if (e == hipSuccess && !units.empty()) e = hipMemcpyAsync(*d_units, units.data(), sizeof(Unit) * units.size(), hipMemcpyHostToDevice, st);
        if (e != hipSuccess) { (void)hipFree(d_also); RSEM_HIP_TRY(e); }
        rc = sell_flag_far_units(L, units, *d_units, st);
        if (rc != RSEM_OK) { (void)hipFree(d_also); return rc; }
        size_t n_far_units = 0;
        for (const Unit& u : units) n_far_units += u.pad[0] != 0;
        if (pass == 1 || !n_far_units || N1 == 0 || !refine) break;
        unsigned long long n = 0;
        e = hipMalloc((void**)&d_also, N1);
        if (e == hipSuccess) e = hipMalloc((void**)&d_n, sizeof(unsigned long long));
        if (e == hipSuccess) e = hipMemsetAsync(d_also, 0, N1, st);
        if (e == hipSuccess) e = hipMemsetAsync(d_n, 0, sizeof(unsigned long long), st);
        if (e == hipSuccess) {
            hipLaunchKernelGGL(k_mark_stray_reads, dim3((unsigned)units.size()), dim3(256), 0, st, (const Unit*)*d_units, (const int32_t*)L.d_ssid,
                               (const uint32_t*)L.d_order, L.T, M, d_row_ptr, d_sid, d_also, d_n);
            e = hipGetLastError();
        }
        if (e == hipSuccess) e = hipMemcpyAsync(&n, d_n, sizeof(n), hipMemcpyDeviceToHost, st);
        if (e == hipSuccess) e = hipStreamSynchronize(st);
        (void)hipFree(d_n);
        if (e != hipSuccess) { (void)hipFree(d_also); RSEM_HIP_TRY(e); }
        if (n == 0) break;
        if (n * 1000ull < N1 && n_far_units * 100 < units.size()) break;
        if (n_strays) *n_strays = n;
        sell_free(L);
    }
    (void)hipFree(d_also);
    if (L.n_x_rows && !(getenv("RSEM_HIP_X_REFINE") && atoi(getenv("RSEM_HIP_X_REFINE")) == 0))
        return sell_refine_split_windows(L, st, d_row_ptr, d_sid, units, *d_units);
    return RSEM_OK;
}

}
```

### rsem_amd/csrc/sell_shape.hpp

```cpp
#pragma once

constexpr int kFmtF64 = 0, kFmtQ32 = 1, kFmtF64X = 2;

struct Shape {
    uint64_t plane_base;
    uint32_t slice_base;
    uint32_t n_slices;
    uint32_t row_base;
    uint32_t n_rows;
    uint32_t slot_base;
    int32_t K;
    int32_t lg;
    int32_t fmt;
    uint64_t val_base;
};

__host__ __device__ inline uint32_t plane_bytes(int fmt) { return fmt == kFmtQ32 ? 256u : 512u; }

__host__ __device__ inline int shape_G(const Shape& S) {
    return 1 << S.lg;
}
__host__ __device__ inline uint32_t shape_R(const Shape& S) {
    return 64u >> S.lg;
}

__host__ __device__ inline void row_to_slot(const Shape& S, uint32_t T, uint32_t q, uint32_t& slice_local, uint32_t& r) {
    const uint32_t R = shape_R(S), rpb = R * T;
    const uint32_t b = q / rpb, qb = q % rpb;
    const uint32_t left = S.n_rows - b * rpb;
    const uint32_t nb = left < rpb ? left : rpb;
    const uint32_t Tb = (nb + R - 1) / R;
    r = qb / Tb;
    slice_local = b * T + qb % Tb;
}
```

Before: 607.0 billion read-alignments/s.

## Add short last-plane shape classes to trim padded value storage in SELL layout

Adds shape classes whose final value plane holds only a quarter-granular fraction of each group's columns, picked per row length from a device histogram when enough rows fall in a class. The E step reads the compacted last plane with a per-lane remapped index and zeroes the lanes past the cut, and the model kernel writes values with the matching offset function. The aim is to stop streaming the padding entries of the last plane, cutting value-plane bytes in the memory-bound E step. In exchange the shape table grows (shape id bits go to 8, table to 148), layout build gains a histogram pass with a host sync, and rows split across more shapes, which could fragment slices and reduce coalescing on the last plane.

```diff
diff --git a/rsem_amd/csrc/em.hip b/rsem_amd/csrc/em.hip
--- a/rsem_amd/csrc/em.hip
+++ b/rsem_amd/csrc/em.hip
@@ -432,6 +432,8 @@
         S.lg = G.lg;
         S.fmt = G.fmt;
         S.val_base = G.val_base;
+        S.cut = G.cut;
+        S.reserved = 0;
         const uint32_t u_end = S.slice_base + U.slice_begin + U.n_slices;
         const uint32_t s_begin = S.slice_base + U.slice_begin + (uint32_t)w * U.per_wave;
         const uint32_t s_end = min(u_end, s_begin + U.per_wave);
@@ -822,6 +824,8 @@
     int* d_fill_err = nullptr;
     int value_bits = 64;
     int value_range_bits = 8;
+    int short_last_plane = 1;
+    int short_min_units = kShortClassMinUnits;
     bool layout_has_q32 = false;
     bool layout_ok = false;
     Unit* d_units = nullptr;
@@ -1078,14 +1082,18 @@
     const bool q32 = c->value_bits == 32 && c->have_values;
     std::vector<Unit> units;
     int split = c->split_rows && resolved_kernel(c) == RSEM_EM_KERNEL_LANE && !q32;
+    int short_on = c->short_last_plane, short_min_units = c->short_min_units;
+    if (const char* e = getenv("RSEM_HIP_SHORT_LAST_PLANE")) short_on = atoi(e) != 0;
+    if (const char* e = getenv("RSEM_HIP_SHORT_MIN_UNITS")) short_min_units = std::max(1, atoi(e));
     if (const char* e = getenv("RSEM_HIP_SPLIT")) split = split && atoi(e) != 0;
     if (split) split = c->split_policy;
     if (const char* e = getenv("RSEM_HIP_SPLIT_POLICY")) { if (split) split = !strcmp(e, "all") ? 2 : 1; }
     int rc = sell_build_refined(c->L, c->stream, c->N1, c->M, c->d_row_ptr, c->d_sid, target_waves, c->forced_T,
-                                q32 ? c->d_cp : nullptr, c->value_range_bits, kWindow, units, &c->d_units, &c->n_stray_reads, split);
+                                q32 ? c->d_cp : nullptr, c->value_range_bits, kWindow, units, &c->d_units, &c->n_stray_reads, split,
+                                short_on ? short_min_units : 0);
     if (rc != RSEM_OK) return rc;
     if (c->L.n_x_rows) {
-        const size_t nxs = (size_t)(c->L.n_slots - c->L.x_slot_base);
+        const size_t nxs = (size_t)c->L.n_x_slots;
         RSEM_HIP_TRY(dmalloc(&c->d_xextra, nxs));
         RSEM_HIP_TRY(dmalloc(&c->d_xinv, nxs));
         RSEM_HIP_TRY(hipMemsetAsync(c->d_xextra, 0, sizeof(double) * std::max<size_t>(nxs, 1), c->stream));
@@ -1355,6 +1363,22 @@
         set_grid_for_kernel(c);
         return RSEM_OK;
     }
+    if (!strcmp(key, "short_last_plane") || !strcmp(key, "short_class_min_units")) {
+        const bool sw = !strcmp(key, "short_last_plane");
+        if (sw) RSEM_REQUIRE(value == 0 || value == 1, "short_last_plane must be 0 or 1");
+        else RSEM_REQUIRE(value >= 1 && value <= 1000000, "short_class_min_units must be in 1..1000000");
+        int& field = sw ? c->short_last_plane : c->short_min_units;
+        if (field == (int)value) return RSEM_OK;
+        field = (int)value;
+        if (!sw && !c->short_last_plane) return RSEM_OK;
+        RSEM_HIP_TRY(hipSetDevice(c->device));
+        { int rc0 = ensure_csr(c); if (rc0 != RSEM_OK) return rc0; }
+        free_layout(c);
+        int rc = build_layout(c);
+        if (rc != RSEM_OK) return rc;
+        set_grid_for_kernel(c);
+        return RSEM_OK;
+    }
     if (!strcmp(key, "check_every")) {
         RSEM_REQUIRE(value >= 1 && value <= kHistCap / 4, "check_every out of range");
         c->check_every = (int)value;
@@ -1391,6 +1415,12 @@
     else if (!strcmp(key, "reads_sliced")) *value = c->L.n_sell_rows;
     else if (!strcmp(key, "reads_long")) *value = c->L.n_long_rows;
     else if (!strcmp(key, "value_plane_bytes")) *value = (int64_t)c->L.val_bytes;
+    else if (!strcmp(key, "value_plane_entries")) *value = (int64_t)c->L.n_val_entries;
+    else if (!strcmp(key, "short_last_plane")) *value = c->short_last_plane;
+    else if (!strcmp(key, "short_class_min_units")) *value = c->short_min_units;
+    else if (!strcmp(key, "short_classes")) *value = (int64_t)__builtin_popcountll(c->L.short_classes);
+    else if (!strcmp(key, "shapes")) *value = c->L.n_shapes;
+    else if (!strcmp(key, "unit_bytes")) *value = (int64_t)sizeof(Unit);
     else if (!strcmp(key, "sid_plane_bytes")) *value = (int64_t)(c->L.n_planes * 256);
     else if (!strcmp(key, "slots")) *value = c->L.n_slots;
     else if (!strcmp(key, "sid_plane_bytes_loaded")) *value = (int64_t)(c->L.n_sid_planes_loaded * 256);
diff --git a/rsem_amd/csrc/estep_block.hpp b/rsem_amd/csrc/estep_block.hpp
--- a/rsem_amd/csrc/estep_block.hpp
+++ b/rsem_amd/csrc/estep_block.hpp
@@ -116,17 +116,22 @@
         return ((unsigned long long)hi << 32) | lo;
     };
     const unsigned ulane = (unsigned)lane, uslot = ulane >> lg;
+    const unsigned Gk = (unsigned)shape_Gk(S);
+    const unsigned last_lane = uslot * Gk + ((unsigned)g < Gk ? (unsigned)g : Gk - 1u);
+    const bool last_ok = (unsigned)g < Gk;
+    const uint32_t vstride = (uint32_t)RSEM_READFIRSTLANE((int)shape_val_stride(S));
     auto issue = [&](uint32_t t, unsigned long long m, SliceRegs<K, kQ>& b) {
         const uint32_t sl = t - S.slice_base;
         const uint64_t v0 = (uint64_t)sl * (K * 64);
-        const ValT* __restrict__ vp = scp + v0;
+        const ValT* __restrict__ vp = scp + (uint64_t)sl * vstride;
         if (kFQ || m != 0ull) {
             const int32_t* __restrict__ ip = ssid + (S.plane_base * 64 + v0);
 #pragma unroll
             for (int k = 0; k < K; k++) b.id[k] = ip[k * 64 + ulane];
         }
 #pragma unroll
-        for (int k = 0; k < K; k++) b.c[k] = stream_load(&vp[k * 64 + ulane]);
+        for (int k = 0; k < K - 1; k++) b.c[k] = stream_load(&vp[k * 64 + ulane]);
+        b.c[K - 1] = stream_load(&vp[(K - 1) * 64 + last_lane]);
         const uint32_t slot0 = S.slot_base + sl * R;
         b.nc = (sncp + slot0)[uslot];
         b.e = kQ ? (int)(sexp + slot0)[uslot] : 0;
@@ -220,7 +225,8 @@
         const double scale = kQ ? pow2_of(cur.e) : 1.0;
 #pragma unroll
         for (int k = 0; k < K; k++) {
-            const double cv = kQ ? (double)cur.c[k] * scale : (double)cur.c[k];
+            const ValT cr = (k == K - 1 && !last_ok) ? ValT(0) : cur.c[k];
+            const double cv = kQ ? (double)cr * scale : (double)cr;
             double v = rth[k] * cv;
             if (v < kEpsilon) v = 0.0;
             f[k] = v;
diff --git a/rsem_amd/csrc/model.hip b/rsem_amd/csrc/model.hip
--- a/rsem_amd/csrc/model.hip
+++ b/rsem_amd/csrc/model.hip
@@ -251,6 +251,10 @@
     if (in_place) {
         const int vrc = rsem::em_planes_view(c->em, &pv);
         if (vrc != RSEM_OK) return vrc;
+    }
+    if (in_place && pv.n_shapes > kPlaneShapesMax) {
+        rsem::set_last_error("the EM layout has %d shapes, the model kernel's table holds %d", pv.n_shapes, kPlaneShapesMax);
+        return RSEM_ERR_STATE;
     }
     if (in_place) PO = PlaneOut{pv.d_rank, (const Shape*)pv.d_shapes, pv.n_shapes, pv.T, pv.n_sell_rows, pv.d_sval, pv.d_sncp};
     int rc;
diff --git a/rsem_amd/csrc/model_block.hpp b/rsem_amd/csrc/model_block.hpp
--- a/rsem_amd/csrc/model_block.hpp
+++ b/rsem_amd/csrc/model_block.hpp
@@ -58,7 +58,7 @@
     unsigned char* sval;
     double* sncp;
 };
-constexpr int kPlaneShapesMax = 96;
+constexpr int kPlaneShapesMax = kShapeTableMax;
 
 RSEM_DEVFN int plane_shape_of(const Shape* shapes, int n_shapes, uint32_t ps) {
     int lo = 0, hi = n_shapes;
@@ -372,7 +372,7 @@
         const int len1 = W[0].len, len2 = kPE ? W[kMates - 1].len : 0;
         double* plane = nullptr;
         double* nslot = nullptr;
-        int p_lg = 0;
+        int p_lg = 0, p_K = 1, p_cut = 0;
         uint32_t p_r = 0;
         if (PO.rank && valid) {
             const uint32_t ps = rank_v;
@@ -380,14 +380,15 @@
                 const Shape& S = PO.shapes[plane_shape_of(PO.shapes, PO.n_shapes, ps)];
                 uint32_t slice_local;
                 row_to_slot(S, PO.T, ps - S.row_base, slice_local, p_r);
-                plane = (double*)(PO.sval + S.val_base) + (uint64_t)slice_local * S.K * 64;
+                plane = (double*)(PO.sval + S.val_base) + (uint64_t)slice_local * shape_val_stride(S);
                 nslot = PO.sncp + (S.slot_base + slice_local * shape_R(S) + p_r);
                 p_lg = S.lg;
-                p_r = (p_r << p_lg);
+                p_K = S.K;
+                p_cut = S.cut;
             }
         }
         auto plane_put = [&](int c_idx, double v) {
-            if (plane) plane[(uint64_t)(c_idx >> p_lg) * 64 + p_r + (uint32_t)(c_idx & ((1 << p_lg) - 1))] = v;
+            if (plane) plane[shape_val_off(p_lg, p_K, p_cut, p_r, c_idx)] = v;
         };
 
         uint64_t carry_a[kMates];
diff --git a/rsem_amd/csrc/sell_layout.hpp b/rsem_amd/csrc/sell_layout.hpp
--- a/rsem_amd/csrc/sell_layout.hpp
+++ b/rsem_amd/csrc/sell_layout.hpp
@@ -11,8 +11,11 @@
 #include "sell_shape.hpp"
 
 constexpr int kShapesPerFmt = 28;
-constexpr int kShapeBits = 7;
-constexpr int kMaxShapes = 3 * kShapesPerFmt;
+constexpr int kShapeBits = 8;
+constexpr int kFullShapes = 3 * kShapesPerFmt;
+constexpr int kShortPerFmt = 32;
+constexpr int kMaxShapes = kFullShapes + 2 * kShortPerFmt;
+static_assert(kMaxShapes <= kShapeTableMax, "the kernels that keep the shape table in LDS size it by kShapeTableMax (sell_shape.hpp)");
 constexpr int kShapeIds = 1 << kShapeBits;
 constexpr int kLongShape = kShapeIds - 1;
 constexpr uint32_t kKeyMinSidCap = (1u << (31 - kShapeBits)) - 1;
@@ -29,19 +32,73 @@
     if (q.e < -1000 || q.e > 900) return false;
     return mn_nonzero >= ldexp(mx, -range_bits);
 }
+struct Q32Range {
+    double vmx = 0.0, vmn = 1.79e308;
+    __host__ __device__ void add(double v) {
+        if (!(v >= 0.0)) vmx = 1e308;
+        vmx = fmax(vmx, v);
+        if (v > 0.0) vmn = fmin(vmn, v);
+    }
+    __host__ __device__ bool takes_q32(int range_bits, Q32Scale& q) const { return q32_scale_of(vmx, vmn, range_bits, q); }
+};
+__host__ __device__ inline bool row_takes_q32(const double* __restrict__ cp, uint64_t fr, uint64_t to, int range_bits) {
+    Q32Range r;
+    for (uint64_t j = fr; j < to; j++) r.add(cp[j]);
+    Q32Scale q;
+    return r.takes_q32(range_bits, q);
+}
 __host__ __device__ inline uint32_t q32_mantissa(double v, int e) {
     const double m = rint(ldexp(v, -e));
     return m >= 4294967295.0 ? 0xffffffffu : (uint32_t)m;
 }
 
-__host__ __device__ inline int shape_id_of(uint64_t L) {
+__host__ __device__ inline int short_class_index(int lg, int K, int q) {
+    if (lg < 1 || lg > 6 || K < 3 || K > 4 || q < 1 || q > 3) return -1;
+    if (lg == 1) return q == 2 ? (K - 3) : -1;
+    return 2 + (lg - 2) * 6 + (K - 3) * 3 + (q - 1);
+}
+__host__ __device__ inline bool shape_of_id(int id, int& fmt, int& lg, int& K, int& cut) {
+    if (id < 0 || id >= kMaxShapes) return false;
+    if (id < kFullShapes) {
+        fmt = id / kShapesPerFmt;
+        lg = (id % kShapesPerFmt) / 4;
+        K = id % 4 + 1;
+        cut = 0;
+        return true;
+    }
+    const int j = id - kFullShapes, i = j % kShortPerFmt;
+    fmt = j / kShortPerFmt;
+    if (i < 2) { lg = 1; K = 3 + i; cut = 2; return true; }
+    lg = 2 + (i - 2) / 6;
+    K = 3 + ((i - 2) % 6) / 3;
+    cut = 3 - (i - 2) % 3;
+    return true;
+}
+__host__ __device__ inline int shape_fmt_of_id(int id) { return id < kFullShapes ? id / kShapesPerFmt : (id - kFullShapes) / kShortPerFmt; }
+__host__ __device__ inline int full_shape_of_id(int id) {
+    int fmt, lg, K, cut;
+    if (id < kFullShapes || !shape_of_id(id, fmt, lg, K, cut)) return id;
+    return fmt * kShapesPerFmt + lg * 4 + K - 1;
+}
+
+__host__ __device__ inline int shape_id_of(uint64_t L, uint32_t short_classes = 0, bool even_quarters = false) {
     if (L <= 4) return (int)(L == 0 ? 0 : L - 1);
     int lg = 1;
     uint64_t cap = 8;
     while (L > cap) { cap <<= 1; ++lg; }
     if (lg > 6) return kLongShape;
     int K = (int)((L + (1u << lg) - 1) >> lg);
+    if (short_classes) {
+        const int G = 1 << lg, n_last = (int)L - (K - 1) * G;
+        int q = (n_last * 4 + G - 1) >> lg;
+        if (even_quarters) q = (q + 1) & ~1;
+        const int i = short_class_index(lg, K, q);
+        if (i >= 0 && ((short_classes >> i) & 1u)) return kFullShapes + i;
+    }
     return lg * 4 + (K - 1);
+}
+__host__ __device__ inline int shape_id_in_fmt(int id, int fmt) {
+    return id < kFullShapes ? id + fmt * kShapesPerFmt : id + fmt * kShortPerFmt;
 }
 
 __host__ __device__ inline bool slot_to_row(const Shape& S, uint32_t T, uint32_t slice_local, uint32_t r, uint32_t& q) {
@@ -67,22 +124,18 @@
 constexpr int kMedianExactMax = 64;
 __host__ __device__ inline uint64_t row_key_of(uint64_t i, int32_t M, const uint64_t* __restrict__ row_ptr,
                                                const int32_t* __restrict__ sid, const double* __restrict__ cp, int range_bits,
-                                               int apart, int* err, int split = 0, uint32_t* split_far = nullptr) {
+                                               int apart, int* err, int split = 0, uint32_t* split_far = nullptr,
+                                               uint64_t short_classes = 0 ) {
     uint64_t fr = row_ptr[i], to = row_ptr[i + 1];
     if (to < fr) { *err = 1; return 0; }
     uint32_t h = 0x811c9dc5u, mn = 0xffffffffu;
-    double vmx = 0.0, vmn = 1.79e308;
+    Q32Range vr;
     for (uint64_t j = fr; j < to; j++) {
         int32_t s = sid[j];
         if (s < 1 || s > M) { *err = 2; s = 1; }
         h = mix32(h, (uint32_t)s);
         mn = (uint32_t)s < mn ? (uint32_t)s : mn;
-        if (cp) {
-            const double v = cp[j];
-            if (!(v >= 0.0)) vmx = 1e308;
-            vmx = fmax(vmx, v);
-            if (v > 0.0) vmn = fmin(vmn, v);
-        }
+        if (cp) vr.add(cp[j]);
     }
     const uint64_t L = to - fr;
     if (L > 1 && !*err) {
@@ -117,31 +170,79 @@
         }
     int shape = shape_id_of(to - fr);
     if (far && split && (split == 2 || 2 * L_in <= L) && shape != kLongShape && (uint64_t)mn <= kKeyMinSidCap) {
-        shape = shape_id_of(L_in) + 2 * kShapesPerFmt;
+        shape = shape_id_in_fmt(shape_id_of(L_in), kFmtF64X);
         if (split_far) *split_far = (uint32_t)(L - L_in);
         return ((uint64_t)shape << (64 - kShapeBits)) | ((uint64_t)mn << 32) | h_in;
     }
     if (mn > kKeyMinSidCap) mn = kKeyMinSidCap;
     Q32Scale q;
-    if (cp && shape != kLongShape && q32_scale_of(vmx, vmn, range_bits, q)) shape += kShapesPerFmt;
+    if (shape != kLongShape) {
+        const bool q32 = cp && vr.takes_q32(range_bits, q);
+        if (short_classes) shape = shape_id_of(to - fr, (uint32_t)(short_classes >> (q32 ? 32 : 0)), q32);
+        if (q32) shape = shape_id_in_fmt(shape, kFmtQ32);
+    }
     return ((uint64_t)shape << (64 - kShapeBits)) | (far << kKeyApartBit) | ((uint64_t)mn << 32) | h;
 }
 
 __global__ void k_row_keys(uint64_t N1, int32_t M, const uint64_t* __restrict__ row_ptr,
                            const int32_t* __restrict__ sid, const double* __restrict__ cp, int range_bits, int apart, int split,
                            const unsigned char* __restrict__ also_apart, uint64_t* keys, uint32_t* vals, int* err,
-                           unsigned long long* n_split = nullptr ) {
+                           unsigned long long* n_split = nullptr , uint64_t short_classes = 0) {
     uint64_t i = (uint64_t)blockIdx.x * blockDim.x + threadIdx.x;
     if (i >= N1) return;
     int e = 0;
     uint32_t nf = 0;
-    uint64_t key = row_key_of(i, M, row_ptr, sid, cp, range_bits, apart, &e, split, &nf);
+    uint64_t key = row_key_of(i, M, row_ptr, sid, cp, range_bits, apart, &e, split, &nf, short_classes);
     if (n_split && nf) { atomicAdd(&n_split[0], 1ull); atomicAdd(&n_split[1], (unsigned long long)nf); }
-    if (also_apart && also_apart[i] && (int)(key >> (64 - kShapeBits)) < 2 * kShapesPerFmt) key |= 1ull << kKeyApartBit;
+    if (also_apart && also_apart[i] && shape_fmt_of_id((int)(key >> (64 - kShapeBits))) != kFmtF64X) key |= 1ull << kKeyApartBit;
     if (e) *err = e;
     if (e == 1) return;
     keys[i] = key;
     vals[i] = (uint32_t)i;
+}
+
+constexpr int kLenHist = 257;
+__global__ void k_row_length_hist(uint64_t N1, const uint64_t* __restrict__ row_ptr, const double* __restrict__ cp, int range_bits,
+                                  unsigned long long* hist ) {
+    __shared__ unsigned int h[2 * kLenHist];
+    for (int i = threadIdx.x; i < 2 * kLenHist; i += blockDim.x) h[i] = 0;
+    __syncthreads();
+    for (uint64_t i = (uint64_t)blockIdx.x * blockDim.x + threadIdx.x; i < N1; i += (uint64_t)gridDim.x * blockDim.x) {
+        const uint64_t fr = row_ptr[i], to = row_ptr[i + 1];
+        if (to < fr || to - fr > 256) continue;
+        const int fmt = (cp && row_takes_q32(cp, fr, to, range_bits)) ? kFmtQ32 : kFmtF64;
+        atomicAdd(&h[fmt * kLenHist + (int)(to - fr)], 1u);
+    }
+    __syncthreads();
+    for (int i = threadIdx.x; i < 2 * kLenHist; i += blockDim.x)
+        if (h[i]) atomicAdd(&hist[i], (unsigned long long)h[i]);
+}
+#ifndef RSEM_SHORT_CLASS_MIN_UNITS
+#define RSEM_SHORT_CLASS_MIN_UNITS 8
+#endif
+constexpr int kShortClassMinUnits = RSEM_SHORT_CLASS_MIN_UNITS;
+inline uint64_t short_classes_worth_it(const unsigned long long* hist, uint32_t target_waves, uint32_t forced_T, int min_units) {
+    uint64_t rows[2][kShortPerFmt] = {}, n_slices = 0;
+    for (int f = 0; f < 2; f++)
+        for (int L = 1; L < kLenHist; L++) {
+            const unsigned long long n = hist[f * kLenHist + L];
+            if (!n) continue;
+            int fmt, lg, K, cut;
+            const int id = shape_id_of((uint64_t)L, 0xffffffffu, f == kFmtQ32);
+            shape_of_id(id, fmt, lg, K, cut);
+            n_slices += (n + (64u >> lg) - 1) >> (6 - lg);
+            if (id >= kFullShapes) rows[f][id - kFullShapes] += n;
+        }
+    const uint32_t T = forced_T ? forced_T : std::min<uint64_t>(256, std::max<uint64_t>(8, n_slices / std::max(1u, target_waves)));
+    uint64_t mask = 0;
+    for (int f = 0; f < 2; f++)
+        for (int i = 0; i < kShortPerFmt; i++) {
+            int fmt, lg, K, cut;
+            shape_of_id(kFullShapes + i, fmt, lg, K, cut);
+            const uint64_t slices = rows[f][i] >> (6 - lg);
+            if (slices >= (uint64_t)min_units * 4 * T && slices > 0) mask |= 1ull << (f * 32 + i);
+        }
+    return mask;
 }
 
 __global__ void k_shape_bounds(uint64_t N1, const uint64_t* __restrict__ keys, uint32_t* first) {
@@ -172,6 +273,7 @@
     uint64_t fr = row_ptr[orig];
     int L = (int)(row_ptr[orig + 1] - fr);
     const uint64_t pl_local = (uint64_t)slice_local * S.K * 64;
+    const uint64_t vl_local = (uint64_t)slice_local * shape_val_stride(S);
     const uint64_t pl0 = S.plane_base * 64 + pl_local;
     const uint32_t slot = S.slot_base + slice_local * shape_R(S) + r;
     Q32Scale q{0};
@@ -185,22 +287,22 @@
     for (int c = 0; c < L; c++) {
         if (S.fmt == kFmtF64X && !in_split_window(sid[fr + c], anchor, reach)) continue;
         const uint64_t off = (uint64_t)(ci >> S.lg) * 64 + r * G + (ci & (G - 1));
+        bool ok;
+        const uint64_t voff = vl_local + shape_val_off(S, r, ci, &ok);
         ++ci;
+        if (!ok) { if (err) *err = 4; continue; }
         if (kIds) ssid[pl0 + off] = sid[fr + c];
         if (cp) {
-            if (S.fmt == kFmtQ32) ((uint32_t*)(sval + S.val_base))[pl_local + off] = q32_mantissa(cp[fr + c], q.e);
-            else ((double*)(sval + S.val_base))[pl_local + off] = cp[fr + c];
+            if (S.fmt == kFmtQ32) ((uint32_t*)(sval + S.val_base))[voff] = q32_mantissa(cp[fr + c], q.e);
+            else ((double*)(sval + S.val_base))[voff] = cp[fr + c];
         }
     }
     if (ncp) sncp[slot] = ncp[orig];
 }
 
-__global__ void k_unfill_sell(const Shape* __restrict__ shapes, int n_shapes, uint32_t T, uint32_t n_sell_rows,
-                              const uint32_t* __restrict__ order, const uint64_t* __restrict__ row_ptr, const int32_t* __restrict__ ssid,
-                              const unsigned char* __restrict__ sval, int32_t* sid, double* cp) {
-    const uint32_t p = blockIdx.x * blockDim.x + threadIdx.x;
-    if (p >= n_sell_rows) return;
-    const Shape S = shapes[find_shape_by_row(shapes, n_shapes, p)];
+__host__ __device__ inline void sell_unfill_row(const Shape& S, uint32_t T, uint32_t p, const uint32_t* __restrict__ order,
+                                                const uint64_t* __restrict__ row_ptr, const int32_t* __restrict__ ssid,
+                                                const unsigned char* __restrict__ sval, int32_t* sid, double* cp) {
     const int G = shape_G(S);
     uint32_t slice_local, r;
     row_to_slot(S, T, p - S.row_base, slice_local, r);
@@ -208,12 +310,20 @@
     const uint64_t fr = row_ptr[orig];
     const int L = (int)(row_ptr[orig + 1] - fr);
     const uint64_t pl_local = (uint64_t)slice_local * S.K * 64;
+    const uint64_t vl_local = (uint64_t)slice_local * shape_val_stride(S);
     const uint64_t pl0 = S.plane_base * 64 + pl_local;
     for (int c = 0; c < L; c++) {
         const uint64_t off = (uint64_t)(c >> S.lg) * 64 + r * G + (c & (G - 1));
         sid[fr + c] = ssid[pl0 + off];
-        cp[fr + c] = ((const double*)(sval + S.val_base))[pl_local + off];
-    }
+        cp[fr + c] = ((const double*)(sval + S.val_base))[vl_local + shape_val_off(S, r, c)];
+    }
+}
+__global__ void k_unfill_sell(const Shape* __restrict__ shapes, int n_shapes, uint32_t T, uint32_t n_sell_rows,
+                              const uint32_t* __restrict__ order, const uint64_t* __restrict__ row_ptr, const int32_t* __restrict__ ssid,
+                              const unsigned char* __restrict__ sval, int32_t* sid, double* cp) {
+    const uint32_t p = blockIdx.x * blockDim.x + threadIdx.x;
+    if (p >= n_sell_rows) return;
+    sell_unfill_row(shapes[find_shape_by_row(shapes, n_shapes, p)], T, p, order, row_ptr, ssid, sval, sid, cp);
 }
 
 template <bool kIds>
@@ -396,6 +506,8 @@
     uint32_t n_slots = 0;
     uint64_t n_planes = 0;
     uint64_t val_bytes = 0;
+    uint64_t n_val_entries = 0;
+    uint64_t short_classes = 0;
     uint32_t n_q32_rows = 0;
     uint64_t n_q32_planes = 0;
     uint64_t n_sid_planes_loaded = 0;
@@ -452,8 +564,7 @@
 inline int sell_build_far(SellLayout& L, hipStream_t st, const uint64_t* d_row_ptr, const int32_t* d_sid, const uint64_t* d_keys_sorted) {
     const uint32_t nx = L.n_x_rows;
     if (!nx) return RSEM_OK;
-    const uint32_t nxs = L.n_slots - L.x_slot_base;
-    L.n_x_slots = nxs;
+    const uint32_t nxs = L.n_x_slots;
     if (d_keys_sorted) {
         RSEM_HIP_TRY(dmalloc(&L.d_xanchor, nx));
         hipLaunchKernelGGL(k_x_anchors, dim3(rsem::ceil_div(nx, kBlock)), dim3(kBlock), 0, st, nx, L.x_row_base, d_keys_sorted, L.d_xanchor);
@@ -527,7 +638,8 @@
 
 inline int sell_build(SellLayout& L, hipStream_t st, uint64_t N1, int32_t M, const uint64_t* d_row_ptr,
                       const int32_t* d_sid, uint32_t target_waves, uint32_t forced_T = 0,
-                      const double* d_cp_for_q32 = nullptr, int range_bits = 0, const unsigned char* d_also_apart = nullptr, int split = 0) {
+                      const double* d_cp_for_q32 = nullptr, int range_bits = 0, const unsigned char* d_also_apart = nullptr, int split = 0,
+                      int short_min_units = 0 ) {
     L.N1 = N1;
     int apart = kLayoutWindow;
     if (const char* e = getenv("RSEM_HIP_APART")) apart = atoi(e) ? kLayoutWindow : 0;
@@ -547,6 +659,24 @@
     RSEM_HIP_TRY(dmalloc(&d_err, 1));
     RSEM_HIP_TRY(hipMemsetAsync(d_err, 0, sizeof(int), st));
     RSEM_HIP_TRY(hipMemsetAsync(d_first, 0xff, kShapeIds * sizeof(uint32_t), st));
+    uint64_t short_classes = 0;
+    if (N1 && short_min_units > 0) {
+        unsigned long long* d_hist = nullptr;
+        unsigned long long h_hist[2 * kLenHist];
+        RSEM_HIP_TRY(dmalloc(&d_hist, 2 * kLenHist));
+        hipError_t e = hipMemsetAsync(d_hist, 0, sizeof(h_hist), st);
+        if (e == hipSuccess) {
+            hipLaunchKernelGGL(k_row_length_hist, dim3((unsigned)std::min<uint64_t>(4096, rsem::ceil_div(N1, kBlock))), dim3(kBlock), 0, st, N1, d_row_ptr,
+                               d_cp_for_q32, range_bits, d_hist);
+            e = hipGetLastError();
+        }
+        if (e == hipSuccess) e = hipMemcpyAsync(h_hist, d_hist, sizeof(h_hist), hipMemcpyDeviceToHost, st);
+        if (e == hipSuccess) e = hipStreamSynchronize(st);
+        (void)hipFree(d_hist);
+        if (e != hipSuccess) { cleanup(); RSEM_HIP_TRY(e); }
+        short_classes = short_classes_worth_it(h_hist, target_waves, forced_T, short_min_units);
+    }
+    L.short_classes = short_classes;
     if (N1) {
         int do_split = apart ? split : 0;
         if (do_split) {
@@ -554,7 +684,7 @@
             RSEM_HIP_TRY(dmalloc(&d_ns, 2));
             RSEM_HIP_TRY(hipMemsetAsync(d_ns, 0, 2 * sizeof(unsigned long long), st));
             hipLaunchKernelGGL(k_row_keys, dim3(rsem::ceil_div(N1, kBlock)), dim3(kBlock), 0, st, N1, M, d_row_ptr, d_sid,
-                               d_cp_for_q32, range_bits, apart, do_split, d_also_apart, d_keys, d_vals, d_err, d_ns);
+                               d_cp_for_q32, range_bits, apart, do_split, d_also_apart, d_keys, d_vals, d_err, d_ns, short_classes);
             RSEM_HIP_TRY(hipGetLastError());
             RSEM_HIP_TRY(hipMemcpyAsync(h_ns, d_ns, sizeof(h_ns), hipMemcpyDeviceToHost, st));
             RSEM_HIP_TRY(hipStreamSynchronize(st));
@@ -562,7 +692,7 @@
         }
         if (!do_split) {
             hipLaunchKernelGGL(k_row_keys, dim3(rsem::ceil_div(N1, kBlock)), dim3(kBlock), 0, st, N1, M, d_row_ptr, d_sid,
-                               d_cp_for_q32, range_bits, apart, 0, d_also_apart, d_keys, d_vals, d_err, (unsigned long long*)nullptr);
+                               d_cp_for_q32, range_bits, apart, 0, d_also_apart, d_keys, d_vals, d_err, (unsigned long long*)nullptr, short_classes);
             RSEM_HIP_TRY(hipGetLastError());
         }
         size_t tb = 0;
@@ -594,6 +724,7 @@
     L.x_slot_base = 0;
     L.n_far = 0;
     L.n_x_slots = 0;
+    L.n_val_entries = 0;
     uint32_t long_first = (h_first[kLongShape] == 0xffffffffu) ? (uint32_t)N1 : h_first[kLongShape];
     L.n_sell_rows = long_first;
     L.n_long_rows = (uint32_t)N1 - long_first;
@@ -603,9 +734,11 @@
         for (int j = id + 1; j < kMaxShapes; j++)
             if (h_first[j] != 0xffffffffu) { next = h_first[j]; break; }
         Shape& S = L.h_shapes[L.n_shapes++];
-        S.fmt = id / kShapesPerFmt;
-        S.lg = (id % kShapesPerFmt) / 4;
-        S.K = id % 4 + 1;
+        {
+            int fmt = 0, lg = 0, K = 1, cut = 0;
+            shape_of_id(id, fmt, lg, K, cut);
+            S.fmt = fmt; S.lg = lg; S.K = K; S.cut = cut; S.reserved = 0;
+        }
         S.row_base = h_first[id];
         S.n_rows = next - h_first[id];
         uint32_t rps = shape_R(S);
@@ -617,11 +750,13 @@
         L.n_slices += S.n_slices;
         L.n_planes += (uint64_t)S.n_slices * S.K;
         L.n_slots += S.n_slices * rps;
-        L.val_bytes += (uint64_t)S.n_slices * S.K * plane_bytes(S.fmt);
+        L.val_bytes += shape_val_bytes(S);
+        L.n_val_entries += (uint64_t)S.n_slices * shape_val_stride(S);
         if (S.fmt == kFmtQ32) { L.n_q32_rows += S.n_rows; L.n_q32_planes += (uint64_t)S.n_slices * S.K; }
         if (S.fmt == kFmtF64X) {
             if (!L.n_x_rows) { L.x_row_base = S.row_base; L.x_slot_base = S.slot_base; }
             L.n_x_rows += S.n_rows;
+            L.n_x_slots += S.n_slices * rps;
         }
     }
     uint32_t T = forced_T ? forced_T : L.n_slices / std::max(1u, target_waves);
@@ -857,14 +992,15 @@
 
 inline int sell_build_refined(SellLayout& L, hipStream_t st, uint64_t N1, int32_t M, const uint64_t* d_row_ptr, const int32_t* d_sid,
                               uint32_t target_waves, uint32_t forced_T, const double* d_cp_for_q32, int range_bits, int window_cap,
-                              std::vector<Unit>& units, Unit** d_units, unsigned long long* n_strays = nullptr, int split = 0) {
+                              std::vector<Unit>& units, Unit** d_units, unsigned long long* n_strays = nullptr, int split = 0,
+                              int short_min_units = 0) {
     unsigned char* d_also = nullptr;
     unsigned long long* d_n = nullptr;
     if (n_strays) *n_strays = 0;
     const char* knob = getenv("RSEM_HIP_APART");
     const bool refine = !(knob && atoi(knob) == 0);
     for (int pass = 0; pass < 2; pass++) {
-        int rc = sell_build(L, st, N1, M, d_row_ptr, d_sid, target_waves, forced_T, d_cp_for_q32, range_bits, d_also, split);
+        int rc = sell_build(L, st, N1, M, d_row_ptr, d_sid, target_waves, forced_T, d_cp_for_q32, range_bits, d_also, split, short_min_units);
         if (rc == RSEM_OK) rc = sell_build_units(L, units, window_cap);
         if (rc != RSEM_OK) { (void)hipFree(d_also); return rc; }
         (void)hipFree(*d_units);
diff --git a/rsem_amd/csrc/sell_shape.hpp b/rsem_amd/csrc/sell_shape.hpp
--- a/rsem_amd/csrc/sell_shape.hpp
+++ b/rsem_amd/csrc/sell_shape.hpp
@@ -1,6 +1,7 @@
 #pragma once
 
 constexpr int kFmtF64 = 0, kFmtQ32 = 1, kFmtF64X = 2;
+constexpr int kShapeTableMax = 148;
 
 struct Shape {
     uint64_t plane_base;
@@ -13,6 +14,8 @@
     int32_t lg;
     int32_t fmt;
     uint64_t val_base;
+    int32_t cut;
+    int32_t reserved;
 };
 
 __host__ __device__ inline uint32_t plane_bytes(int fmt) { return fmt == kFmtQ32 ? 256u : 512u; }
@@ -24,6 +27,31 @@
     return 64u >> S.lg;
 }
 
+__host__ __device__ inline uint32_t shape_val_stride(int K, int cut) {
+    return (uint32_t)(K * 64 - 16 * cut);
+}
+__host__ __device__ inline uint32_t shape_val_stride(const Shape& S) { return shape_val_stride(S.K, S.cut); }
+__host__ __device__ inline int shape_Gk(int lg, int cut) {
+    return ((1 << lg) * (4 - cut)) >> 2;
+}
+__host__ __device__ inline int shape_Gk(const Shape& S) { return shape_Gk(S.lg, S.cut); }
+__host__ __device__ inline uint32_t shape_val_off(int lg, int K, int cut, uint32_t r, int c, bool* ok = nullptr) {
+    const int k = c >> lg, g = c & ((1 << lg) - 1);
+    if (k < K - 1 || cut == 0) {
+        if (ok) *ok = k < K;
+        return (uint32_t)k * 64u + (r << lg) + (uint32_t)g;
+    }
+    const int Gk = shape_Gk(lg, cut);
+    if (ok) *ok = k == K - 1 && g < Gk;
+    return (uint32_t)(K - 1) * 64u + r * (uint32_t)Gk + (uint32_t)g;
+}
+__host__ __device__ inline uint32_t shape_val_off(const Shape& S, uint32_t r, int c, bool* ok = nullptr) {
+    return shape_val_off(S.lg, S.K, S.cut, r, c, ok);
+}
+__host__ __device__ inline uint64_t shape_val_bytes(const Shape& S) {
+    return (uint64_t)S.n_slices * shape_val_stride(S) * (plane_bytes(S.fmt) / 64u);
+}
+
 __host__ __device__ inline void row_to_slot(const Shape& S, uint32_t T, uint32_t q, uint32_t& slice_local, uint32_t& r) {
     const uint32_t R = shape_R(S), rpb = R * T;
     const uint32_t b = q / rpb, qb = q % rpb;
```

Result: faster. 633.4 billion read-alignments/s, median of 6 (+4.3%).
